# loro-dev/loro

Hardware: AMD Instinct MI355X
Metric: merged docs/sec (batch of N docs x M remote ops) (higher is better)
Workload: dtype u32; 1 GPU; configs[1]: 10000 docs/GPU x 100000-op automerge-paper-shaped text trace, 2 concurrent peers, 3 FastUpdates blobs/doc (4683 op runs, 30 changes, 103435 blob bytes/doc); docs_per_gpu=10000, ops_per_doc=100000, contexts_in_flight=2, streams_per_context=2

## Files before the change

loro_amd/csrc/lm_k_dag.h:

```cpp
#pragma once
#include "lm_k_decode.h"

namespace lm {

#ifndef LM_FUSE_ROWS
#define LM_FUSE_ROWS 1
#endif
#ifndef LM_NO_NODE_CUT
#define LM_NO_NODE_CUT 0
#endif

struct DevDag {
  uint32_t* blk_sorted;
  uint32_t* chg_node;
  uint32_t* node_done;
  uint32_t* node_lam;
};

LM_KERNEL void k_doc_ranges(Dev d) {
  uint32_t doc = (uint32_t)(lmw::bid() * lmw::bdim() + lmw::tid());
  if (doc >= d.n_docs) return;
  DocMeta m;
  uint32_t* mw = (uint32_t*)&m;
  for (uint32_t i = 0; i < sizeof(DocMeta) / 4; i++) mw[i] = 0;
// ... 34 lines not shown
  if (m.status == ST_MF_BAIL) { if (lane == 0) { d.doc[doc].status = ST_DATA_CORRUPTION; d.doc[doc].flags = DF_REDO; } return; }
  if (status_fatal(m.status)) { if (lane == 0) d.doc[doc].status = m.status; return; }
  uint32_t P = 0;
  bool too_many = false;
  for (uint32_t i = 0; i < m.n_praw; i++) {
    uint64_t v = d.peer_raw[m.praw0 + i];
    bool hit = false;
    for (uint32_t k = (uint32_t)lane; k < P; k += 64) hit |= s_peers[k] == v;
    if (!lmw::any(hit)) {
      if (P >= MAX_PEERS - 1) { too_many = true; break; }
      if (lane == 0) s_peers[P] = v;
      P++;
      lmw::block_sync();
    }
  }
  if (too_many) { if (lane == 0) LM_SETERR(d.doc[doc].status, ST_UNSUPPORTED); return; }
  lmw::block_sync();
  for (uint32_t e = (uint32_t)lane; e < P; e += 64) {
    uint64_t v = s_peers[e];
    uint32_t rank = 0;
    for (uint32_t j = 0; j < P; j++) rank += s_peers[j] < v ? 1u : 0u;
    d.peer_uniq[m.praw0 + rank] = v;
  }
  lmw::block_sync();
  for (uint32_t i = (uint32_t)lane; i < m.n_praw; i += 64) {
    uint64_t v = d.peer_raw[m.praw0 + i];
    uint32_t lo = 0, hi = P;
    while (lo < hi) { uint32_t mid = (lo + hi) >> 1; if (d.peer_uniq[m.praw0 + mid] < v) lo = mid + 1; else hi = mid; }
    d.peer_map[m.praw0 + i] = lo;
  }
  lmw::block_sync();
  uint32_t C = 0;
  bool cont_overflow = false;
  for (uint32_t i = 0; i < m.n_cid; i++) {
    const uint32_t* w = d.cid_raw + (uint64_t)(m.cid0 + i) * 4;
    uint32_t kr = w[0], blk = w[3];
    const uint32_t* bo = d.boff + (uint64_t)blk * BCN;
    bool is_root = (kr & 0x100) != 0;
    uint64_t noff = 0;
    uint32_t nlen = 0, cpeer = 0, cctr = 0;
    if (is_root) { noff = d.key_off[bo[BC_KEY] + w[2]]; nlen = d.key_len[bo[BC_KEY] + w[2]]; }
    else { cpeer = d.peer_map[bo[BC_PEER] + w[1]]; cctr = w[2]; }
    uint32_t idx = NONE;
    for (uint32_t c0 = 0; c0 < C && idx == NONE; c0 += 64) {
      bool match = false;
      if (c0 + (uint32_t)lane < C) {
        ContRow c = d.cont[m.cid0 + c0 + lane];
        if (c.kind_root == kr) {
          if (is_root) {
            if (c.name_len == nlen) {
              match = true;
              const uint8_t* a = d.data + c.name_off;
              const uint8_t* b = d.data + noff;
              for (uint32_t k = 0; k < nlen; k++) if (a[k] != b[k]) { match = false; break; }
            }
          } else match = c.peer == cpeer && c.counter == cctr;
        }
      }
      uint64_t mm = lmw::ballot(match);
      if (mm) idx = c0 + (uint32_t)lmw::ffs64(mm);
    }
    if (idx != NONE) {}
    else {
      if (C >= MAX_CONTAINERS) { cont_overflow = true; break; }
      idx = C;
      if (lane == 0) {
        ContRow c;
        c.name_off = noff; c.name_len = nlen; c.kind_root = kr; c.peer = cpeer; c.counter = cctr; c.touched = 0; c.pad = 0;
        d.cont[m.cid0 + C] = c;
      }
      C++;
      lmw::block_sync();
    }
    if (lane == 0) d.cid_map[m.cid0 + i] = idx;
  }
  if (lane == 0) {
    d.doc[doc].status = cont_overflow ? ST_UNSUPPORTED : m.status;
    d.doc[doc].n_peers = P;
    d.doc[doc].n_cont = C;
  }
  (void)s_n;
}

LM_KERNEL void k_remap(Dev d, uint32_t n_ops, uint32_t n_chg) {
  uint32_t t = (uint32_t)(lmw::bid() * lmw::bdim() + lmw::tid());
  uint32_t m_chg = NONE, m_bit = 0;
  if (t < n_ops) {
    uint32_t blk = d.op_blk[t];
    const BlockDesc& bd = d.blk[blk];
    if (bd.status == ST_OK && d.doc[bd.doc].status == ST_OK) {
      const uint32_t* bo = d.boff + (uint64_t)blk * BCN;
      OpRow r = d.op[t];
      uint32_t local = r.cidx_kind & 0xffff, kind = (r.cidx_kind >> 16) & 0xff;
      uint32_t ci = d.cid_map[bo[BC_CID] + local];
      if (r.cidx_kind & OPF_NESTED) {
        const uint8_t* vend = d.data + bd.base + bd.sec_rel[SEC_VALUES] + bd.sec_len[SEC_VALUES];
        Rd v{d.data + d.op_val[t], vend, false};
        uint32_t n_keys = d.bcnt[(uint64_t)blk * BCN + BC_KEY];
        if (kind == OK_STYLE_START) { (void)rd_u8(v); (void)rd_uleb(v); (void)rd_uleb(v); }
        uint32_t vf = 0;
        skip_loro_value_keys(v, vf, n_keys);
        if ((vf & VF_CORRUPT) && !v.bad) LM_SETERR(d.doc[bd.doc].status, ST_DATA_CORRUPTION);
      }
      r.cidx_kind = ci | (kind << 16);
      if (kind == OK_DEL || kind == OK_LIST_MOVE || kind == OK_LIST_SET) r.a0 = d.peer_map[bo[BC_PEER] + r.a0];
      else if (kind == OK_MAP_SET || kind == OK_MAP_DEL) r.a0 = bo[BC_KEY] + (uint32_t)r.prop;
      d.op[t] = r;
      m_chg = r.chg; m_bit = ci & 63;
    }
  }
  {
    uint32_t p_chg = lmw::shfl_up(m_chg, 1), p_bit = lmw::shfl_up(m_bit, 1);
    bool lead = m_chg != NONE && (lmw::lane() == 0 || p_chg != m_chg || p_bit != m_bit);
    if (lead) lmw::atomic_or(&d.chg_mask[2 * (uint64_t)m_chg + (m_bit >> 5)], 1u << (m_bit & 31));
  }
  if (t < n_chg) {
    ChangeRow c = d.chg[t];
    const BlockDesc& bd = d.blk[c.blk];
    if (bd.status == ST_OK && d.doc[bd.doc].status == ST_OK) {
      const uint32_t* bo = d.boff + (uint64_t)c.blk * BCN;
      c.peer = d.peer_map[bo[BC_PEER] + 0];
      d.chg[t] = c;
      for (uint32_t k = c.dep0; k < c.dep0 + c.n_dep; k++) d.dep_peer[k] = d.peer_map[bo[BC_PEER] + d.dep_peer[k]];
    }
  }
}

LM_DEV uint32_t find_change(const Dev& d, const DocMeta& m, uint32_t peer, uint32_t c) {
  uint32_t lo = d.peer_chg0[m.praw0 + peer], hi = d.peer_chg1[m.praw0 + peer];
  uint32_t end = hi;
  while (lo < hi) {
    uint32_t mid = (lo + hi) >> 1;
    const ChangeRow& ch = d.chg[d.chg_sorted[m.chg0 + mid]];
    if (ch.ctr + ch.len <= c) lo = mid + 1; else hi = mid;
  }
  if (lo >= end) return NONE;
  const ChangeRow& ch = d.chg[d.chg_sorted[m.chg0 + lo]];
  return ch.ctr <= c ? lo : NONE;
}

#ifdef LM_PROF_DAG
#define DAG_PH(i) do { uint64_t n_ = lmw::clock(); dpacc[i] += n_ - dptp; dptp = n_; } while (0)
#else
#define DAG_PH(i) do {} while (0)
#endif
LM_DEV bool vvo_has(const Dev& d, uint32_t doc) { return d.vvo && d.vvo_off[doc + 1] - d.vvo_off[doc] > 8; }
LM_DEV uint64_t vvo_synth_peer(const Dev& d, uint32_t doc) { uint64_t v = 0; const uint8_t* p = d.vvo + d.vvo_off[doc]; for (int k = 0; k < 8; k++) v |= (uint64_t)p[k] << (8 * k); return v; }
LM_DEV uint32_t vvo_base_end(const Dev& d, uint32_t doc, uint64_t peer) {
  if (!vvo_has(d, doc)) return 0;
  Rd r = rd_make(d.vvo + d.vvo_off[doc] + 8, d.vvo_off[doc + 1] - d.vvo_off[doc] - 8);
  const uint64_t n = rd_uleb(r);
  for (uint64_t i = 0; i < n && !r.bad; i++) {
    const uint64_t q = rd_uleb(r);
    const uint64_t z = rd_uleb(r);
    if (q == peer) return (uint32_t)(z >> 1);
    if (q > peer) break;
  }
  return 0;
}
LM_KERNEL void k_dag_a(Dev d, DevDag g) {
  uint32_t doc = (uint32_t)lmw::bid();
  int lane = lmw::lane();
#ifdef LM_PROF_DAG
  uint64_t dpacc[8] = {0, 0, 0, 0, 0, 0, 0, 0}, dptp = lmw::clock();
#endif
  LM_SHARED(uint32_t, s_valid, MAX_PEERS);
  LM_SHARED(uint32_t, s_ext, MAX_PEERS);
  DocMeta m = d.doc[doc];
  if (status_fatal(m.status)) return;
  uint32_t P = m.n_peers;
  for (uint32_t i = (uint32_t)lane; i < m.n_blk; i += 64) {
    uint32_t bi = m.blk0 + i;
    const BlockDesc& b = d.blk[bi];
    uint64_t key = ((uint64_t)d.chg[d.boff[(uint64_t)bi * BCN + BC_CHG]].peer << 32) | b.counter_start;
    uint32_t rank = 0;
    for (uint32_t j = 0; j < m.n_blk; j++) {
      uint32_t bj = m.blk0 + j;
      uint64_t kj = ((uint64_t)d.chg[d.boff[(uint64_t)bj * BCN + BC_CHG]].peer << 32) | d.blk[bj].counter_start;
      rank += (kj < key || (kj == key && j < i)) ? 1u : 0u;
    }
    g.blk_sorted[m.blk0 + rank] = bi;
  }
  for (uint32_t p = (uint32_t)lane; p < P; p += 64) { s_ext[p] = vvo_base_end(d, doc, d.peer_uniq[m.praw0 + p]); d.peer_base[m.praw0 + p] = s_ext[p]; s_valid[p] = 0; d.peer_chg0[m.praw0 + p] = 0; d.peer_chg1[m.praw0 + p] = 0; }
  lmw::block_sync();
  DAG_PH(0);
  uint32_t n_sorted = 0;
  bool any_skip = false;
  uint32_t pending = 0;
  uint32_t cur_peer = NONE, covered = 0;
  bool gap = false;
  for (uint32_t i = 0; i < m.n_blk; i++) {
    uint32_t bi = g.blk_sorted[m.blk0 + i];
    const BlockDesc& b = d.blk[bi];
    uint32_t c0 = d.boff[(uint64_t)bi * BCN + BC_CHG];
    uint32_t peer = d.chg[c0].peer;
    if (peer != cur_peer) {
      if (cur_peer != NONE && lane == 0) { s_ext[cur_peer] = covered; d.peer_chg1[m.praw0 + cur_peer] = n_sorted; }
      cur_peer = peer; covered = s_ext[peer]; gap = false;
      if (lane == 0) d.peer_chg0[m.praw0 + peer] = n_sorted;
    }
    if (b.counter_start > covered) gap = true;
    uint32_t bend = b.counter_start + b.counter_len;
    for (uint32_t k0 = 0; k0 < b.n_changes; k0 += 64) {
      uint32_t k = k0 + (uint32_t)lane;
      bool in = k < b.n_changes;
      uint32_t row = c0 + (in ? k : 0);
      ChangeRow ch = d.chg[row];
// ... 60 lines not shown
  for (uint32_t p = (uint32_t)lane; p < P; p += 64) { d.peer_chg0[m.praw0 + p] = NONE; d.peer_chg1[m.praw0 + p] = 0; }
  lmw::block_sync();
  for (uint32_t i = (uint32_t)lane; i < n_valid; i += 64) {
    uint32_t peer = d.chg[d.chg_sorted[m.chg0 + i]].peer;
    uint32_t prev = i ? d.chg[d.chg_sorted[m.chg0 + i - 1]].peer : NONE;
    uint32_t next = i + 1 < n_valid ? d.chg[d.chg_sorted[m.chg0 + i + 1]].peer : NONE;
    if (prev != peer) d.peer_chg0[m.praw0 + peer] = i;
    if (next != peer) d.peer_chg1[m.praw0 + peer] = i + 1;
  }
  lmw::block_sync();
  for (uint32_t p = (uint32_t)lane; p < P; p += 64) {
    if (d.peer_chg0[m.praw0 + p] == NONE) { d.peer_chg0[m.praw0 + p] = 0; d.peer_chg1[m.praw0 + p] = 0; }
    d.peer_end[m.praw0 + p] = s_valid[p];
    d.peer_ext[m.praw0 + p] = s_ext[p];
  }
  {
    uint32_t run = 0;
    for (uint32_t p0 = 0; p0 < P; p0 += 64) {
      uint32_t p = p0 + (uint32_t)lane;
      uint32_t e = p < P ? s_ext[p] : 0;
      uint32_t inc = lmw::scan_incl_add(e);
      if (p < P) d.elem_base[m.praw0 + p] = run + inc - e;
      run += lmw::bcast(inc, 63);
    }
    if (vvo_has(d, doc)) { if (run > m.atoms && lane == 0) d.doc[doc].atoms = run; }
    else if (run > m.atoms && lane == 0) LM_SETERR(d.doc[doc].status, ST_INTERNAL);
  }
  lmw::mem_fence();
  lmw::block_sync();
  DAG_PH(4);
  for (uint32_t i = (uint32_t)lane; i < n_valid; i += 64) {
    uint32_t row = d.chg_sorted[m.chg0 + i];
    const ChangeRow& ch = d.chg[row];
    for (uint32_t k = ch.dep0; k < ch.dep0 + ch.n_dep; k++) {
      uint32_t q = d.dep_peer[k], c = d.dep_ctr[k];
      uint32_t ci = NONE;
      if (q == ch.peer && i > 0 && c + 1 == ch.ctr) {
        const ChangeRow& pv = d.chg[d.chg_sorted[m.chg0 + i - 1]];
        if (pv.peer == q && pv.ctr <= c && c < pv.ctr + pv.len) ci = i - 1;
      }
      if (ci == NONE && q < P) ci = find_change(d, m, q, c);
      d.dep_ci[k] = ci;
      if (q != ch.peer && ci != NONE && d.chg_skip[row] == 0)
        lmw::atomic_or(&d.chg_flag[d.chg_sorted[m.chg0 + ci]], 2u);
    }
  }
  lmw::mem_fence();
  lmw::block_sync();
  DAG_PH(5);
  const bool cut_doc = !LM_NO_NODE_CUT && m.n_op >= d.cut_min_rows;
  uint32_t n_nodes = 0;
  for (uint32_t i0 = 0; i0 < n_valid; i0 += 64) {
    uint32_t i = i0 + (uint32_t)lane;
    bool in = i < n_valid;
    bool head = false;
    if (in) {
      uint32_t row = d.chg_sorted[m.chg0 + i];
      const ChangeRow& ch = d.chg[row];
      bool cont = false;
      if (d.chg_skip[row] != 0) cont = true;
      else if (ch.n_dep == 1 && d.dep_peer[ch.dep0] == ch.peer && ch.ctr > 0 && d.dep_ctr[ch.dep0] == ch.ctr - 1) cont = true;
      if (cont && (i == 0 || d.chg[d.chg_sorted[m.chg0 + i - 1]].peer != ch.peer)) cont = false;
      if (cont && cut_doc && d.chg_skip[row] == 0 && (d.chg_flag[d.chg_sorted[m.chg0 + i - 1]] & 2u)) cont = false;
      head = !cont;
    }
    uint64_t hm = lmw::ballot(head);
    uint32_t nid = n_nodes + (uint32_t)lmw::popc64(hm & ((2ull << lane) - 1)) - 1;
    if (in) {
      g.chg_node[m.chg0 + i] = nid;
      if (head) d.node_first[m.chg0 + nid] = i;
    }
    n_nodes += (uint32_t)lmw::popc64(hm);
  }
  lmw::block_sync();
  for (uint32_t n = (uint32_t)lane; n < n_nodes; n += 64) {
    d.node_last[m.chg0 + n] = (n + 1 < n_nodes ? d.node_first[m.chg0 + n + 1] : n_valid) - 1;
    g.node_done[m.chg0 + n] = 0;
  }
  DAG_PH(6);
  uint32_t n_map = 0, n_el = 0, n_style = 0;
  for (uint32_t i = (uint32_t)lane; i < m.n_blk; i += 64) {
    const BlockDesc& kb = d.blk[m.blk0 + i];
    if (kb.status != ST_OK) continue;
    n_map += kb.flags & 0x7fffffffu; n_el += kb.pad; n_style += kb.flags >> 31;
  }
  bool has_ml = false;
  for (uint32_t c = (uint32_t)lane; c < m.n_cont; c += 64) has_ml |= (d.cont[m.cid0 + c].kind_root & 0xff) == CK_MOVABLE;
  has_ml = lmw::any(has_ml);
  bool any_skip_doc = lmw::any(any_skip);
  n_map = lmw::reduce_add(n_map);
  n_el = lmw::reduce_add(n_el);
  n_style = lmw::reduce_add(n_style);
  if (lane == 0) {
    d.doc[doc].n_valid_chg = n_valid;
    d.doc[doc].n_nodes = n_nodes;
    d.doc[doc].pending_lo = pending;
    d.doc[doc].pending_hi = 0;
    d.doc[doc].n_mapop = n_map;
    d.doc[doc].n_elems = n_el;
    if (cut_doc) d.doc[doc].flags |= DF_CUT;
    if (has_ml) d.doc[doc].flags |= DF_MOVABLE;
    else if (!any_skip_doc && n_style == 0) d.doc[doc].flags |= DF_PLAIN | ((LM_FUSE_ROWS && (uint64_t)n_valid * 8 > m.n_op) ? DF_FUSED : 0u);
  }
#ifdef LM_PROF_DAG
  DAG_PH(7);
  if (lane == 0) for (int i = 0; i < 8; i++) atomicAdd(&d.prof[i], (unsigned long long)dpacc[i]);
#endif
}

LM_KERNEL void k_dag_b(Dev d, DevDag g, uint32_t res_mode) {
  uint32_t doc = (uint32_t)lmw::bid();
  int lane = lmw::lane();
  DocMeta m = d.doc[doc];
  if (status_fatal(m.status)) return;
  uint32_t P = m.n_peers, N = m.n_nodes;
  uint64_t vvh0 = ((uint64_t)m.vvh0_hi << 32) | m.vvh0_lo;
  uint32_t n_done = 0;
  if (res_mode == 2) {
    for (uint32_t p = (uint32_t)lane; p < P; p += 64) d.peer_end[m.praw0 + p] = d.peer_end_all[m.praw0 + p];
    lmw::mem_fence();
    lmw::block_sync();
    N = 0;
  }
  LM_SHARED(uint32_t, s_next, MAX_PEERS);
  LM_SHARED(uint32_t, s_pend, MAX_PEERS);
  for (uint32_t p = (uint32_t)lane; p < P; p += 64) { s_next[p] = 0; s_pend[p] = 0; }
  lmw::block_sync();
  if (res_mode != 2)
    for (uint32_t n = (uint32_t)lane; n < N; n += 64) {
      uint32_t pr = d.chg[d.chg_sorted[m.chg0 + d.node_first[m.chg0 + n]]].peer;
      uint32_t prev = n ? d.chg[d.chg_sorted[m.chg0 + d.node_first[m.chg0 + n - 1]]].peer : NONE;
      uint32_t next = n + 1 < N ? d.chg[d.chg_sorted[m.chg0 + d.node_first[m.chg0 + n + 1]]].peer : NONE;
      if (pr < P && prev != pr) s_next[pr] = n;
      if (pr < P && next != pr) s_pend[pr] = n + 1;
    }
  lmw::block_sync();
  for (uint32_t pass = 0; pass <= N && n_done < N; pass++) {
    uint32_t batch0 = n_done;
    if (m.flags & DF_CUT) {
    {
      uint32_t pick = NONE;
      for (uint32_t p0 = ((P - 1) >> 6) << 6;; p0 -= 64) {
        uint32_t pr = p0 + (uint32_t)lane;
        uint32_t n = pr < P ? s_next[pr] : NONE;
        bool ready = false;
        if (pr < P && n < s_pend[pr] && !g.node_done[m.chg0 + n]) {
          ready = true;
          const ChangeRow& ch = d.chg[d.chg_sorted[m.chg0 + d.node_first[m.chg0 + n]]];
          for (uint32_t k = ch.dep0; k < ch.dep0 + ch.n_dep; k++) {
            uint32_t ci = d.dep_ci[k];
            if (ci == NONE || !g.node_done[m.chg0 + g.chg_node[m.chg0 + ci]]) ready = false;
          }
        }
        uint64_t rm = lmw::ballot(ready);
        if (rm) { pick = p0 + (uint32_t)(63 - __builtin_clzll((unsigned long long)rm)); break; }
        if (p0 == 0) break;
      }
      if (pick != NONE) {
        lmw::block_sync();
        uint32_t n = s_next[pick];
        lmw::block_sync();
        if (lane == 0) { d.node_order[m.chg0 + n_done] = n; s_next[pick] = n + 1; }
        n_done++;
      }
    }
    } else {
    for (uint32_t p0 = 0; p0 < P; p0 += 64) {
// ... 79 lines not shown
    cnt = rd_uleb(r);
    if (r.bad || cnt > f1 - f0) ferr = ST_DECODE_ERROR;
    for (uint64_t i = 0; i < cnt && !ferr; i++) {
      uint64_t peer = rd_uleb(r);
      int64_t ctr = rd_zigzag(r);
      if (r.bad) { ferr = ST_DECODE_ERROR; break; }
      uint32_t lo = 0, hi = P;
      while (lo < hi) { uint32_t mid = (lo + hi) >> 1; if (d.peer_uniq[m.praw0 + mid] < peer) lo = mid + 1; else hi = mid; }
      if (lo >= P || d.peer_uniq[m.praw0 + lo] != peer || ctr < 0 || (uint64_t)ctr >= d.peer_end[m.praw0 + lo] ||
          find_change(d, m, lo, (uint32_t)ctr) == NONE)
        ferr = ST_FRONTIERS_NOT_FOUND;
    }
    if (!ferr && rd_left(r) != 0) ferr = ST_DECODE_ERROR;
  }
  lmw::block_sync();
  if (ferr && res_mode == 2) { if (lane == 0) { d.doc[doc].front_err = ferr; d.doc[doc].flags |= DF_FRONT_ERR; } return; }
  if (ferr) { if (lane == 0) LM_SETERR(d.doc[doc].status, ferr); return; }
  if (res_mode == 0) for (uint32_t p = (uint32_t)lane; p < P; p += 64) d.peer_end_all[m.praw0 + p] = d.peer_end[m.praw0 + p];
  lmw::block_sync();
  for (uint32_t p0 = 0; p0 < P; p0 += 64) {
    uint32_t p = p0 + (uint32_t)lane, acc = 0;
    Rd r = rd_make(d.front + f0, f1 - f0);
    (void)rd_uleb(r);
    for (uint64_t i = 0; i < cnt; i++) {
      uint64_t peer = rd_uleb(r);
      uint32_t ctr = (uint32_t)rd_zigzag(r);
      uint32_t lo = 0, hi = P;
      while (lo < hi) { uint32_t mid = (lo + hi) >> 1; if (d.peer_uniq[m.praw0 + mid] < peer) lo = mid + 1; else hi = mid; }
      uint32_t ci = find_change(d, m, lo, ctr);
      if (p < P) {
        uint32_t x = d.vvh[vvh0 + (uint64_t)g.chg_node[m.chg0 + ci] * P + p];
        if (p == lo && ctr + 1 > x) x = ctr + 1;
        acc = x > acc ? x : acc;
      }
    }
    if (p < P) d.peer_end[m.praw0 + p] = acc;
  }
}

template <bool BYTES>
LM_DEV bool fill_text_coop(const Dev& d, const uint8_t* s, uint32_t nbytes, uint64_t e0, uint32_t len) {
  uint32_t lane = (uint32_t)lmw::lane();
  bool bad = false;
  uint32_t n = 0;
  for (uint32_t c = 0; c < nbytes;) {
    uint32_t i = c + lane;
    bool inb = i < nbytes;
    uint32_t b = inb ? s[i] : 0u;
    if (!lmw::ballot(b >= 0x80)) {
      if (inb & (n + lane < len)) { if (BYTES) d.tb[e0 + n + lane] = (uint8_t)b; else d.cp[e0 + n + lane] = b; }
      uint32_t took = nbytes - c < 64 ? nbytes - c : 64u;
      n += took; c += 64;
      continue;
    }
    bool last_chunk = c + 61 >= nbytes;
    bool mine = inb & (last_chunk | (lane < 61));
    bool lead = mine & ((b & 0xC0) != 0x80);
    uint32_t b1 = lmw::shfl(b, (int)((lane + 1) & 63)), b2 = lmw::shfl(b, (int)((lane + 2) & 63)), b3 = lmw::shfl(b, (int)((lane + 3) & 63));
    uint64_t lm_ = lmw::ballot(lead);
    uint32_t rank = (uint32_t)lmw::popc64(lm_ & ((1ull << lane) - 1));
    if (lead) {
      uint32_t cpv, extra;
      if (b < 0x80) { cpv = b; extra = 0; }
      else if ((b & 0xE0) == 0xC0) { cpv = ((b & 0x1F) << 6) | (b1 & 0x3F); extra = 1; }
      else if ((b & 0xF0) == 0xE0) { cpv = ((b & 0x0F) << 12) | ((b1 & 0x3F) << 6) | (b2 & 0x3F); extra = 2; }
      else if ((b & 0xF8) == 0xF0) { cpv = ((b & 0x07) << 18) | ((b1 & 0x3F) << 12) | ((b2 & 0x3F) << 6) | (b3 & 0x3F); extra = 3; }
      else { cpv = 0; extra = 0; bad = true; }
      if (i + extra >= nbytes) bad = true;
      if (extra >= 1 && (b1 & 0xC0) != 0x80) bad = true;
      if (extra >= 2 && (b2 & 0xC0) != 0x80) bad = true;
      if (extra >= 3 && (b3 & 0xC0) != 0x80) bad = true;
      if (lane + extra > 63) bad = true;
      if (n + rank < len) {
        if (BYTES) { d.tb[e0 + n + rank] = (uint8_t)(extra ? TB_WIDE : cpv); if (extra) d.cp[e0 + n + rank] = cpv; }
        else d.cp[e0 + n + rank] = cpv;
      }
    }
    n += (uint32_t)lmw::popc64(lm_);
    c += 61;
  }
  return lmw::any(bad) || n != len;
}

LM_KERNEL void k_elem_fill(Dev d) {
  uint32_t bi = (uint32_t)lmw::bid();
  int lane = lmw::lane();
  const BlockDesc& bd = d.blk[bi];
  if (bd.status != ST_OK) return;
  uint32_t doc = bd.doc;
  const DocMeta& m = d.doc[doc];
  if (status_fatal(m.status)) return;
  if (d.res_old_blobs && (m.flags & DF_FILL_KEPT) && bd.blob - d.doc_blob[doc] < d.res_old_blobs[doc]) return;
  const bool span = d.span != 0;
  const uint32_t* off = d.boff + (uint64_t)bi * BCN;
  uint32_t op0 = off[BC_OP], n_op = d.bcnt[(uint64_t)bi * BCN + BC_OP];
  uint32_t chg0 = off[BC_CHG];
  uint32_t peer = d.chg[chg0].peer;
  uint64_t ebase = (((uint64_t)m.elem0_hi << 32) | m.elem0_lo) + d.elem_base[m.praw0 + peer];
  uint32_t ext = d.peer_ext[m.praw0 + peer];
  uint64_t doc_data0 = d.blob_off[d.doc_blob[doc]];
  const uint8_t* vsec = d.data + bd.base + bd.sec_rel[SEC_VALUES];
  const uint8_t* lim = vsec + bd.sec_len[SEC_VALUES];
  LM_SHARED(uint32_t, s_inc, 64);
  LM_SHARED(uint32_t, s_nb, 64);
  LM_SHARED(uint32_t, s_src, 64);
  LM_SHARED(uint32_t, s_dst, 64);
  bool bad = false;
  for (uint32_t g0 = 0; g0 < n_op; g0 += 64) {
    uint32_t row = op0 + g0 + (uint32_t)lane;
    bool valid = g0 + (uint32_t)lane < n_op;
    OpRow r;
    r.cidx_kind = 0; r.prop = 0; r.len = 0; r.ctr = 0; r.a0 = r.a1 = 0; r.a2 = 0; r.chg = 0;
    if (valid) r = d.op[row];
    uint32_t kind = (r.cidx_kind >> 16) & 0xff;
    bool want = valid && (kind == OK_TEXT_INS || kind == OK_LIST_INS || kind == OK_STYLE_START || kind == OK_STYLE_END);
    const bool cand_text = want && kind == OK_TEXT_INS;
    if (want && !d.chg_flag[r.chg]) want = false;
    if (want && r.ctr + r.len > ext) want = false;
    if (cand_text && !want) {
      const uint8_t* q = d.data + d.op_val[row];
      Rd vq = rd_make(q, q < lim ? (uint64_t)(lim - q) : 0ull);
      uint64_t nb = rd_uleb(vq);
      if (vq.bad || nb > rd_left(vq)) bad = true;
      else {
        uint32_t n = 0;
        for (uint64_t i = 0; i < nb && !bad;) {
          uint32_t b0 = vq.p[i], extra = b0 < 0x80 ? 0u : (b0 & 0xE0) == 0xC0 ? 1u : (b0 & 0xF0) == 0xE0 ? 2u : (b0 & 0xF8) == 0xF0 ? 3u : 4u;
          if (extra == 4 || i + extra >= nb + (extra ? 0 : 1)) { bad = true; break; }
          for (uint32_t k = 1; k <= extra; k++) if ((vq.p[i + k] & 0xC0) != 0x80) bad = true;
          n++; i += extra + 1;
        }
        if (n != r.len) bad = true;
      }
    }
    uint64_t e0 = ebase + r.ctr;
    if (want && (kind == OK_STYLE_START || kind == OK_STYLE_END)) { if (span) d.tb[e0] = (uint8_t)TB_ANCHOR; d.cp[e0] = CP_ANCHOR | (row - m.op0); want = false; }
    const uint8_t* p = want ? d.data + d.op_val[row] : lim;
    Rd v = rd_make(p, (uint64_t)(lim - p));
    uint64_t nbytes = 0;
    bool is_long = false, flat = false;
    if (want && kind == OK_TEXT_INS) {
      nbytes = rd_uleb(v);
      if (v.bad || nbytes > rd_left(v)) { bad = true; want = false; }
      else if (span && nbytes == r.len) flat = true;
      else if (nbytes > 64) { is_long = true; }
      else {
        const uint8_t* s = v.p;
        uint32_t n = 0;
        for (uint32_t i = 0; i < (uint32_t)nbytes;) {
          if (span && i + 4 <= (uint32_t)nbytes && n + 3 < r.len) {
            uint32_t w = ld32u(s + i);
            if (!(w & 0x80808080u)) { st32u(d.tb + e0 + n, w); n += 4; i += 4; continue; }
          }
          if (!span && i + 4 <= (uint32_t)nbytes) {
            uint32_t q0 = s[i], q1 = s[i + 1], q2 = s[i + 2], q3 = s[i + 3];
            if (((q0 | q1 | q2 | q3) & 0x80) == 0) {
              if (n + 3 < r.len) { d.cp[e0 + n] = q0; d.cp[e0 + n + 1] = q1; d.cp[e0 + n + 2] = q2; d.cp[e0 + n + 3] = q3; }
              else { if (n < r.len) d.cp[e0 + n] = q0; if (n + 1 < r.len) d.cp[e0 + n + 1] = q1; if (n + 2 < r.len) d.cp[e0 + n + 2] = q2; }
              n += 4; i += 4;
              continue;
            }
          }
          uint32_t b = s[i], cpv, extra;
          if (b < 0x80) { cpv = b; extra = 0; }
          else if ((b & 0xE0) == 0xC0) { cpv = b & 0x1F; extra = 1; }
          else if ((b & 0xF0) == 0xE0) { cpv = b & 0x0F; extra = 2; }
          else if ((b & 0xF8) == 0xF0) { cpv = b & 0x07; extra = 3; }
          else { bad = true; break; }
          if (i + extra >= (uint32_t)nbytes) { bad = true; break; }
          for (uint32_t k = 1; k <= extra; k++) {
            uint32_t t = s[i + k];
            if ((t & 0xC0) != 0x80) bad = true;
            cpv = (cpv << 6) | (t & 0x3F);
          }
          if (n < r.len) {
            if (span) { d.tb[e0 + n] = (uint8_t)(extra ? TB_WIDE : cpv); if (extra) d.cp[e0 + n] = cpv; }
            else d.cp[e0 + n] = cpv;
          }
          n++;
          i += extra + 1;
        }
        if (n != r.len) bad = true;
      }
    } else if (want) {
      (void)rd_u8(v);
      uint64_t cnt = rd_uleb(v);
      if (cnt != r.len) bad = true;
      for (uint32_t k = 0; k < r.len && !bad; k++) {
        d.cp[e0 + k] = (uint32_t)((uint64_t)(v.p - d.data) - doc_data0);
        bool u = false;
        skip_loro_value(v, u);
        if (v.bad) bad = true;
      }
    }
    if (span) {
      uint32_t nd = flat ? ((uint32_t)nbytes + 3) / 4 : 0u;
      uint32_t inc = lmw::scan_incl_add(nd);
      uint32_t total = lmw::bcast(inc, 63);
      if (total) {
        lmw::block_sync();
        s_inc[lane] = inc; s_nb[lane] = (uint32_t)nbytes; s_src[lane] = (uint32_t)(v.p - vsec); s_dst[lane] = r.ctr;
        lmw::block_sync();
        uint32_t hi = 0;
        for (uint32_t f0 = 0; f0 < total; f0 += 64) {
          uint32_t f = f0 + (uint32_t)lane;
          if (f < total) {
            uint32_t lo = 0, hh = 63;
            while (lo < hh) { uint32_t mid = (lo + hh) >> 1; if (s_inc[mid] > f) hh = mid; else lo = mid + 1; }
            uint32_t nbr = s_nb[lo];
            uint32_t k4 = 4u * (f - (s_inc[lo] - (nbr + 3) / 4));
            const uint8_t* src = vsec + s_src[lo] + k4;
            uint8_t* dst = d.tb + ebase + s_dst[lo] + k4;
            if (k4 + 4 <= nbr) { uint32_t w = ld32u(src); hi |= w; st32u(dst, w); }
            else for (uint32_t i = 0; k4 + i < nbr; i++) { uint32_t b = src[i]; hi |= b; dst[i] = (uint8_t)b; }
          }
        }
        if (hi & 0x80808080u) bad = true;
      }
    }
    uint64_t lm_ = lmw::ballot(is_long);
    while (lm_) {
      int l = lmw::ffs64(lm_);
      lm_ &= lm_ - 1;
      uint64_t sp = (uint64_t)(v.p - d.data);
      uint32_t sp_lo = lmw::bcast((uint32_t)sp, l), sp_hi = lmw::bcast((uint32_t)(sp >> 32), l);
      uint32_t nb = lmw::bcast((uint32_t)nbytes, l);
      uint32_t e_lo = lmw::bcast((uint32_t)e0, l), e_hi = lmw::bcast((uint32_t)(e0 >> 32), l);
      uint32_t ln = lmw::bcast(r.len, l);
      const uint8_t* str = d.data + (((uint64_t)sp_hi << 32) | sp_lo);
      uint64_t e0l = ((uint64_t)e_hi << 32) | e_lo;
      if (span ? fill_text_coop<true>(d, str, nb, e0l, ln) : fill_text_coop<false>(d, str, nb, e0l, ln)) bad = true;
    }
  }
  if (lmw::any(bad) && lane == 0) LM_SETERR(d.doc[doc].status, ST_DATA_CORRUPTION);
}

}
```

loro_amd/csrc/lm_k_decode.h:

```cpp
#pragma once
#include "lm_dev_util.h"

namespace lm {

struct Dev {
  const uint8_t* data;
  const uint64_t* blob_off;
  const uint32_t* blob_len;
  const uint32_t* doc_blob;
  uint32_t n_blobs, n_docs;
  uint32_t span;
  const uint32_t* res_old_blobs;
  uint32_t loc_cleared;
  uint32_t* posdel;
  const uint64_t* posdel_off;
  uint32_t* pd_row_idx;
  const uint8_t* vvo;
  const uint64_t* vvo_off;
  const uint8_t* doc_fused;
  uint32_t n_op_rows;
  uint32_t* blk_kind;
  uint32_t posdel_redo;
  uint32_t no_linear;
  uint32_t res_vis;
// ... 338 lines not shown
      lmw::atomic_add(&d.dec_stat[0], 1u); lmw::atomic_max32(&d.dec_stat[1], span);
      lmw::atomic_max32(&d.dec_stat[2], (uint32_t)((bd.base + bd.sec_rel[SEC_OPS]) & 15) + bd.sec_rel[SEC_VALUES] - bd.sec_rel[SEC_OPS]);
    }
  }
  c[BC_CHG] = N;
  c[BC_DEP] = (uint32_t)ndep;
  c[BC_OP] = fused ? 0u : (uint32_t)nops;
  c[BC_KEY] = (uint32_t)nkeys;
  c[BC_CID] = (uint32_t)ncid;
  c[BC_PEER] = (uint32_t)np;
  c[BC_MAPOP] = fused ? (uint32_t)nops : 0u;
  c[BC_ATOMS] = bd.counter_len;
}

static constexpr uint32_t VF_UNSUPPORTED = 1u, VF_CORRUPT = 2u;
template <bool KEYS = false, class R> LM_DEV void skip_loro_value_fs(R& r, uint32_t& vf, int cdepth, uint32_t* f_cnt, uint32_t n_keys = 0xffffffffu);
template <class R> LM_DEV void skip_loro_value_top(R& r, uint32_t& vf, int cdepth, uint32_t* f_cnt, uint32_t tag_peek) {
  if (tag_peek > 6 || r.bad) { skip_loro_value_fs(r, vf, cdepth, f_cnt); return; }
  (void)rd_u8(r);
  if (tag_peek == 3) (void)rd_sleb(r);
  else if (tag_peek == 4) rd_skip(r, 8);
  else if (tag_peek >= 5) { uint64_t l = rd_uleb(r); rd_skip(r, l); }
}
template <bool KEYS, class R> LM_DEV void skip_loro_value_fs(R& r, uint32_t& vf, int cdepth, uint32_t* f_cnt, uint32_t n_keys) {
  uint32_t f_map = 0;
  int sp = 0;
  uint32_t cnt = 1;
  bool in_map = false;
  for (uint32_t guard = 0; guard < (1u << 28); guard++) {
    while (cnt == 0) {
      if (sp == 0) return;
      sp--;
      cnt = f_cnt[sp];
      in_map = (f_map >> sp) & 1;
    }
    if (r.bad) return;
    cnt--;
    if (in_map) {
      uint64_t kidx = rd_uleb(r);
      if (KEYS) vf |= (kidx >= n_keys && !r.bad) ? VF_CORRUPT : 0u;
    }
    uint32_t tag = rd_u8(r);
    switch (tag) {
      case 0: case 1: case 2: break;
      case 3: (void)rd_sleb(r); break;
      case 4: rd_skip(r, 8); break;
      case 5: case 6: { uint64_t l = rd_uleb(r); rd_skip(r, l); break; }
      case 7: case 8: {
        uint64_t n = rd_uleb(r);
        if (KEYS) vf |= (n > (1u << 28) && !r.bad) ? VF_CORRUPT : 0u;
        if (n > (1u << 28) || sp >= 16) { r.bad = true; return; }
        f_cnt[sp] = cnt;
        f_map = (f_map & ~(1u << sp)) | ((in_map ? 1u : 0u) << sp);
        sp++;
        cnt = (uint32_t)n;
        in_map = tag == 8;
        break;
      }
      case 9: { (void)rd_u8(r); if (sp > cdepth) vf |= VF_UNSUPPORTED; break; }
      default: if (KEYS) vf |= r.bad ? 0u : VF_CORRUPT; r.bad = true; return;
    }
  }
  r.bad = true;
}
LM_DEV void skip_loro_value(Rd& r, uint32_t& vf, int cdepth = -1) {
  uint32_t f_cnt[16];
  skip_loro_value_fs(r, vf, cdepth, f_cnt);
}
LM_DEV void skip_loro_value_keys(Rd& r, uint32_t& vf, uint32_t n_keys) {
  uint32_t f_cnt[16];
  skip_loro_value_fs<true>(r, vf, -1, f_cnt, n_keys);
}
LM_DEV void skip_loro_value(Rd& r, bool& unsupported, int cdepth = -1) {
  uint32_t vf = 0;
  skip_loro_value(r, vf, cdepth);
  if (vf & VF_UNSUPPORTED) unsupported = true;
}

#if defined(LM_EMU) && defined(LM_EMU_TRACE)
#define DEC_ST(code) do { if (!st) { if (getenv("LM_EMU_DEC")) fprintf(stderr, "lm emu: block verdict " #code " at %s:%d\n", __FILE__, __LINE__); st = (code); } } while (0)
#else
#define DEC_ST(code) do { st = st ? st : (code); } while (0)
#endif
LM_DEV void kc_add(uint32_t& n_map, uint32_t& n_el, uint32_t& n_style, uint32_t k, uint32_t len) {
  n_map += (k == OK_MAP_SET || k == OK_MAP_DEL || k == OK_LIST_MOVE || k == OK_LIST_SET || k == OK_OTHER) ? 1u : 0u;
  n_el += (k == OK_TEXT_INS || k == OK_LIST_INS || k == OK_STYLE_START || k == OK_STYLE_END) ? len : (k == OK_LIST_MOVE ? 1u : 0u);
  n_style += (k == OK_STYLE_START || k == OK_STYLE_END) ? 1u : 0u;
}
LM_DEV uint32_t kc_pack(uint32_t n_map, uint32_t n_style) { return (n_map & 0x7fffffffu) | (n_style ? 0x80000000u : 0u); }

static constexpr uint32_t DEC_RECLASS = 0xDEC0DE01u;
template <bool EXACT> LM_DEV void lane_skip_value(Rd& r, uint32_t& vf, int cdepth, uint32_t n_keys) {
  uint32_t f_cnt[16];
  if (EXACT) skip_loro_value_fs<true>(r, vf, cdepth, f_cnt, n_keys);
  else skip_loro_value_fs(r, vf, cdepth, f_cnt);
}
template <bool EXACT, bool HEAD = false> LM_DEV void block_decode_lane(Dev d) {
  uint32_t bi = (uint32_t)(lmw::bid() * lmw::bdim() + lmw::tid());
  if (bi >= d.n_blocks) return;
  BlockDesc bd = d.blk[bi];
  if (EXACT ? ((bd.status != ST_DECODE_ERROR && bd.status != ST_DATA_CORRUPTION) || bd.pad != DEC_RECLASS) : (bd.status != ST_OK)) return;
  if (HEAD != (d.doc_fused && d.doc_fused[bd.doc])) return;
  const uint32_t* off = d.boff + (uint64_t)bi * BCN;
  const uint32_t* cnt = d.bcnt + (uint64_t)bi * BCN;
  uint32_t N = bd.n_changes;
  uint32_t chg0 = off[BC_CHG], dep0 = off[BC_DEP], op0 = off[BC_OP], key0 = off[BC_KEY], cid0 = off[BC_CID], peer0 = off[BC_PEER];
  uint32_t n_peers = cnt[BC_PEER], n_ops = cnt[BC_OP], n_keys = cnt[BC_KEY], n_cids = cnt[BC_CID];
  int32_t st = ST_OK;
  bool unsupported = false;
  uint32_t kc_map = 0, kc_el = 0, kc_style = 0;
  Rd h = blk_sec(d, bd, SEC_HEADER);
  (void)rd_uleb(h);
  for (uint32_t i = 0; i < n_peers; i++) {
    uint64_t v = 0;
    for (int k = 0; k < 8; k++) v |= (uint64_t)rd_u8(h) << (8 * k);
    d.peer_raw[peer0 + i] = v;
  }
  {
    uint64_t known = 0;
    uint32_t ctr = bd.counter_start;
    for (uint32_t i = 0; i < N; i++) {
      uint64_t l;
      if (i + 1 < N) { l = rd_uleb(h); known += l; if (known > bd.counter_len) { st = ST_DECODE_ERROR; l = 0; } }
      else l = bd.counter_len - (known > bd.counter_len ? bd.counter_len : known);
      ChangeRow c;
      c.peer = 0; c.ctr = ctr; c.len = (uint32_t)l; c.dep0 = 0; c.n_dep = 0; c.op0 = 0; c.n_op = 0; c.blk = bi;
      d.chg[chg0 + i] = c;
      ctr += (uint32_t)l;
    }
    BoolCur bc = bool_make(h);
    for (uint32_t i = 0; i < N; i++) d.chg[chg0 + i].op0 = bool_next(bc) ? 1u : 0u;
    if (bc.rem != 0) bc.r.bad = true;
    RleCur dc = rle_make(bc.r);
    uint32_t dcur = dep0;
    uint64_t others_total = 0;
    for (uint32_t i = 0; i < N; i++) {
      uint64_t others = rle_next_uvar(dc);
      ChangeRow c = d.chg[chg0 + i];
      uint32_t ds = c.op0;
      if (dcur + ds + others > dep0 + cnt[BC_DEP]) { st = ST_DECODE_ERROR; others = 0; ds = 0; }
      others_total += others;
      c.dep0 = dcur;
      c.n_dep = ds + (uint32_t)others;
      if (ds) {
        if (c.ctr == 0) st = ST_DECODE_ERROR;
        d.dep_peer[dcur] = 0;
        d.dep_ctr[dcur] = c.ctr ? c.ctr - 1 : 0;
      }
      dcur += c.n_dep;
      d.chg[chg0 + i] = c;
    }
    if (dc.rem != 0) dc.r.bad = true;
    if (dcur - dep0 != cnt[BC_DEP]) st = ST_DECODE_ERROR;
    RleCur pc = rle_make(dc.r);
    uint64_t D = 0;
    for (uint32_t i = 0; i < N && others_total; i++) {
      ChangeRow c = d.chg[chg0 + i];
      for (uint32_t k = c.dep0 + c.op0; k < c.dep0 + c.n_dep; k++) {
        uint64_t pi = rle_next_uvar(pc);
        if (pi >= n_peers) { st = ST_DECODE_ERROR; pi = 0; }
        d.dep_peer[k] = (uint32_t)pi;
        D++;
      }
    }
    if (pc.rem != 0) pc.r.bad = true;
    Rd hr = pc.r;
    DodCur dd = dod_make(hr);
    for (uint32_t i = 0; i < N && D; i++) {
      ChangeRow c = d.chg[chg0 + i];
      for (uint32_t k = c.dep0 + c.op0; k < c.dep0 + c.n_dep; k++) {
        int64_t v = dod_next(dd);
        if (v < 0 || v >= (int64_t)MAX_COUNTER) { st = st ? st : ST_DECODE_ERROR; v = 0; }
// ... 18 lines not shown
    dod_skip(td, N);
    dod_finish(td, m, N);
    RleCur mc = rle_make(m);
    const uint64_t tot = rle_sum_uvar(mc, N);
    if (mc.rem != 0) mc.r.bad = true;
    if (mc.r.bad || tot > rd_left(mc.r)) DEC_ST(ST_DATA_CORRUPTION);
  }
  if (!HEAD) {
    Rd k = blk_sec(d, bd, SEC_KEYS);
    for (uint32_t i = 0; i < n_keys; i++) {
      uint64_t l = rd_uleb(k);
      d.key_off[key0 + i] = (uint64_t)(k.p - d.data);
      d.key_len[key0 + i] = (uint32_t)l;
      rd_skip(k, l);
    }
    if (k.bad) st = st ? st : ST_DECODE_ERROR;
  }
  uint32_t head_root = 0;
  {
    Rd k = blk_sec(d, bd, SEC_CIDS);
    if (n_cids) (void)rd_uleb(k);
    for (uint32_t i = 0; i < n_cids; i++) {
      uint64_t fields = rd_uleb(k);
      uint32_t is_root = rd_u8(k), kind = rd_u8(k);
      uint64_t pidx = rd_uleb(k);
      int64_t koc = rd_zigzag(k);
      if (fields != 4) st = st ? st : ST_DECODE_ERROR;
      uint32_t* w = d.cid_raw + (uint64_t)(cid0 + i) * 4;
      if (HEAD && is_root) {
        Rd kk = blk_sec(d, bd, SEC_KEYS);
        bool found = koc >= 0;
        uint64_t l = 0;
        for (int64_t q = 0; found && q <= koc; q++) { if (kk.p >= kk.end) { found = false; break; } l = rd_uleb(kk); if (q < koc) rd_skip(kk, l); if (kk.bad) found = false; }
        if (found && l > rd_left(kk)) found = false;
        if (!found || head_root >= n_keys) { DEC_ST(ST_DATA_CORRUPTION); d.key_off[key0 + (head_root < n_keys ? head_root : 0)] = 0; d.key_len[key0 + (head_root < n_keys ? head_root : 0)] = 0; koc = 0; }
        else { d.key_off[key0 + head_root] = (uint64_t)(kk.p - d.data); d.key_len[key0 + head_root] = (uint32_t)l; koc = head_root; }
        head_root++;
      }
      else if (is_root) { if (koc < 0 || (uint64_t)koc >= n_keys) { DEC_ST(ST_DATA_CORRUPTION); koc = 0; } }
      else { if (pidx >= n_peers) { DEC_ST(ST_DATA_CORRUPTION); pidx = 0; } if (koc < 0 || koc >= (int64_t)MAX_COUNTER) { st = st ? st : ST_UNSUPPORTED; koc = 0; } }
      w[0] = kind | (is_root ? 0x100u : 0u);
      w[1] = (uint32_t)pidx;
      w[2] = (uint32_t)koc;
      w[3] = bi;
    }
    if (k.bad) st = st ? st : ST_DECODE_ERROR;
  }
  if (HEAD) {
    d.blk[bi].status = (st != ST_OK || unsupported) ? (int32_t)ST_MF_BAIL : (int32_t)ST_OK;
    d.blk[bi].flags = kc_pack(d.blk_kind[bi] & 0x7fffffffu, 0); d.blk[bi].pad = 0;
    return;
  }
  {
    Rd o = blk_sec(d, bd, SEC_OPS);
    (void)rd_uleb(o); (void)rd_uleb(o);
    RleCur c_cont = rle_make(rd_bytes(o));
    RleCur c_prop = rle_make(rd_bytes(o));
    RleCur c_vt = rle_make(rd_bytes(o));
    RleCur c_len = rle_make(rd_bytes(o));
    Rd dsec = blk_sec(d, bd, SEC_DEL);
    bool has_del = dsec.p < dsec.end;
    RleCur d_peer = rle_make(dsec), d_ctr = rle_make(dsec), d_len = rle_make(dsec);
    if (has_del) {
      uint64_t outer = rd_uleb(dsec), ncols = rd_uleb(dsec);
      if (outer != 1 || ncols != 3) st = st ? st : ST_DECODE_ERROR;
      d_peer = rle_make(rd_bytes(dsec));
      d_ctr = rle_make(rd_bytes(dsec));
      d_len = rle_make(rd_bytes(dsec));
    }
    {
      bool colbad = false;
      { RleCur t = c_cont; uint32_t n = rle_drain(t, 2, n_ops); colbad |= t.r.bad || n != n_ops; }
      { RleCur t = c_prop; uint32_t n = rle_drain(t, 2, n_ops); colbad |= t.r.bad || n != n_ops; }
      { RleCur t = c_vt; uint32_t n = rle_drain(t, 0, n_ops); colbad |= t.r.bad || n != n_ops; }
      { RleCur t = c_len; uint32_t n = rle_drain(t, 1, n_ops); colbad |= t.r.bad || n != n_ops; }
      if (has_del) {
        RleCur t1 = d_peer, t2 = d_ctr, t3 = d_len;
        uint32_t n1 = rle_drain(t1, 2), n2 = rle_drain(t2, 2), n3 = rle_drain(t3, 2);
        colbad |= t1.r.bad || t2.r.bad || t3.r.bad || n1 != n2 || n1 != n3;
      }
      if (colbad) st = st ? st : ST_DECODE_ERROR;
    }
    Rd v = blk_sec(d, bd, SEC_VALUES);
    uint64_t counter = bd.counter_start;
    uint32_t change_index = 0;
    uint64_t next_boundary = N > 1 ? d.chg[chg0 + 1].ctr : (uint64_t)bd.counter_start + bd.counter_len;
    d.chg[chg0].op0 = op0;
    for (uint32_t row = 0; row < n_ops; row++) {
      int64_t ci = rle_next_delta(c_cont);
      int64_t prop = rle_next_delta(c_prop);
      uint32_t vt = rle_next_u8(c_vt) & 0x7f;
      uint64_t len = rle_next_uvar(c_len);
      if (ci < 0 || (uint64_t)ci >= n_cids) { DEC_ST(ST_DATA_CORRUPTION); ci = 0; }
      if (prop < INT32_MIN || prop > INT32_MAX) { st = st ? st : ST_DECODE_ERROR; prop = 0; }
      uint32_t ckind = n_cids ? (d.cid_raw[(uint64_t)(cid0 + (uint32_t)ci) * 4] & 0xff) : 0xff;
      OpRow r;
      r.cidx_kind = (uint32_t)ci;
      r.prop = (int32_t)prop;
      r.len = (uint32_t)len;
      r.ctr = (uint32_t)counter;
      r.a0 = 0; r.a1 = 0; r.a2 = 0;
      r.chg = chg0 + change_index;
      uint64_t val_at = (uint64_t)(v.p - d.data);
      uint32_t kind = OK_OTHER;
      uint32_t mark_len = 0;
      uint64_t mv_from = 0, mv_peer = 0, mv_lam = 0;
      uint32_t vfl = 0;
      bool nested = false;
      bool is_list_value = false;
      switch (vt) {
        case 0: case 1: case 2: case 8: case 9: break;
        case 3: (void)rd_sleb(v); break;
        case 4: rd_skip(v, 8); break;
        case 5: case 6: { uint64_t l = rd_uleb(v); rd_skip(v, l); break; }
        case 7: (void)rd_uleb(v); break;
        case 10: (void)rd_sleb(v); break;
        case 11: {
          is_list_value = v.p < v.end && *v.p == 7;
          nested = v.p < v.end && (*v.p == 7 || *v.p == 8);
          if (is_list_value) {
            Rd t = v;
            (void)rd_u8(t);
            r.a0 = (uint32_t)rd_uleb(t);
          }
          lane_skip_value<EXACT>(v, vfl, ckind == CK_MAP ? 0 : (is_list_value && (ckind == CK_LIST || ckind == CK_MOVABLE) ? 1 : (ckind > CK_TEXT && ckind != CK_MOVABLE ? 16 : -1)), n_keys);
          break;
        }
        case 12: {
          (void)rd_u8(v);
          mark_len = (uint32_t)rd_uleb(v);
          uint64_t key_idx = rd_uleb(v);
          if (key_idx >= n_keys) DEC_ST(ST_DATA_CORRUPTION);
          uint32_t u = 0;
          lane_skip_value<EXACT>(v, u, -1, n_keys);
          vfl |= u & VF_CORRUPT;
          nested = true;
          break;
        }
        case 13: { (void)rd_uleb(v); uint32_t isn = rd_u8(v); (void)rd_uleb(v); if (!isn) (void)rd_uleb(v); break; }
        case 14: mv_from = rd_uleb(v); mv_peer = rd_uleb(v); mv_lam = rd_uleb(v); break;
        case 15: {
          mv_peer = rd_uleb(v); mv_lam = rd_uleb(v);
          val_at = (uint64_t)(v.p - d.data);
          if (ckind == CK_MOVABLE) lane_skip_value<EXACT>(v, vfl, 0, n_keys);
          else { uint32_t u = 0; lane_skip_value<EXACT>(v, u, -1, n_keys); vfl |= u & VF_CORRUPT; }
          nested = true;
          break;
        }
        case 16: {
          (void)rd_uleb(v); (void)rd_uleb(v); (void)rd_uleb(v);
          uint32_t isn = rd_u8(v);
          if (!isn) { (void)rd_uleb(v); (void)rd_uleb(v); }
          break;
        }
        default: { uint64_t l = rd_uleb(v); rd_skip(v, l); break; }
      }
      if (vfl & VF_UNSUPPORTED) unsupported = true;
      if (vfl & VF_CORRUPT) DEC_ST(ST_DATA_CORRUPTION);
      if (EXACT && v.bad) DEC_ST(ST_DECODE_ERROR);
      bool take_del = false;
      if (ckind == CK_TEXT) {
        if (vt == 5) kind = OK_TEXT_INS;
        else if (vt == 9) { kind = OK_DEL; take_del = true; }
        else if (vt == 12) { kind = OK_STYLE_START; r.a0 = mark_len; }
        else if (vt == 0) kind = OK_STYLE_END;
        else DEC_ST(ST_DATA_CORRUPTION);
      } else if (ckind == CK_MAP) {
        if (prop < 0 || (uint64_t)prop >= n_keys) DEC_ST(ST_DATA_CORRUPTION);
        if (vt == 8) kind = OK_MAP_DEL;
        else if (vt == 11) kind = OK_MAP_SET;
        else DEC_ST(ST_DATA_CORRUPTION);
      } else if (ckind == CK_LIST) {
        if (vt == 11) { if (is_list_value) kind = OK_LIST_INS; else DEC_ST(ST_DATA_CORRUPTION); }
        else if (vt == 9) { kind = OK_DEL; take_del = true; }
        else DEC_ST(ST_DATA_CORRUPTION);
      } else if (ckind == CK_MOVABLE) {
        if (vt == 11) { if (is_list_value) kind = OK_LIST_INS; else DEC_ST(ST_DATA_CORRUPTION); }
        else if (vt == 9) { kind = OK_DEL; take_del = true; }
        else if (vt == 14 || vt == 15) {
          kind = vt == 14 ? OK_LIST_MOVE : OK_LIST_SET;
          if (mv_peer >= n_peers || mv_lam > 0xFFFFFFFFull || mv_from > 0x7FFFFFFFull || prop < 0 || len != 1) { DEC_ST(ST_DATA_CORRUPTION); mv_peer = 0; }
          r.a0 = (uint32_t)mv_peer; r.a1 = (uint32_t)mv_lam; r.a2 = (int32_t)(uint32_t)mv_from;
        } else DEC_ST(ST_DATA_CORRUPTION);
      }
      if (take_del) {
        if (!has_del) DEC_ST(ST_DATA_CORRUPTION);
        else {
          int64_t dp = rle_next_delta(d_peer), dctr = rle_next_delta(d_ctr), dl = rle_next_delta(d_len);
          if (dp < 0 || (uint64_t)dp >= n_peers) { DEC_ST(ST_DATA_CORRUPTION); dp = 0; }
          if (dl == 0 || dl > (int64_t)MAX_COUNTER || dl < -(int64_t)MAX_COUNTER) { DEC_ST(ST_DATA_CORRUPTION); dl = 1; }
          if (dctr < 0 || dctr >= (int64_t)MAX_COUNTER) { DEC_ST(ST_DATA_CORRUPTION); dctr = 0; }
          r.a0 = (uint32_t)dp; r.a1 = (uint32_t)dctr; r.a2 = (int32_t)dl;
          if (d_peer.r.bad || d_ctr.r.bad || d_len.r.bad) DEC_ST(ST_DATA_CORRUPTION);
        }
      }
      r.cidx_kind |= (kind << 16) | ((nested && (vt != 12 || kind == OK_STYLE_START)) ? OPF_NESTED : 0u);
      kc_add(kc_map, kc_el, kc_style, kind, (uint32_t)len);
      d.op[op0 + row] = r;
      d.op_val[op0 + row] = val_at;
      d.op_blk[op0 + row] = bi;
      counter += len;
      if (counter > MAX_COUNTER) { st = st ? st : ST_UNSUPPORTED; counter = MAX_COUNTER; }
      if (change_index >= N) { DEC_ST(ST_DATA_CORRUPTION); change_index = N - 1; }
      d.chg[chg0 + change_index].n_op++;
      if (counter > next_boundary && change_index + 1 < N) DEC_ST(ST_DATA_CORRUPTION);
      if (counter >= next_boundary && change_index + 1 < N) {
        change_index++;
        d.chg[chg0 + change_index].op0 = op0 + row + 1;
        next_boundary = change_index + 1 < N ? d.chg[chg0 + change_index + 1].ctr : (uint64_t)bd.counter_start + bd.counter_len;
      }
    }
    for (uint32_t i = 1; i < N; i++) if (d.chg[chg0 + i].n_op == 0) d.chg[chg0 + i].op0 = op0 + n_ops;
    if (c_cont.r.bad || c_prop.r.bad || c_vt.r.bad || c_len.r.bad || v.bad) st = st ? st : ST_DECODE_ERROR;
    if (counter != (uint64_t)bd.counter_start + bd.counter_len) DEC_ST(ST_DATA_CORRUPTION);
  }
  if (EXACT) { if (st == ST_DATA_CORRUPTION || st == ST_DECODE_ERROR) d.blk[bi].status = st; return; }
  if (st == ST_OK && unsupported) st = ST_UNSUPPORTED;
  d.blk[bi].status = st;
  d.blk[bi].flags = kc_pack(kc_map, kc_style); d.blk[bi].pad = (st == ST_DECODE_ERROR || st == ST_DATA_CORRUPTION) ? DEC_RECLASS : kc_el;
}
LM_KERNEL void k_block_decode(Dev d) { block_decode_lane<false>(d); }
LM_KERNEL void k_block_head(Dev d) { block_decode_lane<false, true>(d); }
LM_KERNEL void k_block_reclassify(Dev d) { block_decode_lane<true>(d); }

}

#include "lm_k_decode_wave.h"
```

loro_amd/csrc/lm_k_decode_wave.h:

```cpp
#pragma once

namespace lm {

#ifndef LM_DEC_G
#define LM_DEC_G 8
#endif
#ifndef LM_NO_PARTIAL_STAGE
#define LM_NO_PARTIAL_STAGE 0
#endif
static constexpr uint32_t DEC_G = LM_DEC_G;
static constexpr uint32_t DEC_R = 8;
static constexpr uint32_t DEC_WW = 6;
static constexpr uint32_t DEC_VW2 = 128;
static constexpr uint32_t DEC_LDS_FIXED = DEC_G * 16 * 4 + DEC_G * DEC_R * 8 * 4 + DEC_G * DEC_R * DEC_WW * 4 + DEC_G * DEC_VW + DEC_G * DEC_VW2;
static constexpr uint32_t DEC_KINDS = 16;
LM_DEV void dec_err(uint32_t& key, uint32_t row, uint32_t prio, int32_t code) {
  uint32_t k = (row << 8) | (prio << 4) | (uint32_t)code;
  if (k < key) key = k;
}

#ifdef LM_PROF_DEC
#define DEC_PH(i) do { uint64_t n_ = lmw::clock(); pacc[i] += n_ - ptp; ptp = n_; } while (0)
#else
#define DEC_PH(i) do {} while (0)
// ... 234 lines not shown
    }
    {
      Rd m = sec(SEC_META);
      DodCur td = dod_make(m);
      dod_skip(td, N);
      dod_finish(td, m, N);
      RleCur mc = rle_make(m);
      const uint64_t tot = rle_sum_uvar(mc, N);
      if (mc.rem != 0) mc.r.bad = true;
      if (mc.r.bad || tot > rd_left(mc.r)) st = st ? st : ST_DATA_CORRUPTION;
    }
    {
      Rd k = sec(SEC_KEYS);
      for (uint32_t i = 0; i < n_keys; i++) {
        uint64_t l = rd_uleb(k);
        d.key_off[key0 + i] = abs_of(k.p);
        d.key_len[key0 + i] = (uint32_t)l;
        rd_skip(k, l);
      }
      if (k.bad) st = st ? st : ST_DECODE_ERROR;
    }
    {
      Rd k = sec(SEC_CIDS);
      if (n_cids) (void)rd_uleb(k);
      for (uint32_t i = 0; i < n_cids; i++) {
        uint64_t fields = rd_uleb(k);
        uint32_t is_root = rd_u8(k), kind = rd_u8(k);
        uint64_t pidx = rd_uleb(k);
        int64_t koc = rd_zigzag(k);
        if (fields != 4) st = st ? st : ST_DECODE_ERROR;
        uint32_t* w = d.cid_raw + (uint64_t)(cid0 + i) * 4;
        if (is_root) { if (koc < 0 || (uint64_t)koc >= n_keys) { st = st ? st : ST_DATA_CORRUPTION; koc = 0; } }
        else { if (pidx >= n_peers) { st = st ? st : ST_DATA_CORRUPTION; pidx = 0; } if (koc < 0 || koc >= (int64_t)MAX_COUNTER) { st = st ? st : ST_UNSUPPORTED; koc = 0; } }
        w[0] = kind | (is_root ? 0x100u : 0u);
        w[1] = (uint32_t)pidx;
        w[2] = (uint32_t)koc;
        w[3] = bi;
        if (i < DEC_KINDS) s_kinds[b * DEC_KINDS + i] = (uint8_t)kind;
      }
      if (k.bad) st = st ? st : ST_DECODE_ERROR;
    }
  }
  lmw::block_sync();
  DEC_PH(1);
  RleCur col = rle_make(rd_make(blk_p, 0));
  ColCur fcol = col_make((lm_lds_bytes)slot, 0, 0, false);
  bool has_del = false;
  uint32_t errk = 0xffffffffu;
  uint32_t kc_map = 0, kc_el = 0, kc_style = 0;
  bool colbad = false;
  uint32_t n_del_read = 0;
  bool shape_bad = false;
  if (ok) {
    Rd o = sec(SEC_OPS);
    uint64_t outer = rd_uleb(o), ncols = rd_uleb(o);
    Rd mine = rd_make(blk_p, 0);
    for (uint32_t c = 0; c < 4; c++) { Rd cc = rd_bytes(o); if (r == c) mine = cc; }
    if (outer != 1 || ncols != 4 || o.bad) shape_bad = true;
    Rd ds = sec(SEC_DEL);
    has_del = ds.p < ds.end;
    if (has_del) {
      uint64_t douter = rd_uleb(ds), dcols = rd_uleb(ds);
      if (douter != 1 || dcols != 3) shape_bad = true;
      for (uint32_t c = 4; c < 7; c++) { Rd cc = rd_bytes(ds); if (r == c) mine = cc; }
    }
    col = rle_make(mine);
    if (staged) fcol = col_make((lm_lds_bytes)slot, (uint32_t)(mine.p - (const uint8_t*)slot), (uint32_t)(mine.end - (const uint8_t*)slot), mine.bad);
  }
  uint32_t mode = r == 2 ? 0u : (r == 3 ? 1u : 2u);
  int64_t v_lo = 0, v_repl = 0;
  uint64_t v_span = 256;
  uint32_t v_prio = 0, v_mask = 0xffffffffu;
  int32_t v_code = ST_DATA_CORRUPTION;
  bool v_nz = false;
  if (r == 0) { v_span = n_cids; v_prio = 0; }
  else if (r == 1) { v_lo = INT32_MIN; v_span = 1ull << 32; v_prio = 1; v_code = ST_DECODE_ERROR; }
  else if (r == 2) { v_mask = 0x7f; }
  else if (r == 3) { v_span = (uint64_t)MAX_COUNTER + 1; v_repl = MAX_COUNTER; v_prio = 5; v_code = ST_UNSUPPORTED; }
  else if (r == 4) { v_span = n_peers; v_prio = 6; }
  else if (r == 5) { v_span = MAX_COUNTER; v_prio = 8; }
  else if (r == 6) { v_lo = -(int64_t)MAX_COUNTER; v_span = 2ull * MAX_COUNTER + 1; v_nz = true; v_repl = 1; v_prio = 7; }
  Rd v = rd_make(blk_p, 0);
  const uint64_t v_end_abs = ok ? bd.base + bdp->sec_rel[SEC_VALUES] + bdp->sec_len[SEC_VALUES] : 0ull;
  uint64_t counter = bd.counter_start;
  uint32_t change_index = 0, rows_in_change = 0;
  uint64_t next_boundary = 0;
  Rd hl7 = rd_make(d.data, 0);
  uint64_t kn7 = 0;
  auto next_len7 = [&]() -> uint64_t { uint64_t l = rd_uleb(hl7); kn7 += l; return kn7 > bd.counter_len ? 0ull : l; };
  bool unsupported = false;
  if (ok && r == 7) {
    v = rd_make(d.data + bd.base + bdp->sec_rel[SEC_VALUES], bdp->sec_len[SEC_VALUES]);
    hl7 = sec(SEC_HEADER);
    (void)rd_uleb(hl7);
    rd_skip(hl7, (uint64_t)n_peers * 8);
    next_boundary = N > 1 ? (uint64_t)bd.counter_start + next_len7() : (uint64_t)bd.counter_start + bd.counter_len;
    d.chg[chg0].op0 = op0;
  }
  uint32_t max_rows = lmw::reduce_max(ok ? n_ops : 0u);
  uint32_t* sx = s_x + (size_t)b * (DEC_R * 8);
  uint32_t* sw = s_w + (size_t)b * (DEC_R * DEC_WW);
  DEC_PH(2);
  for (uint32_t k = 0; k < DEC_R; k++) {
    if (ok && k < n_ops && r < 4) {
      int64_t w = staged ? col_next_any(fcol, mode) : rle_next_any(col, mode);
      if ((uint64_t)(w - v_lo) >= v_span) { dec_err(errk, k, v_prio, v_code); w = v_repl; }
      sx[k * 8 + r] = (uint32_t)w & v_mask;
    }
  }
  lmw::wave_sync();
  for (uint32_t c0 = 0; c0 < max_rows; c0 += DEC_R) {
    DEC_PH(3);
    uint32_t row = c0 + r;
    bool act = ok && row < n_ops;
    uint32_t ci = 0, prop = 0, vt = 0, len = 0;
    if (act) { ci = sx[r * 8]; prop = sx[r * 8 + 1]; vt = sx[r * 8 + 2]; len = sx[r * 8 + 3]; }
    uint32_t ckind = 0xff;
    if (act && n_cids) ckind = ci < DEC_KINDS ? s_kinds[b * DEC_KINDS + ci] : (d.cid_raw[(uint64_t)(cid0 + ci) * 4] & 0xff);
    bool take_del = act && vt == 9 && (ckind == CK_TEXT || ckind == CK_LIST || ckind == CK_MOVABLE);
    if (act) sx[r * 8 + 7] = ckind;
    uint64_t tdm = lmw::ballot(take_del && has_del);
    uint32_t todo = (r >= 4 && r < 7) ? (uint32_t)(tdm >> (b * 8)) & 0xffu : 0u;
    DEC_PH(4);
    {
      uint32_t wn = (ok && r == 7 && c0 < n_ops) ? (n_ops - c0 < DEC_R ? n_ops - c0 : DEC_R) : 0u;
      uint32_t* fs = s_fs + b * 16;
      bool spec = false;
      {
        const bool str_r = act && vt == 5;
        const uint32_t hdr_r = len < 128u ? 1u : (len < 16384u ? 2u : (len < 2097152u ? 3u : 4u));
        const uint32_t pay_r = str_r ? hdr_r + len : 0u;
        bool ok_r = !act || str_r || vt <= 2 || vt == 8 || vt == 9;
        if (lmw::any(str_r)) {
          uint32_t inc = lmw::scan_incl_add(pay_r);
          uint32_t base = lmw::shfl(inc, (int)(b ? b * 8 - 1 : 0));
          if (!b) base = 0;
          int wl_ = (int)(b * 8 + 7);
          uint64_t vp = (uint64_t)(v.p - d.data);
          uint64_t wpos = ((uint64_t)lmw::shfl((uint32_t)(vp >> 32), wl_) << 32) | lmw::shfl((uint32_t)vp, wl_);
          if (str_r) {
            uint64_t pos = wpos + (inc - pay_r - base);
            ok_r = pos + pay_r <= v_end_abs;
            if (ok_r) {
              uint32_t w4 = ld32u(d.data + pos);
              uint32_t b0 = w4 & 0xff, b1 = (w4 >> 8) & 0xff, b2 = (w4 >> 16) & 0xff, b3 = w4 >> 24;
              uint32_t val, used;
              if (!(b0 & 0x80)) { val = b0; used = 1; }
              else if (!(b1 & 0x80)) { val = (b0 & 0x7f) | (b1 << 7); used = 2; }
              else if (!(b2 & 0x80)) { val = (b0 & 0x7f) | ((b1 & 0x7f) << 7) | (b2 << 14); used = 3; }
              else { val = (b0 & 0x7f) | ((b1 & 0x7f) << 7) | ((b2 & 0x7f) << 14) | ((b3 & 0x7f) << 21); used = (b3 & 0x80) ? 0u : 4u; }
              ok_r = val == len && used == hdr_r;
            }
          }
          uint64_t okm = lmw::ballot(ok_r);
          spec = ((okm >> (b * 8)) & 0xffull) == 0xffull;
          uint32_t cinc = lmw::scan_incl_add(act ? len : 0u);
          uint32_t cbase = lmw::shfl(cinc, (int)(b ? b * 8 - 1 : 0));
          if (!b) cbase = 0;
          uint32_t tot_len = lmw::shfl(cinc, wl_) - cbase, tot_pay = lmw::shfl(inc, wl_) - base;
          uint32_t ctr7 = lmw::shfl((uint32_t)counter, wl_), ci7 = lmw::shfl(change_index, wl_);
          uint32_t nb7 = lmw::shfl((uint32_t)(next_boundary > 0xffffffffull ? 0xffffffffull : next_boundary), wl_);
          const bool whole = spec && ci7 < N && (uint64_t)ctr7 + tot_len <= MAX_COUNTER && ((uint64_t)ctr7 + tot_len < nb7 || ci7 + 1 >= N);
          if (whole) {
            if (act) {
              uint64_t va = wpos + (inc - pay_r - base);
              uint32_t* o = sw + r * DEC_WW;
              o[0] = (uint32_t)va; o[1] = (uint32_t)(va >> 32); o[2] = 0; o[3] = 0; o[4] = ctr7 + (cinc - len - cbase); o[5] = chg0 + ci7;
            }
            if (wn) { v.p += tot_pay; counter += tot_len; rows_in_change += wn; wn = 0; }
          }
        }
      }
#ifndef LM_NO_I64_FAST
      if (I64)
      {
        const bool int_r = act && vt == 11 && ckind == CK_MAP;
        const uint64_t cand_m = lmw::ballot(int_r || !act);
        const bool blk_cand = ((cand_m >> (b * 8)) & 0xffull) == 0xffull;
        const uint32_t wn_blk = lmw::shfl(wn, (int)(b * 8 + 7));
        if (lmw::any(blk_cand && wn_blk != 0)) {
          int wl_ = (int)(b * 8 + 7);
          uint64_t vp = (uint64_t)(v.p - d.data);
          uint64_t wpos = ((uint64_t)lmw::shfl((uint32_t)(vp >> 32), wl_) << 32) | lmw::shfl((uint32_t)vp, wl_);
          const bool go = blk_cand && wn_blk != 0;
          uint8_t* win = s_vw2 + (size_t)b * DEC_VW2;
          if (go && wpos + 16ull * r < v_end_abs) {
            struct V16b { uint32_t x, y, z, w; } pc;
            __builtin_memcpy(&pc, d.data + wpos + 16ull * r, 16);
            *(V16b*)(win + 16u * r) = pc;
          }
          lmw::wave_sync();
          bool ok_r = true;
          uint32_t st_k = 0, en_k = 0;
          if (go && act) {
            uint64_t left = v_end_abs - wpos;
            uint64_t t0 = 0, t1 = 0;
            const uint32_t* w32 = (const uint32_t*)win;
            for (uint32_t q = 0; q < 16; q++) {
              uint32_t x = ~w32[q] & 0x80808080u;
              uint64_t nib = ((x >> 7) & 1u) | ((x >> 14) & 2u) | ((x >> 21) & 4u) | ((x >> 28) & 8u);
              t0 |= nib << (4 * q);
            }
            for (uint32_t q = 16; q < 32; q++) {
              uint32_t x = ~w32[q] & 0x80808080u;
              uint64_t nib = ((x >> 7) & 1u) | ((x >> 14) & 2u) | ((x >> 21) & 4u) | ((x >> 28) & 8u);
              t1 |= nib << (4 * (q - 16));
            }
            if (left < 64) { t0 &= (1ull << left) - 1; t1 = 0; }
            else if (left < 128) t1 &= (1ull << (left - 64)) - 1;
            auto nth = [&](uint32_t n, uint32_t& pos) -> bool {
              uint64_t a = t0, bq = t1;
              uint32_t c0 = (uint32_t)lmw::popc64(a);
              if (n < c0) { for (uint32_t i = 0; i < n; i++) a &= a - 1; pos = (uint32_t)lmw::ffs64(a); return true; }
              n -= c0;
              if (n >= (uint32_t)lmw::popc64(bq)) return false;
              for (uint32_t i = 0; i < n; i++) bq &= bq - 1;
              pos = 64u + (uint32_t)lmw::ffs64(bq);
              return true;
            };
            ok_r = nth(2 * r, st_k) && nth(2 * r + 1, en_k);
            if (ok_r) ok_r = win[st_k] == 3 && en_k - st_k <= 10;
            if (ok_r) {
              uint32_t pen = 0;
              if (r == 0) ok_r = st_k == 0;
              else ok_r = nth(2 * r - 1, pen) && st_k == pen + 1;
            }
          }
          uint64_t okm = lmw::ballot(!go || !act || ok_r);
          const bool all_ok = go && ((okm >> (b * 8)) & 0xffull) == 0xffull;
          uint32_t n_act = (uint32_t)lmw::popc64((lmw::ballot(act) >> (b * 8)) & 0xffull);
          uint32_t last_en = lmw::shfl(en_k, (int)(b * 8 + (n_act ? n_act - 1 : 0)));
          uint32_t cinc = lmw::scan_incl_add(act ? len : 0u);
          uint32_t cbase = lmw::shfl(cinc, (int)(b ? b * 8 - 1 : 0));
          if (!b) cbase = 0;
          uint32_t tot_len = lmw::shfl(cinc, wl_) - cbase;
          uint32_t ctr7 = lmw::shfl((uint32_t)counter, wl_), ci7 = lmw::shfl(change_index, wl_);
          uint32_t nb7 = lmw::shfl((uint32_t)(next_boundary > 0xffffffffull ? 0xffffffffull : next_boundary), wl_);
          const bool whole = all_ok && n_act == wn_blk && ci7 < N && (uint64_t)ctr7 + tot_len <= MAX_COUNTER && ((uint64_t)ctr7 + tot_len < nb7 || ci7 + 1 >= N);
#ifdef LM_EMU_TRACE
          if (getenv("LM_EMU_I64") && go && r == 7) fprintf(stderr, "I64 %s\n", whole ? "fast" : (all_ok ? "boundary" : "declined"));
#endif
          if (whole) {
            if (act) {
              uint64_t va = wpos + st_k;
              uint32_t* o = sw + r * DEC_WW;
              o[0] = (uint32_t)va; o[1] = (uint32_t)(va >> 32); o[2] = 0; o[3] = 0; o[4] = ctr7 + (cinc - len - cbase); o[5] = chg0 + ci7;
            }
            if (wn) { v.p += last_en + 1; counter += tot_len; rows_in_change += wn; wn = 0; }
          }
        }
      }
#endif
      auto walk = [&](auto& v, const uint32_t k) {
        uint32_t wvt = sx[k * 8 + 2], wlen = sx[k * 8 + 3], wkind = sx[k * 8 + 7];
        uint64_t val_at = (uint64_t)(v.p - d.data);
        uint32_t aux = 0, flags = 0;
        uint32_t vfl = 0;
        switch (wvt) {
          case 0: case 1: case 2: case 8: case 9: break;
          case 3: (void)rd_sleb(v); break;
          case 4: rd_skip(v, 8); break;
          case 5: if (spec) { v.p += (wlen < 128u ? 1u : (wlen < 16384u ? 2u : (wlen < 2097152u ? 3u : 4u))) + wlen; break; }
            [[fallthrough]];
          case 6: { uint64_t l = rd_uleb(v); rd_skip(v, l); break; }
          case 7: (void)rd_uleb(v); break;
          case 10: (void)rd_sleb(v); break;
          case 11: {
            uint32_t tag0 = v.p < v.end ? rd_peek(v) : 0xffu;
            bool is_list_value = tag0 == 7;
            if (is_list_value) { auto t = v; (void)rd_u8(t); aux = (uint32_t)rd_uleb(t); flags = 1; }
            if (tag0 == 7 || tag0 == 8) flags |= 4;
            skip_loro_value_top(v, vfl, wkind == CK_MAP ? 0 : (is_list_value && (wkind == CK_LIST || wkind == CK_MOVABLE) ? 1 : (wkind > CK_TEXT && wkind != CK_MOVABLE ? 16 : -1)), fs, tag0);
            break;
          }
          case 12: {
            (void)rd_u8(v);
            aux = (uint32_t)rd_uleb(v);
            uint64_t key_idx = rd_uleb(v);
            if (key_idx >= n_keys) dec_err(errk, c0 + k, 2, ST_DATA_CORRUPTION);
            uint32_t u = 0;
            skip_loro_value_fs(v, u, -1, fs);
            vfl |= u & VF_CORRUPT;
            flags |= 4;
            break;
          }
          case 13: { (void)rd_uleb(v); uint32_t isn = rd_u8(v); (void)rd_uleb(v); if (!isn) (void)rd_uleb(v); break; }
          case 14: {
            uint64_t f = rd_uleb(v), pi = rd_uleb(v), lm_ = rd_uleb(v);
            if (pi >= n_peers || lm_ > 0xFFFFFFFFull || f > 0x7FFFFFFFull) flags |= 2;
            sx[k * 8 + 4] = (uint32_t)pi; sx[k * 8 + 5] = (uint32_t)lm_; sx[k * 8 + 6] = (uint32_t)f;
            break;
          }
          case 15: {
            uint64_t pi = rd_uleb(v), lm_ = rd_uleb(v);
            if (pi >= n_peers || lm_ > 0xFFFFFFFFull) flags |= 2;
            sx[k * 8 + 4] = (uint32_t)pi; sx[k * 8 + 5] = (uint32_t)lm_; sx[k * 8 + 6] = 0;
            val_at = (uint64_t)(v.p - d.data);
            if (wkind == CK_MOVABLE) skip_loro_value_fs(v, vfl, 0, fs);
            else { uint32_t u = 0; skip_loro_value_fs(v, u, -1, fs); vfl |= u & VF_CORRUPT; }
            flags |= 4;
            break;
          }
          case 16: {
            (void)rd_uleb(v); (void)rd_uleb(v); (void)rd_uleb(v);
            uint32_t isn = rd_u8(v);
            if (!isn) { (void)rd_uleb(v); (void)rd_uleb(v); }
            break;
          }
          default: { uint64_t l = rd_uleb(v); rd_skip(v, l); break; }
        }
        if (vfl & VF_UNSUPPORTED) unsupported = true;
        if (vfl & VF_CORRUPT) dec_err(errk, c0 + k, 2, ST_DATA_CORRUPTION);
        uint32_t* o = sw + k * DEC_WW;
        o[0] = (uint32_t)val_at; o[1] = (uint32_t)(val_at >> 32); o[2] = aux; o[3] = flags;
        o[4] = (uint32_t)counter; o[5] = chg0 + change_index;
        counter += wlen;
        if (counter > MAX_COUNTER) { dec_err(errk, c0 + k, 10, ST_UNSUPPORTED); counter = MAX_COUNTER; }
        if (change_index >= N) { dec_err(errk, c0 + k, 11, ST_DATA_CORRUPTION); change_index = N - 1; }
        rows_in_change++;
        if (counter > next_boundary && change_index + 1 < N) dec_err(errk, c0 + k, 12, ST_DATA_CORRUPTION);
        if (counter >= next_boundary && change_index + 1 < N) {
          d.chg[chg0 + change_index].n_op = rows_in_change;
          rows_in_change = 0;
          change_index++;
          d.chg[chg0 + change_index].op0 = op0 + c0 + k + 1;
          next_boundary = change_index + 1 < N ? next_boundary + next_len7() : (uint64_t)bd.counter_start + bd.counter_len;
        }
      };
      bool dense = false, jumps = false;
      for (uint32_t k = 0; k < wn; k++) { uint32_t t_ = sx[k * 8 + 2]; jumps |= t_ == 5 || t_ == 6 || t_ > 16; dense |= t_ == 3 || t_ == 4 || (t_ >= 10 && t_ <= 16); }
      dense &= !jumps;
      if (!lmw::any(dense)) {
        for (uint32_t k = 0; k < wn; k++) walk(v, k);
      } else {
        RdW w;
        w.p = v.p; w.end = v.end; w.bad = v.bad; w.wl = (lm_lds_bytes)(s_vw + (size_t)b * DEC_VW);
        uint32_t wk = 0;
        while (lmw::any(wk < wn)) {
          uint64_t vp = (uint64_t)(w.p - d.data);
          int wl_ = (int)(b * 8 + 7);
          uint64_t wpos = ((uint64_t)lmw::shfl((uint32_t)(vp >> 32), wl_) << 32) | lmw::shfl((uint32_t)vp, wl_);
          bool more = lmw::shfl((dense && wk < wn) ? 1u : 0u, wl_) != 0;
          if (more && wpos + 8ull * r < v_end_abs) {
            struct V8 { uint32_t x, y; } pc;
            __builtin_memcpy(&pc, d.data + wpos + 8ull * r, 8);
            *(V8*)(s_vw + (size_t)b * DEC_VW + 8u * r) = pc;
          }
          lmw::wave_sync();
          if (wk < wn) {
            w.wp = dense ? w.p : w.p - DEC_VW;
            for (bool first = true; wk < wn && (first || !dense || (uint64_t)(w.p - w.wp) + 12 <= DEC_VW); wk++, first = false) walk(w, wk);
          }
          lmw::wave_sync();
        }
        v.p = w.p; v.bad = w.bad;
      }
    }
    lmw::wave_sync();
    DEC_PH(5);
    for (uint32_t k = 0; k < DEC_R; k++) {
      const bool a1 = ok && r < 4 && c0 + DEC_R + k < n_ops, a2 = todo != 0;
      if (!lmw::any(a1 | a2)) break;
      if (a1 | a2) {
        uint32_t kk = a2 ? (uint32_t)__builtin_ctz(todo) : k;
        uint32_t rowx = a2 ? c0 + kk : c0 + DEC_R + k;
        todo &= todo - 1;
        const bool used_up = a2 && (staged ? col_exhausted(fcol) : rle_exhausted(col));
        int64_t w = used_up ? v_repl : (staged ? col_next_any(fcol, mode) : rle_next_any(col, mode));
        if (a2 && !used_up) { if (staged ? fcol.bad : col.r.bad) colbad = true; else n_del_read++; }
        if (!used_up && ((uint64_t)(w - v_lo) >= v_span || (v_nz && w == 0))) { dec_err(errk, rowx, v_prio, v_code); w = v_repl; }
        if (a2 && (used_up || (staged ? fcol.bad : col.r.bad))) dec_err(errk, rowx, 9, ST_DATA_CORRUPTION);
        sx[kk * 8 + r] = (uint32_t)w & v_mask;
      }
    }
    lmw::wave_sync();
    if (act) {
      const uint32_t* o = sw + r * DEC_WW;
      uint32_t aux = o[2];
      bool is_list_value = (o[3] & 1) != 0;
      OpRow orow;
      orow.cidx_kind = ci;
      orow.prop = (int32_t)prop;
      orow.len = len;
      orow.ctr = o[4];
      orow.a0 = (vt == 11 && is_list_value) ? aux : 0u; orow.a1 = 0; orow.a2 = 0;
      orow.chg = o[5];
      uint32_t kind = OK_OTHER;
      if (ckind == CK_TEXT) {
        if (vt == 5) kind = OK_TEXT_INS;
        else if (vt == 9) kind = OK_DEL;
        else if (vt == 12) { kind = OK_STYLE_START; orow.a0 = aux; }
        else if (vt == 0) kind = OK_STYLE_END;
        else dec_err(errk, row, 3, ST_DATA_CORRUPTION);
      } else if (ckind == CK_MAP) {
        if ((int32_t)prop < 0 || prop >= n_keys) dec_err(errk, row, 3, ST_DATA_CORRUPTION);
        if (vt == 8) kind = OK_MAP_DEL;
        else if (vt == 11) kind = OK_MAP_SET;
        else dec_err(errk, row, 3, ST_DATA_CORRUPTION);
      } else if (ckind == CK_LIST) {
        if (vt == 11) { if (is_list_value) kind = OK_LIST_INS; else dec_err(errk, row, 3, ST_DATA_CORRUPTION); }
        else if (vt == 9) kind = OK_DEL;
        else dec_err(errk, row, 3, ST_DATA_CORRUPTION);
      } else if (ckind == CK_MOVABLE) {
        if (vt == 11) { if (is_list_value) kind = OK_LIST_INS; else dec_err(errk, row, 3, ST_DATA_CORRUPTION); }
        else if (vt == 9) kind = OK_DEL;
        else if (vt == 14 || vt == 15) {
          kind = vt == 14 ? OK_LIST_MOVE : OK_LIST_SET;
          orow.a0 = sx[r * 8 + 4]; orow.a1 = sx[r * 8 + 5]; orow.a2 = (int32_t)sx[r * 8 + 6];
          if ((o[3] & 2) || (int32_t)prop < 0 || len != 1) { dec_err(errk, row, 3, ST_DATA_CORRUPTION); orow.a0 = 0; }
        } else dec_err(errk, row, 3, ST_DATA_CORRUPTION);
      }
      if (take_del) {
        if (!has_del) dec_err(errk, row, 4, ST_DATA_CORRUPTION);
        else { orow.a0 = sx[r * 8 + 4]; orow.a1 = sx[r * 8 + 5]; orow.a2 = (int32_t)sx[r * 8 + 6]; }
      }
      orow.cidx_kind |= (kind << 16) | (((o[3] & 4) && (vt != 12 || kind == OK_STYLE_START)) ? OPF_NESTED : 0u);
      kc_add(kc_map, kc_el, kc_style, kind, len);
      d.op[op0 + row] = orow;
      d.op_val[op0 + row] = (uint64_t)o[0] | ((uint64_t)o[1] << 32);
      d.op_blk[op0 + row] = bi;
    }
    lmw::wave_sync();
    DEC_PH(6);
  }
  uint32_t tail = 0;
  if (ok && r == 7) {
    d.chg[chg0 + change_index].n_op = rows_in_change;
    for (uint32_t i = change_index + 1; i < N; i++) { d.chg[chg0 + i].op0 = op0 + n_ops; d.chg[chg0 + i].n_op = 0; }
    if (v.bad) tail |= 1;
    if (counter != (uint64_t)bd.counter_start + bd.counter_len) tail |= 2;
    if (unsupported) tail |= 4;
  }
  if (ok && r < 4 && ((staged ? fcol.bad : col.r.bad) || !(staged ? col_exhausted(fcol) : rle_exhausted(col)))) tail |= 16;
  {
    uint32_t tot = n_del_read;
    if (ok && has_del && r >= 4 && r < 7) {
      tot += staged ? col_drain(fcol, mode) : rle_drain(col, mode);
      if (colbad || (staged ? fcol.bad : col.r.bad)) tail |= 16;
    }
    uint32_t t4 = lmw::shfl(tot, (int)(b * 8 + 4)), t5 = lmw::shfl(tot, (int)(b * 8 + 5)), t6 = lmw::shfl(tot, (int)(b * 8 + 6));
    if (ok && has_del && (t4 != t5 || t4 != t6)) tail |= 16;
  }
  if (ok && shape_bad) tail |= 8;
  for (int m = 1; m < 8; m <<= 1) {
    uint32_t oe = lmw::shfl_xor(errk, m), ot = lmw::shfl_xor(tail, m);
    errk = oe < errk ? oe : errk;
    tail |= ot;
    kc_map += lmw::shfl_xor(kc_map, m); kc_el += lmw::shfl_xor(kc_el, m); kc_style += lmw::shfl_xor(kc_style, m);
  }
  if (ok && r == 0) {
#ifdef LM_EMU_TRACE
    if (getenv("LM_EMU_DECERR") && (st != ST_OK || errk != 0xffffffffu || tail)) fprintf(stderr, "DECERR blk %u st %d errk %x tail %x\n", bi, st, errk, tail);
#endif
    if (st == ST_OK && (tail & 8)) st = ST_DECODE_ERROR;
    if (st == ST_OK && (tail & 16)) st = ST_DECODE_ERROR;
    if (st == ST_OK && errk != 0xffffffffu) st = (int32_t)(errk & 0xf);
    if (st == ST_OK && (tail & 1)) st = ST_DECODE_ERROR;
    if (st == ST_OK && (tail & 2)) st = ST_DATA_CORRUPTION;
    if (st == ST_OK && (tail & 4)) st = ST_UNSUPPORTED;
    d.blk[bi].status = st;
    d.blk[bi].flags = kc_pack(kc_map, kc_style); d.blk[bi].pad = (st == ST_DECODE_ERROR || st == ST_DATA_CORRUPTION) ? DEC_RECLASS : kc_el;
  }
#ifdef LM_PROF_DEC
  DEC_PH(7);
  if (lane == 0) for (int i = 0; i < 8; i++) atomicAdd(&d.prof[i], (unsigned long long)pacc[i]);
#endif
}

LM_KERNEL LM_WAVES_PER_SIMD(3) LM_ONE_WAVE_GROUPS void k_block_decode_wave(Dev d, uint32_t slot_cap, uint32_t head_lo, uint32_t head_hi) {
  block_decode_wave_body<false>(d, slot_cap, head_lo, head_hi);
}
LM_KERNEL LM_WAVES_PER_SIMD(3) LM_ONE_WAVE_GROUPS void k_block_decode_wave_map(Dev d, uint32_t slot_cap, uint32_t head_lo, uint32_t head_hi) {
  block_decode_wave_body<true>(d, slot_cap, head_lo, head_hi);
}

}
```

loro_amd/csrc/lm_k_map_fused.h:

```cpp
#pragma once

namespace lm {

static constexpr uint32_t MF_WG = 1024;
static constexpr uint32_t MF_WAVES = MF_WG / 64;
static constexpr uint32_t MF_KMAX = 1020;
static constexpr uint32_t MF_RMAX = 1024;
static constexpr uint32_t MF_WAVE_LDS = (MF_KMAX + 4) * 2 + MF_RMAX * 2 * 2 + 3 * 64 * 4 + 128;
static constexpr uint32_t MF_LDS = LWW_LDS_CAP * 24 + (MAX_PEERS + MAX_CONTAINERS / 32 + 8) * 4 + MF_WAVES * MF_WAVE_LDS;

struct DevMf {
  const uint32_t* docs;
  const uint8_t* doc_fused;
  const uint32_t* key0;
  uint32_t stop_after;
};

struct MfCol { uint64_t p, end; int64_t rem; int64_t runv; int32_t acc; uint32_t mode; bool run, uniform; int32_t uval; };

#ifdef LM_PROF_MF
#define MF_PH(i) do { uint64_t n_ = lmw::clock(); mfp[i] += n_ - mft; mft = n_; } while (0)
#define MF_PH_ARGS , uint64_t* mfp, uint64_t& mft
#define MF_PH_PASS , mfp, mft
#else
// ... 369 lines not shown
    if (n >= max_n) { bad = true; break; }
    const uint64_t w0 = start;
    const uint64_t at = w0 + (uint32_t)lane;
    uint32_t len = 0;
    if (at < send) {
      Rd r = rd_make(data + at, send - at);
      if (KEYS) { uint64_t l = rd_uleb(r); rd_skip(r, l); }
      else {
        uint32_t tag = rd_u8(r);
        switch (tag) {
          case 0: case 1: case 2: break;
          case 3: (void)rd_sleb(r); break;
          case 4: rd_skip(r, 8); break;
          case 5: case 6: { uint64_t l = rd_uleb(r); rd_skip(r, l); break; }
          case 9: (void)rd_u8(r); break;
          default: r.bad = true; break;
        }
      }
      if (!r.bad) len = (uint32_t)(r.p - (data + at));
    }
    uint32_t off = 0;
    while (off < 64 && (KEYS ? w0 + off < send : n < want_n)) {
      if (!KEYS) {
        bool d = (dels[n >> 5] >> (n & 31)) & 1u;
        if (d) { if (lane == 0) out[n] = (uint16_t)(w0 + off - sec); n++; continue; }
        if (w0 + off >= send) { bad = true; break; }
      }
      if (n >= max_n) { bad = true; break; }
      const uint32_t l = lmw::bcast(len, (int)off);
      if (l == 0) { bad = true; break; }
      if (lane == 0) out[n] = (uint16_t)(w0 + off - sec);
      n++;
      off += l;
    }
    if (bad) break;
    start = w0 + off;
  }
  if (bad || start > send || (KEYS && start != send)) return NONE;
  if (!KEYS && start != send) return NONE;
  if (KEYS && lane == 0) out[n] = (uint16_t)(send - sec);
  mf_wave_lds_sync();
  return n;
}

LM_KERNEL LM_WAVES_PER_SIMD(4) void k_map_fused(Dev d, DevMf f, uint32_t* retry_count) {
  const uint32_t doc = f.docs[(uint32_t)lmw::bid()];
  const uint32_t tid = (uint32_t)lmw::tid();
  const int lane = lmw::lane();
  const uint32_t wv = (uint32_t)lmw::wave_in_block();
  const DocMeta m = d.doc[doc];
  if (status_fatal(m.status)) return;
  const uint32_t cap = d.ht_cap[doc];
  LM_DYN_SHARED(unsigned long long, s_mem64);
  unsigned long long* s_key = s_mem64;
  unsigned long long* s_pfx = s_key + LWW_LDS_CAP;
  unsigned long long* s_best = s_pfx + LWW_LDS_CAP;
  uint32_t* s_end = (uint32_t*)(s_best + LWW_LDS_CAP);
  uint32_t* s_touch = s_end + MAX_PEERS;
  uint32_t* s_misc = s_touch + MAX_CONTAINERS / 32;
  uint8_t* s_wave = (uint8_t*)(s_misc + 8) + (size_t)wv * MF_WAVE_LDS;
  uint16_t* kpos = (uint16_t*)s_wave;
  uint16_t* a_prop = kpos + (MF_KMAX + 4);
  uint16_t* a_voff = a_prop + MF_RMAX;
  uint32_t* tmp = (uint32_t*)(a_voff + MF_RMAX);
  uint32_t* dels = tmp + 3 * 64;
  if (cap == 0 || cap > LWW_LDS_CAP) {
    if (cap != 0 && tid == 0) { lmw::atomic_or(&d.doc[doc].flags, DF_REDO); LM_SETERR(d.doc[doc].status, ST_DATA_CORRUPTION); }
    return;
  }
  for (uint32_t i = tid; i < cap; i += MF_WG) { s_key[i] = HT_EMPTY; s_pfx[i] = LWW_PFX_UNSET; s_best[i] = 0; }
  for (uint32_t i = tid; i < m.n_peers && i < MAX_PEERS; i += MF_WG) s_end[i] = d.peer_end[m.praw0 + i];
  for (uint32_t i = tid; i < MAX_CONTAINERS / 32 + 8; i += MF_WG) s_touch[i] = 0;
  lmw::block_sync();
  const uint64_t seed = 0xcbf29ce484222325ull;
  const uint8_t* data = d.data;
#ifdef LM_PROF_MF
  uint64_t mfp[16] = {0, 0, 0, 0, 0, 0, 0, 0, 0, 0, 0, 0, 0, 0, 0, 0}, mft = lmw::clock();
#endif
  for (uint32_t bk = wv; bk < m.n_blk; bk += MF_WAVES) {
    const uint32_t bi = m.blk0 + (m.n_blk - 1 - bk);
    const BlockDesc* bdp = d.blk + bi;
    const uint64_t base = bdp->base;
    const uint32_t N = bdp->n_changes, cs = bdp->counter_start, cl = bdp->counter_len;
    const uint32_t n_ops = bdp->flags & 0x7fffffffu;
    const uint32_t* bo = d.boff + (uint64_t)bi * BCN;
    const uint32_t chg0 = bo[BC_CHG], cidr0 = bo[BC_CID];
    const uint32_t n_cids = d.bcnt[(uint64_t)bi * BCN + BC_CID];
    bool bail = lmw::bcast(s_misc[1] != 0 ? 1u : 0u, 0) != 0;
    if (n_ops > MF_RMAX || n_ops != cl || N == 0 || N > n_ops || bdp->sec_len[SEC_DEL] != 0) bail = true;
    MF_PH(0);
    const uint64_t k0 = base + bdp->sec_rel[SEC_KEYS];
    const uint32_t klen_sec = bdp->sec_len[SEC_KEYS];
    uint32_t nk = 0;
    if (!bail) {
      if (klen_sec > 0xfff0u) bail = true;
      bool fastk = !bail;
      for (uint32_t w0 = 0; w0 < klen_sec && fastk; w0 += 256) {
        const uint32_t o = w0 + 4u * (uint32_t)lane;
        const uint32_t x = mf_ld4(data, k0 + o, k0 + klen_sec, 0xffu);
        const uint32_t c5 = ~(x | (x >> 1) | (x >> 2)) & 0x20202020u;
        const uint32_t cand = ((c5 >> 5) & 1u) | ((c5 >> 12) & 2u) | ((c5 >> 19) & 4u) | ((c5 >> 26) & 8u);
        const uint32_t ncl = (uint32_t)__builtin_popcount(c5);
        const uint32_t incl = lmw::scan_incl_add(ncl);
        uint32_t rk = nk + incl - ncl;
        const uint32_t tot = lmw::bcast(incl, 63);
        if (nk + tot > MF_KMAX) { fastk = false; bail = true; break; }
#pragma unroll
        for (int q = 0; q < 4; q++) if ((cand >> q) & 1u) { kpos[rk] = (uint16_t)(o + q); rk++; }
        nk += tot;
      }
      if (fastk) {
        if ((uint32_t)lane == 0) kpos[nk] = (uint16_t)klen_sec;
        mf_wave_lds_sync();
        bool okc = nk == 0 ? klen_sec == 0 : kpos[0] == 0;
        for (uint32_t k = (uint32_t)lane; k < nk; k += 64) {
          const uint32_t a = kpos[k], nx = kpos[k + 1];
          okc &= a + 1u + (uint32_t)data[k0 + a] == nx;
        }
        if (lmw::ballot(!okc)) fastk = false;
        mf_wave_lds_sync();
      }
      if (!fastk && !bail) {
        nk = mf_chain<true>(data, k0, k0 + klen_sec, MF_KMAX, 0, nullptr, kpos, lane);
        if (nk == NONE) { nk = 0; bail = true; }
      }
    }
    MF_PH(1);
    if (f.stop_after == 1) continue;
    MfCol c_ci, c_vt, c_len;
    c_ci.p = c_ci.end = c_vt.p = c_vt.end = c_len.p = c_len.end = 0; c_ci.rem = c_vt.rem = c_len.rem = 0; c_ci.uniform = c_vt.uniform = c_len.uniform = false;
    c_ci.runv = c_vt.runv = c_len.runv = 0; c_ci.acc = c_vt.acc = c_len.acc = 0; c_ci.mode = 2; c_vt.mode = 0; c_len.mode = 1; c_ci.run = c_vt.run = c_len.run = false; c_ci.uval = c_vt.uval = c_len.uval = 0;
    const uint64_t vsec = base + bdp->sec_rel[SEC_VALUES], vend = vsec + bdp->sec_len[SEC_VALUES];
    if (!bail) {
      const uint64_t os = base + bdp->sec_rel[SEC_OPS], oe = os + bdp->sec_len[SEC_OPS];
      MfWin w = mf_win(data, os, oe, lane);
      MfRd o{os, oe, false};
      uint64_t outer = mw_uleb(data, w, o), ncols = mw_uleb(data, w, o);
      if (outer != 1 || ncols != 4) bail = true;
      uint64_t pp = 0, pe = 0;
      MfWin wprop = w;
      auto open_col = [&](MfCol& c, uint32_t mode) {
        if (bail) return;
        if (o.p + 12 > w.w0 + 256) w = mf_win(data, o.p, oe, lane);
        uint64_t n = mw_uleb(data, w, o);
        if (o.bad || n > o.end - o.p) { bail = true; return; }
        c.p = o.p; c.end = o.p + n;
        c.rem = 0; c.runv = 0; c.acc = 0; c.run = false; c.uniform = false; c.uval = 0; c.mode = mode;
        if (c.p + 24 > w.w0 + 256 && n) w = mf_win(data, c.p, oe, lane);
        if (!mf_col_open(data, w, c, n_ops)) bail = true;
        o.p += n;
      };
      open_col(c_ci, 2u);
      if (!bail) {
        if (o.p + 12 > w.w0 + 256) w = mf_win(data, o.p, oe, lane);
        uint64_t n = mw_uleb(data, w, o);
        if (o.bad || n > o.end - o.p) bail = true;
        else { pp = o.p; pe = o.p + n; wprop = w; o.p += n; }
      }
      open_col(c_vt, 0u);
      open_col(c_len, 1u);
      if (o.bad || o.p != o.end || bdp->sec_len[SEC_VALUES] > 0xfff0u) bail = true;
      (void)wprop;
      MF_PH(2);
      if (!bail && !mf_prop_all(data, pp, pe, n_ops, nk, a_prop, (uint8_t*)a_voff, MF_RMAX * 2 - 8, (uint8_t*)tmp, 3 * 64 * 4, lane MF_PH_PASS)) bail = true;
    }
    if (f.stop_after == 2) continue;
    if (!bail) {
// ... 175 lines not shown
```

loro_amd/csrc/lm_pipeline.h:

```cpp
#pragma once
#include <algorithm>
#include <map>
#include <mutex>
#include <thread>
#include <atomic>
#include <cstdint>
#include <cstring>
#include <cstdlib>
#include <functional>
#include <string>
#include <vector>
#include <stdexcept>
#include "lm_k_scan.h"
#include "lm_k_emit.h"
#include "lm_k_lww_doc.h"
#include "lm_k_map_fused.h"
#include "lm_k_fuse.h"
#include "lm_k_lca.h"
#include "lm_k_richtext.h"
#include "lm_k_cursor.h"
#include "lm_k_delta.h"
#include "lm_k_delta_map.h"
#include "lm_k_delta_movable.h"
#include "lm_k_delta_richtext.h"
// ... 66 lines not shown
  std::vector<uint8_t> h_fused;
  uint32_t n_fused = 0;
  DBuf b_chg, b_dep_peer, b_dep_ctr, b_dep_ci, b_op, b_op_val, b_op_blk, b_key_off, b_key_len, b_cid_raw, b_cid_map, b_peer_raw, b_peer_map;
  DBuf b_doc, b_peer_uniq, b_peer_end, b_peer_ext, b_peer_base, b_peer_end_all, b_elem_base, b_peer_chg0, b_peer_chg1, b_cont;
  DBuf b_chg_mask, b_chg_sorted, b_chg_lamport, b_chg_skip, b_chg_flag, b_node_first, b_node_last, b_node_order, b_vvh;
  DBuf b_blk_sorted, b_chg_node, b_node_done, b_node_lam;
  DBuf b_cp, b_loc, b_kept, b_tb, b_fuse, b_dcnt, b_posdel;
  DBuf b_it, b_dir_out, b_lf_chunk;
  DBuf b_cont_root0, b_cont_nroot;
  DBuf b_ht_key, b_ht_pfx, b_ht_best, b_ht0, b_ht_cap, b_ht_list, b_ht_cnt;
  DBuf b_out, b_out_off, b_vv_out, b_vv_off, b_hash, b_order, b_prof, b_slab, b_vslab, b_slab_off, b_vslab_off, b_slab2, b_slab2_off;
  uint64_t payload_bytes = 0;
  std::vector<uint64_t> h_prof, h_hash, h_ht0;
  std::vector<uint32_t> h_ht_cap, h_ht_full;
  std::vector<DocMeta> h_doc;
  std::vector<DocResult> results;
  std::vector<uint8_t> h_out, h_vv;
  std::vector<uint64_t> h_out_off, h_vv_off;
  uint64_t out_bytes = 0, vv_bytes = 0;
  bool ran = false, fetched = false;
  Dev last_d;
  DBuf b_rt_out, b_rt_off, b_rt_len;
  std::vector<uint8_t> h_rt;
  std::vector<uint64_t> h_rt_off;
  std::vector<uint32_t> h_rt_len;
  std::vector<int32_t> h_rt_status;
  bool rt_ran = false;
  int rt_launches = 0;
  DBuf b_cur_doc, b_cur_dg, b_cur_grp, b_cur_q, b_cur_names, b_cur_res;
  bool no_map_fused = false;
  bool keep_tombstones = false;
  double cur_ms = 0;
  DBuf b_dl_q, b_dl_bnd, b_dl_bits, b_dl_res, b_dl_out, b_dl_off, b_dl_pack, b_dl_poff;
  uint64_t dl_d2h_bytes = 0;
  std::vector<KernelTime> dl_times;
  int dl_launches = 0;
  std::vector<KernelTime> times;
  bool profiling = false;
  std::string last_error;
  uint64_t device_bytes = 0;
  uint32_t last_retries = 0, last_reemits = 0, last_posdel = 0;
  lmbe::StreamCtx* sc = nullptr;
  long long* sum_rows = nullptr;
  long long sum_id0 = 0, sum_stride = 1;

  struct BlobRef { uint64_t off; uint32_t len; };
  bool resident = false;
  uint32_t shared_mode = 0;
  std::vector<std::vector<BlobRef>> r_blobs;
  std::vector<uint32_t> r_step;
  std::vector<std::vector<uint8_t>> r_front;
  uint64_t arena_top = 0;
  bool tables_valid = false;
  std::vector<uint32_t> tk_leaf0, tk_leaf_cap, tk_pcap, tk_ccap, tk_elem_cap, h_old_blobs;
  std::vector<uint64_t> tk_off, tk_elem0;
  uint64_t elem_top = 0;
  DBuf b_elem_cap, b_old_blobs, b_prev_doc, b_prev_uniq, b_prev_end, b_lca_out, b_lca_scratch, b_lca_off;
  bool have_prev = false;
  std::vector<uint32_t> h_lca;
  std::vector<std::vector<std::pair<uint64_t, uint32_t>>> keep_ver;
  std::vector<uint8_t> keep_on;
  bool prev_copied = false;
  DBuf b_keep_idx, b_keep_uniq, b_keep_end;
  std::vector<uint8_t> tk_reset;
  void upload_res() {
    std::vector<ResDoc> hres(n_docs);
    for (uint32_t i = 0; i < n_docs; i++) hres[i] = ResDoc{tk_off[i], tk_pcap[i], tk_ccap[i], tk_reset[i], tk_elem_cap[i]};
    b_res.ensure((size_t)n_docs * sizeof(ResDoc));
    lmbe::h2d(b_res.p, hres.data(), (size_t)n_docs * sizeof(ResDoc));
  }
  uint64_t tk_top = 0;
  uint32_t leaf_top = 0;
  int dir_parity = 0;
  DBuf b_tk, b_res, b_dir_out2, b_dir_b, b_dir_b2, b_doc_saved;
  uint32_t last_fresh = 0;
  struct Saved {
    Dev d; DevDag g;
    uint32_t NB = 0, NC = 0, NO = 0, NCID = 0, NP = 0, dir_cap = 0, dir_opt = 0, pmax = 0;
    uint64_t ht = 0;
    bool any_ml = false, any_common = false;
    std::vector<DocMeta> h_doc;
  } sv;

  struct Knobs { bool span = true, decode_wave = true, no_opt_dir = false, loc_memset = true, loc_poison = false; int plain = 2; uint32_t dec_slot = 1264, dec_slot_big = 4096, dec_big_mode = 1, dir_opt_max = 0; size_t lds_pad = 0; long long slab_cap = -1; uint32_t ht_opt = 2048, cut_min_rows = 2048, vs_row_cost = 300; bool lww_lds = true, fuse_rows = true, version_sweep = true, span_auto = true, linear = true, posdel = true, reclass = true, redo = true, map_fused = true, snapshot_state = true, snapshot_state_force = false, stage_direct = true; uint32_t mf_min_rows = 2048, mf_chg_ratio = 4, pd_state_pieces = 2; } kn;
  void read_knobs() {
    Knobs k;
    if (const char* e = getenv("LM_SPAN")) k.span = atoi(e) != 0;
    if (const char* e = getenv("LM_PLAIN")) k.plain = atoi(e);
    if (const char* e = getenv("LM_DECODE")) k.decode_wave = atoi(e) != 0;
    if (const char* e = getenv("LM_RECLASS")) k.reclass = atoi(e) != 0;
    if (const char* e = getenv("LM_DEC_SLOT")) k.dec_slot = ((uint32_t)atoi(e) + 15u) & ~15u;
    if (const char* e = getenv("LM_DEC_SLOT_BIG")) k.dec_slot_big = ((uint32_t)atoi(e) + 15u) & ~15u;
    if (const char* e = getenv("LM_DEC_BIG_MODE")) k.dec_big_mode = (uint32_t)atoi(e);
    if (const char* e = getenv("LM_LDS_PAD")) k.lds_pad = (size_t)atoi(e);
    k.no_opt_dir = getenv("LM_NO_OPT_DIR") != nullptr;
    if (const char* e = getenv("LM_LOC_MEMSET")) k.loc_memset = atoi(e) != 0;
    if (const char* e = getenv("LM_LOC_POISON")) k.loc_poison = atoi(e) != 0;
    if (const char* e = getenv("LM_DIR_OPT_MAX")) k.dir_opt_max = (uint32_t)atoi(e);
    if (const char* e = getenv("LM_SLAB_CAP")) k.slab_cap = atoll(e);
    if (const char* e = getenv("LM_HT_OPT")) k.ht_opt = (uint32_t)atoi(e);
    if (const char* e = getenv("LM_CUT_MIN_ROWS")) k.cut_min_rows = (uint32_t)atoll(e);
    if (const char* e = getenv("LM_SPAN_AUTO")) k.span_auto = atoi(e) != 0;
    if (const char* e = getenv("LM_VS_ROW_COST")) k.vs_row_cost = (uint32_t)atoi(e);
    if (const char* e = getenv("LM_VERSION_SWEEP")) k.version_sweep = atoi(e) != 0;
    if (const char* e = getenv("LM_FUSE_ROWS")) k.fuse_rows = atoi(e) != 0;
    if (const char* e = getenv("LM_POSDEL")) k.posdel = atoi(e) != 0;
    if (const char* e = getenv("LM_LINEAR")) k.linear = atoi(e) != 0;
    if (const char* e = getenv("LM_LWW_LDS")) k.lww_lds = atoi(e) != 0;
    if (const char* e = getenv("LM_REDO")) k.redo = atoi(e) != 0;
    if (const char* e = getenv("LM_MAP_FUSED")) k.map_fused = atoi(e) != 0;
    if (const char* e = getenv("LM_MF_MIN_ROWS")) k.mf_min_rows = (uint32_t)atoi(e);
    if (const char* e = getenv("LM_STAGE_DIRECT")) k.stage_direct = atoi(e) != 0;
    if (const char* e = getenv("LM_PD_STATE_PIECES")) k.pd_state_pieces = (uint32_t)atoi(e);
    if (const char* e = getenv("LM_SNAPSHOT_STATE")) { k.snapshot_state = atoi(e) != 0; k.snapshot_state_force = atoi(e) == 2; }
    if (const char* e = getenv("LM_MF_CHG_RATIO")) k.mf_chg_ratio = (uint32_t)atoi(e);
    if (force_span) { k.span = true; k.span_auto = false; k.posdel = true; k.redo = false; k.map_fused = false; }
    kn = k;
  }
  bool force_span = false;
  bool allow_state = true;
  std::vector<uint8_t> h_vvo;
  std::vector<uint64_t> h_vvo_off;
  std::vector<std::vector<std::vector<uint8_t>>> st_hist;
  uint32_t n_state_docs = 0;
  bool stage_history_only = false;
  DBuf b_vvo, b_vvo_off, b_pd_off, b_pd_row;
  std::vector<uint8_t> redo_hist;
  bool st_valid = false;
  std::vector<uint32_t> st_doc_blob, st_blob_len;
  std::vector<uint64_t> st_blob_off, st_froot_off;
  std::vector<uint8_t> st_froot;
  std::vector<uint32_t> redo_docs;
  struct RedoItem { uint32_t doc; const uint8_t* front; size_t front_len; };
  bool redo_by_history(uint32_t doc) const { return doc < redo_hist.size() && redo_hist[doc] != 0; }
  void stage_from(const std::vector<Engine*>& parents, const std::vector<RedoItem>& items) {
    for (Engine* pe : parents) if (!pe->st_valid) throw std::runtime_error("redo: the staged blobs are gone");
    std::vector<std::vector<const uint8_t*>> bp(items.size());
    std::vector<std::vector<size_t>> bl(items.size());
    std::vector<DocIn> in(items.size());
    for (size_t k = 0; k < items.size(); k++) {
      const uint32_t i = items[k].doc;
      Engine& parent = *parents[k];
      if (parent.redo_by_history(i)) for (auto& hb : parent.st_hist[i]) { bp[k].push_back(hb.data()); bl[k].push_back(hb.size()); }
      else
      for (uint32_t b = parent.st_doc_blob[i]; b < parent.st_doc_blob[i + 1]; b++) { bp[k].push_back(parent.st_base + parent.st_blob_off[b]); bl[k].push_back(parent.st_blob_len[b]); }
      in[k] = DocIn{bp[k].data(), bl[k].data(), bp[k].size(), items[k].front, items[k].front_len};
    }
    stage_history_only = true;
    try { stage(in.data(), in.size()); } catch (...) { stage_history_only = false; throw; }
    stage_history_only = false;
    h_froot.clear();
    h_froot_off.assign(items.size() + 1, 0);
    for (size_t k = 0; k < items.size(); k++) {
      h_froot_off[k] = h_froot.size();
      const uint32_t i = items[k].doc;
      Engine& parent = *parents[k];
      if ((size_t)i + 1 < parent.st_froot_off.size()) h_froot.insert(h_froot.end(), parent.st_froot.begin() + parent.st_froot_off[i], parent.st_froot.begin() + parent.st_froot_off[i + 1]);
    }
    h_froot_off[items.size()] = h_froot.size();
    h_vvo.clear(); h_vvo_off.assign(items.size() + 1, 0); n_state_docs = 0;
    for (size_t k = 0; k < items.size(); k++) {
      h_vvo_off[k] = h_vvo.size();
      Engine& parent = *parents[k];
      const uint32_t i = items[k].doc;
      if (parent.n_state_docs && (size_t)i + 1 < parent.h_vvo_off.size() && parent.h_vvo_off[i + 1] > parent.h_vvo_off[i] && !parent.redo_by_history(i)) {
        h_vvo.insert(h_vvo.end(), parent.h_vvo.begin() + parent.h_vvo_off[i], parent.h_vvo.begin() + parent.h_vvo_off[i + 1]);
        n_state_docs++;
      }
    }
    h_vvo_off[items.size()] = h_vvo.size();
    lmbe::bind(sc);
    if (n_state_docs) {
      b_vvo.ensure(h_vvo.size() + 16); lmbe::h2d(b_vvo.p, h_vvo.data(), h_vvo.size());
      b_vvo_off.ensure((items.size() + 1) * 8); lmbe::h2d(b_vvo_off.p, h_vvo_off.data(), (items.size() + 1) * 8);
    }
    b_froot.ensure(h_froot.size() + 16); if (!h_froot.empty()) lmbe::h2d(b_froot.p, h_froot.data(), h_froot.size());
    b_froot_off.ensure((items.size() + 1) * 8); lmbe::h2d(b_froot_off.p, h_froot_off.data(), (items.size() + 1) * 8);
    lmbe::sync();
  }

  explicit Engine(int device) { sc = lmbe::stream_create(device); }
  Engine(const Engine&) = delete;
  Engine& operator=(const Engine&) = delete;
  uint8_t* h_stage = nullptr;
  const uint8_t* st_base = nullptr;
  bool staged_direct = false;
  size_t h_stage_cap = 0;
  ~Engine() { release_all(); if (h_stage) lmbe::hfree(h_stage); lmbe::stream_destroy(sc); }
  void release_all() {
// ... 408 lines not shown
        src.push_back(Src{p, l, top});
        add_refs[i].push_back(BlobRef{top, (uint32_t)l});
        top += (l + 15) & ~(uint64_t)15;
      }
      if (!add_refs[i].empty()) {
        uint64_t first = r_blobs[i].empty() ? add_refs[i].front().off : r_blobs[i].front().off;
        if (add_refs[i].back().off + add_refs[i].back().len - first >= 0xfffffff0ull)
          throw std::runtime_error("lm_import: a resident document's blobs span more than 4 GiB of the arena (stage the batch again)");
      }
    }
    uint64_t add = top - arena_top;
    if (add) {
      st_valid = false;
      if (add + 64 > h_stage_cap) {
        uint8_t* nh = (uint8_t*)lmbe::halloc(add + add / 4 + 4096);
        if (!nh) throw std::runtime_error("host staging allocation failed");
        if (h_stage) lmbe::hfree(h_stage);
        h_stage = nh; h_stage_cap = add + add / 4 + 4096;
      }
      for (const Src& x : src) {
        uint64_t o = x.off - arena_top, pad = ((x.l + 15) & ~(uint64_t)15) - x.l;
        memcpy(h_stage + o, x.p, x.l);
        if (pad) memset(h_stage + o + x.l, 0, pad);
      }
      memset(h_stage + add, 0, 64);
      b_data.ensure_keep(top + 64, arena_top);
      lmbe::h2d_async((uint8_t*)b_data.p + arena_top, h_stage, add + 64);
    }
    for (size_t i = 0; i < nd; i++) {
      r_blobs[i].insert(r_blobs[i].end(), add_refs[i].begin(), add_refs[i].end());
      r_step[i] += (uint32_t)add_refs[i].size();
      std::vector<uint8_t> f;
      if (docs[i].front) f.assign(docs[i].front, docs[i].front + docs[i].front_len);
      r_front[i].swap(f);
    }
    if (add) { arena_top = top; tables_valid = false; }
    rebuild_blob_tables();
    lmbe::sync();
    ran = fetched = false;
  }

  void scan(const uint32_t* in, uint32_t* out, uint32_t n, uint32_t ncomp) {
    uint32_t tiles = (n + 1 + SCAN_TILE - 1) / SCAN_TILE;
    b_tile.ensure((size_t)tiles * ncomp * 4 + 64);
    b_tot.ensure(64 * 4);
    LM_LAUNCH(k_scan_tile, tiles, SCAN_TILE, in, out, b_tile.as<uint32_t>(), n, ncomp);
    LM_LAUNCH(k_scan_sums, 1, 64, b_tile.as<uint32_t>(), tiles, ncomp, b_tot.as<uint32_t>());
    LM_LAUNCH(k_scan_add, tiles, SCAN_TILE, out, b_tile.as<uint32_t>(), b_tot.as<uint32_t>(), n, ncomp);
  }

  int selftest() {
    lmbe::bind(sc);
    DBuf b;
    b.ensure(64 * 4);
    LM_LAUNCH(k_selftest, 64, 64, b.as<uint32_t>(), 200u);
    uint32_t h[64];
    lmbe::d2h(h, b.p, sizeof h);
    b.release();
    int bad = 0;
    for (int i = 0; i < 64; i++) bad += (int)h[i];
    return bad;
  }

  static uint32_t cdiv(uint64_t a, uint32_t b) { return (uint32_t)((a + b - 1) / b); }

  void run() {
    lmbe::bind(sc);
    times.clear();
    lmbe::reset_times();
    Dev d;
    memset(&d, 0, sizeof d);
    d.data = b_data.as<uint8_t>();
    d.front = b_front.as<uint8_t>(); d.front_off = b_front_off.as<uint64_t>();
    d.froot = b_froot.as<uint8_t>(); d.froot_off = b_froot_off.as<uint64_t>();
    d.blob_off = b_blob_off.as<uint64_t>();
    d.blob_len = b_blob_len.as<uint32_t>();
    d.doc_blob = b_doc_blob.as<uint32_t>();
    d.n_blobs = n_blobs;
    d.n_docs = n_docs;
    if (n_state_docs && !resident) { d.vvo = b_vvo.as<uint8_t>(); d.vvo_off = b_vvo_off.as<uint64_t>(); }
    results.assign(n_docs, DocResult{0, 0, 0, 0, 0, 0});
    if (n_docs == 0) { ran = true; return; }
    const bool reuse = resident && tables_valid;
    prev_copied = resident && have_prev;
    if (resident && have_prev) {
      b_prev_doc.ensure((size_t)n_docs * sizeof(DocMeta)); lmbe::d2d(b_prev_doc.p, b_doc_saved.p, (size_t)n_docs * sizeof(DocMeta));
      b_prev_uniq.ensure((size_t)(sv.NP + 1) * 8); lmbe::d2d(b_prev_uniq.p, b_peer_uniq.p, (size_t)(sv.NP + 1) * 8);
      b_prev_end.ensure((size_t)(sv.NP + 1) * 4); lmbe::d2d(b_prev_end.p, b_peer_end_all.p, (size_t)(sv.NP + 1) * 4);
    }
    uint32_t NB = 0, NC = 0, NO = 0, NCID = 0, NP = 0, sv_NK = 0;
    DevDag g;
    memset(&g, 0, sizeof g);
    bool span = kn.span;
    if (resident && !span) throw std::runtime_error("resident documents need the span-granular integrate kernel (LM_SPAN=0 is set)");
    uint64_t ht = 0;
    uint32_t dir_cap = 64, dir_opt = 64, pmax = 2;
    uint32_t DIR_CAP_MAX = span ? 18000u : 36000u;
    int plain_mode = !span ? 0 : kn.plain;
    bool plain_on = plain_mode == 1 || plain_mode == 2;
    bool any_plain = false, any_fused = false, want_dcnt = false;
    if (reuse) {
      d = sv.d; g = sv.g;
      d.front = b_front.as<uint8_t>(); d.front_off = b_front_off.as<uint64_t>();
      d.blob_off = b_blob_off.as<uint64_t>(); d.blob_len = b_blob_len.as<uint32_t>(); d.doc_blob = b_doc_blob.as<uint32_t>(); d.blob_doc = b_blob_doc.as<uint32_t>();
      NB = sv.NB; NC = sv.NC; NO = sv.NO; NCID = sv.NCID; NP = sv.NP; ht = sv.ht; dir_cap = sv.dir_cap; dir_opt = sv.dir_opt; pmax = sv.pmax;
      h_doc = sv.h_doc;
      lmbe::d2d(b_doc.p, b_doc_saved.p, (size_t)n_docs * sizeof(DocMeta));
      if (ht) { lmbe::dmemset(b_ht_key.p, 0xff, ht * 8); lmbe::dmemset(b_ht_best.p, 0, ht * 8); }
      lmbe::dmemset(b_ht_cnt.p, 0, (size_t)n_docs * 4 + 4);
      if (shared_mode == 2 && NCID) LM_LAUNCH(k_cont_untouch, cdiv(NCID, 256), 256, d, NCID);
    } else {
    b_blob_status.ensure((size_t)n_blobs * 4 + 4);
    b_blob_nblk.ensure((size_t)(n_blobs + 1) * 4);
    b_blob_blk0.ensure((size_t)(n_blobs + 1) * 4);
    d.blob_status = b_blob_status.as<int32_t>();
    d.blob_nblk = b_blob_nblk.as<uint32_t>();
    d.blob_blk0 = b_blob_blk0.as<uint32_t>();
    d.blob_doc = b_blob_doc.as<uint32_t>();
    lmbe::tic(profiling);
    {
      std::vector<uint32_t> big;
      for (uint32_t i = 0; i < n_blobs; i++) if (h_blob_len[i] >= BIG_BLOB) big.push_back(i);
      std::stable_sort(big.begin(), big.end(), [&](uint32_t a, uint32_t b) { return h_blob_len[a] > h_blob_len[b]; });
      b_blob_hash.ensure((size_t)n_blobs * 4 + 4);
      d.blob_hash = b_blob_hash.as<uint32_t>();
      if (!big.empty()) {
        b_big.ensure(big.size() * 4);
        lmbe::h2d(b_big.p, big.data(), big.size() * 4);
        LM_LAUNCH(k_hash_big_blobs, cdiv(big.size(), HASH_G), 64, d, (const uint32_t*)b_big.as<uint32_t>(), (uint32_t)big.size());
      }
    }
    if (n_blobs) LM_LAUNCH(k_frame_count, cdiv(n_blobs, 64), 64, d);
    lmbe::toc("k_frame_count", times, profiling);
    scan(d.blob_nblk, d.blob_blk0, n_blobs, 1);
    lmbe::d2h(&NB, d.blob_blk0 + n_blobs, 4);
    d.n_blocks = NB;
    b_blk.ensure((size_t)(NB + 1) * sizeof(BlockDesc));
    b_bcnt.ensure((size_t)(NB + 1) * BCN * 4);
    b_boff.ensure((size_t)(NB + 1) * BCN * 4);
    d.blk = b_blk.as<BlockDesc>();
    d.bcnt = b_bcnt.as<uint32_t>();
    d.boff = b_boff.as<uint32_t>();
    lmbe::tic(profiling);
    if (n_blobs) LM_LAUNCH(k_frame_fill, cdiv(n_blobs, 64), 64, d);
    if (NB) LM_LAUNCH(k_block_desc, cdiv(NB, 64), 64, d);
    b_tot.ensure(64 * 4);
    d.dec_stat = b_tot.as<uint32_t>() + 48; d.dec_slot = kn.dec_slot; d.cut_min_rows = kn.cut_min_rows; d.vs_row_cost = kn.vs_row_cost;
    lmbe::dmemset(d.dec_stat, 0, 12);
    n_fused = 0;
    h_fused.assign(n_docs, 0);
    const bool mf_on = kn.map_fused && !no_map_fused && kn.redo && kn.lww_lds && kn.ht_opt && kn.ht_opt <= LWW_LDS_CAP && !resident && st_valid && NB;
    if (mf_on) {
      b_blk_kind.ensure((size_t)(NB + 1) * 4); b_doc_fused.ensure((size_t)n_docs + 16);
      d.blk_kind = b_blk_kind.as<uint32_t>();
      LM_LAUNCH(k_block_kind, cdiv(NB, 64), 64, d);
      LM_LAUNCH(k_doc_kind, cdiv(n_docs, 64), 64, d, b_doc_fused.as<uint8_t>(), kn.mf_min_rows, kn.mf_chg_ratio);
      d.doc_fused = b_doc_fused.as<uint8_t>();
    }
    if (NB) LM_LAUNCH(k_block_count, cdiv(NB, 64), 64, d);
    lmbe::toc("k_frame_fill+k_block_count", times, profiling);
    scan(d.bcnt, d.boff, NB, BCN);
    uint32_t tot[BCN];
    lmbe::d2h(tot, d.boff + (uint64_t)NB * BCN, sizeof tot);
    if (mf_on) { lmbe::d2h(h_fused.data(), b_doc_fused.p, n_docs); for (uint32_t i = 0; i < n_docs; i++) n_fused += h_fused[i]; }
    if (!n_fused) d.doc_fused = nullptr;
    const uint32_t NF = n_fused ? tot[BC_MAPOP] : 0u;
    const uint32_t KF = n_fused * LWW_LDS_CAP;
    uint32_t dec_stat[3] = {0, 0, 0};
    lmbe::d2h(dec_stat, d.dec_stat, 12);
    uint32_t ND = tot[BC_DEP], NK = tot[BC_KEY];
    NC = tot[BC_CHG]; NO = tot[BC_OP]; NCID = tot[BC_CID]; NP = tot[BC_PEER];
    b_chg.ensure((size_t)(NC + 1) * sizeof(ChangeRow));
    b_dep_peer.ensure((size_t)(ND + 1) * 4); b_dep_ctr.ensure((size_t)(ND + 1) * 4); b_dep_ci.ensure((size_t)(ND + 1) * 4);
    if ((uint64_t)NO + NF > 0xfffffff0ull || (uint64_t)NK + KF > 0xfffffff0ull) throw std::runtime_error("batch too large for 32-bit row indices");
    b_op.ensure((size_t)(NO + NF + 1) * sizeof(OpRow)); b_op_val.ensure((size_t)(NO + NF + 1) * 8); b_op_blk.ensure((size_t)(NO + NF + 1) * 4);
    b_key_off.ensure((size_t)(NK + KF + 1) * 8); b_key_len.ensure((size_t)(NK + KF + 1) * 4);
    d.n_op_rows = NO; sv_NK = NK;
    b_cid_raw.ensure((size_t)(NCID + 1) * 16); b_cid_map.ensure((size_t)(NCID + 1) * 4);
    b_peer_raw.ensure((size_t)(NP + 1) * 8); b_peer_map.ensure((size_t)(NP + 1) * 4);
    b_doc.ensure((size_t)n_docs * sizeof(DocMeta));
    b_peer_uniq.ensure((size_t)(NP + 1) * 8);
    for (DBuf* b : {&b_peer_end, &b_peer_ext, &b_peer_base, &b_peer_end_all, &b_elem_base, &b_peer_chg0, &b_peer_chg1}) b->ensure((size_t)(NP + 1) * 4);
    b_cont.ensure((size_t)(NCID + 1) * sizeof(ContRow));
    for (DBuf* b : {&b_chg_sorted, &b_chg_lamport, &b_chg_skip, &b_chg_flag, &b_node_first, &b_node_last, &b_node_order, &b_chg_node,
                    &b_node_done, &b_node_lam})
      b->ensure((size_t)(NC + 1) * 4);
    b_blk_sorted.ensure((size_t)(NB + 1) * 4);
    b_chg_mask.ensure((size_t)(NC + 1) * 8);
    b_cont_root0.ensure((size_t)(NCID + 1) * 4); b_cont_nroot.ensure((size_t)(NCID + 1) * 4);
    d.chg = b_chg.as<ChangeRow>(); d.dep_peer = b_dep_peer.as<uint32_t>(); d.dep_ctr = b_dep_ctr.as<uint32_t>(); d.dep_ci = b_dep_ci.as<uint32_t>();
    d.op = b_op.as<OpRow>(); d.op_val = b_op_val.as<uint64_t>(); d.op_blk = b_op_blk.as<uint32_t>();
    d.key_off = b_key_off.as<uint64_t>(); d.key_len = b_key_len.as<uint32_t>();
    d.cid_raw = b_cid_raw.as<uint32_t>(); d.cid_map = b_cid_map.as<uint32_t>();
    d.peer_raw = b_peer_raw.as<uint64_t>(); d.peer_map = b_peer_map.as<uint32_t>();
    d.doc = b_doc.as<DocMeta>(); d.peer_uniq = b_peer_uniq.as<uint64_t>();
    d.peer_end = b_peer_end.as<uint32_t>(); d.peer_ext = b_peer_ext.as<uint32_t>(); d.peer_base = b_peer_base.as<uint32_t>(); d.peer_end_all = b_peer_end_all.as<uint32_t>(); d.elem_base = b_elem_base.as<uint32_t>();
    d.peer_chg0 = b_peer_chg0.as<uint32_t>(); d.peer_chg1 = b_peer_chg1.as<uint32_t>();
    d.cont = b_cont.as<ContRow>();
    d.chg_sorted = b_chg_sorted.as<uint32_t>(); d.chg_lamport = b_chg_lamport.as<uint32_t>();
    d.chg_skip = b_chg_skip.as<uint32_t>(); d.chg_flag = b_chg_flag.as<uint32_t>(); d.chg_mask = b_chg_mask.as<uint32_t>();
    d.node_first = b_node_first.as<uint32_t>(); d.node_last = b_node_last.as<uint32_t>(); d.node_order = b_node_order.as<uint32_t>();
    d.cont_root0 = b_cont_root0.as<uint32_t>(); d.cont_nroot = b_cont_nroot.as<uint32_t>();
    g.blk_sorted = b_blk_sorted.as<uint32_t>(); g.chg_node = b_chg_node.as<uint32_t>();
    g.node_done = b_node_done.as<uint32_t>(); g.node_lam = b_node_lam.as<uint32_t>();
    lmbe::dmemset(b_chg_flag.p, 0, (size_t)(NC + 1) * 4);
    lmbe::dmemset(b_chg_mask.p, 0, (size_t)(NC + 1) * 8);
    lmbe::dmemset(b_chg_skip.p, 0, (size_t)(NC + 1) * 4);
    lmbe::dmemset(b_chg_lamport.p, 0, (size_t)(NC + 1) * 4);
    lmbe::tic(profiling);
    if (NB) {
#if defined(LM_PROF_DEC) || defined(LM_PROF_DAG)
      b_prof.ensure((size_t)n_docs * 16 * 8); d.prof = b_prof.as<unsigned long long>(); lmbe::dmemset(b_prof.p, 0, (size_t)n_docs * 16 * 8);
#endif
      if (n_fused) LM_LAUNCH(k_block_head, cdiv(NB, 64), 64, d);
      if (n_fused == n_docs) {}
      else if (!kn.decode_wave) LM_LAUNCH(k_block_decode, cdiv(NB, 64), 64, d);
      else {
        uint32_t slot_cap = kn.dec_slot;
        uint32_t slot_big = 0;
        if (dec_stat[0] && kn.dec_slot_big && (kn.dec_big_mode == 2 || (uint64_t)dec_stat[0] * 10 >= (uint64_t)NB * 9)) {
          if (kn.dec_big_mode == 2) { slot_big = (dec_stat[1] + 15u) & ~15u; if (slot_big > kn.dec_slot_big) slot_big = kn.dec_slot_big; }
          else { slot_big = (dec_stat[2] + 15u) & ~15u; if (slot_big < 64) slot_big = 64; if (slot_big >= slot_cap) slot_big = 0; }
        }
        if (!(slot_big && dec_stat[0] == NB))
          LM_LAUNCH_DYN(k_block_decode_wave, cdiv(NB, DEC_G), 64, (size_t)DEC_G * slot_cap + DEC_LDS_FIXED + DEC_G * DEC_KINDS, d, slot_cap, 0u, slot_big ? slot_cap : 0xffffffffu);
        if (slot_big) LM_LAUNCH_DYN(k_block_decode_wave_map, cdiv(NB, DEC_G), 64, (size_t)DEC_G * slot_big + DEC_LDS_FIXED + DEC_G * DEC_KINDS, d, slot_big, slot_cap, 0xffffffffu);
      }
      if (kn.reclass) LM_LAUNCH(k_block_reclassify, cdiv(NB, 64), 64, d);
    }
    lmbe::toc("k_block_decode", times, profiling);
    lmbe::tic(profiling);
    LM_LAUNCH(k_doc_ranges, cdiv(n_docs, 64), 64, d);
    LM_LAUNCH(k_doc_tables, n_docs, 64, d);
    uint32_t nmax = NO > NC ? NO : NC;
    if (nmax) LM_LAUNCH(k_remap, cdiv(nmax, 256), 256, d, NO, NC);
    lmbe::toc("k_doc_tables+k_remap", times, profiling);
    lmbe::tic(profiling);
    LM_LAUNCH(k_dag_a, n_docs, 64, d, g);
    lmbe::toc("k_dag_a", times, profiling);
    h_doc.resize(n_docs);
    lmbe::d2h(h_doc.data(), d.doc, (size_t)n_docs * sizeof(DocMeta));
    if (span && !resident && kn.span_auto) {
      uint64_t rows_all = 0, rows_common = 0, atoms_common = 0;
      uint32_t rows_max = 0, elems_max = 0;
      for (uint32_t i = 0; i < n_docs; i++) {
        const DocMeta& m = h_doc[i];
        if (m.status != ST_OK) continue;
        const bool checked_out = h_front_off.size() > i + 1 && h_front_off[i + 1] > h_front_off[i];
        rows_all += m.n_op;
        if (!(m.flags & DF_PLAIN) || checked_out || !plain_on) { rows_common += m.n_op; atoms_common += m.atoms; }
        rows_max = m.n_op > rows_max ? m.n_op : rows_max;
        elems_max = m.n_elems > elems_max ? m.n_elems : elems_max;
      }
      if (rows_all && rows_max < 4096 && elems_max < 65536 && rows_common * 2 >= rows_all && atoms_common < 3 * rows_common) {
        span = false; DIR_CAP_MAX = 36000u; plain_mode = 0; plain_on = false;
      }
    }
    d.span = span ? 1u : 0u;
    d.res_vis = resident ? 1u : 0u;
    uint64_t elem = 0, leaves = 0, vvh = 0;
    h_ht0.assign(n_docs, 0); h_ht_cap.assign(n_docs, 0); h_ht_full.assign(n_docs, 0);
    for (uint32_t i = 0; i < n_docs; i++) {
      DocMeta& m = h_doc[i];
      bool ok = m.status == ST_OK;
      if (!plain_on || !ok || (!resident && h_front_off.size() > i + 1 && h_front_off[i + 1] > h_front_off[i])) m.flags &= ~(DF_PLAIN | DF_FUSED);
      if (resident || plain_mode != 2 || !kn.fuse_rows) m.flags &= ~DF_FUSED;
      any_plain |= (m.flags & DF_PLAIN) != 0;
      any_fused |= (m.flags & DF_FUSED) != 0;
      want_dcnt |= ok && !(m.flags & (DF_PLAIN | DF_MOVABLE));
      m.elem0_lo = (uint32_t)elem; m.elem0_hi = (uint32_t)(elem >> 32);
      if (resident) {
        uint64_t need = (uint64_t)m.atoms + m.atoms / 2 + 96ull * (m.n_peers + 1) + 8;
        if (ok && need > tk_elem_cap[i]) {
          uint64_t cap = ((need + need / 2 + 80ull * 8) + 31) & ~31ull;
          if (cap > 0xfffffff0ull) throw std::runtime_error("resident element slice beyond 32-bit indices");
          tk_elem0[i] = elem_top; tk_elem_cap[i] = (uint32_t)cap; elem_top += cap;
        }
        m.elem0_lo = (uint32_t)tk_elem0[i]; m.elem0_hi = (uint32_t)(tk_elem0[i] >> 32);
      }
      uint32_t lc = ok ? m.n_elems / 32 + 2 * m.n_cont + 2 : 0;
      if (ok && span) {
        uint64_t items = 3ull * m.n_op + 2ull * m.n_nodes * m.n_peers + 64;
        uint64_t lcs = items / 32 + 2 * m.n_cont + 2;
        if (lcs < lc) lc = (uint32_t)lcs;
      }
      if (leaves + lc > 0xfffffff0ull) throw std::runtime_error("batch too large for 32-bit pool indices");
      m.leaf0 = (uint32_t)leaves; m.leaf_cap = lc;
      if (resident) {
        if (ok && lc > tk_leaf_cap[i]) {
          uint32_t cap = lc + lc / 2 + 8;
          if ((uint64_t)leaf_top + cap > 0xfffffff0ull) throw std::runtime_error("resident leaf pool beyond 32-bit indices");
          tk_leaf0[i] = leaf_top; tk_leaf_cap[i] = cap; leaf_top += cap; tk_reset[i] = 1;
        }
        m.leaf0 = tk_leaf0[i]; m.leaf_cap = ok ? tk_leaf_cap[i] : 0;
        if (ok && (tk_pcap[i] == 0 || m.n_peers > tk_pcap[i] || m.n_cont > tk_ccap[i])) tk_grow(i, m.n_peers, m.n_cont);
      }
      m.vvh0_lo = (uint32_t)vvh; m.vvh0_hi = (uint32_t)(vvh >> 32);
      if (ok) { elem += ((uint64_t)m.atoms + 31) & ~31ull; leaves += lc; vvh += (uint64_t)m.n_nodes * m.n_peers; }
      if (ok && m.leaf_cap > dir_cap) dir_cap = m.leaf_cap;
      uint32_t lo = ok ? m.n_elems / 40 + 2 * m.n_cont + 16 : 0;
      if (ok && span) { uint32_t los = (uint32_t)((3ull * m.n_op / 2) / 40) + 2 * m.n_cont + 16; if (los < lo) lo = los; }
      if (lo > lc) lo = lc;
      if (lo > dir_opt) dir_opt = lo;
      if (ok && m.n_peers > pmax) pmax = m.n_peers;
      uint32_t cap = 0;
      if (ok && m.n_mapop) { cap = 64; while (cap < 2 * m.n_mapop) cap <<= 1; }
      h_ht_full[i] = cap;
      if (kn.ht_opt && !resident && !(m.flags & DF_MOVABLE) && cap > kn.ht_opt) cap = kn.ht_opt;
      h_ht0[i] = ht; h_ht_cap[i] = cap;
      ht += cap;
    }
    if (resident) tk_flush();
    if (dir_cap > DIR_CAP_MAX) dir_cap = DIR_CAP_MAX;
    {
      std::vector<uint32_t> order(n_docs);
      for (uint32_t i = 0; i < n_docs; i++) order[i] = i;
      std::stable_sort(order.begin(), order.end(), [&](uint32_t a, uint32_t b) { return h_doc[a].n_op > h_doc[b].n_op; });
      b_order.ensure((size_t)n_docs * 4 + 4);
// ... 57 lines not shown
      const uint64_t n4 = ((uint64_t)elem / 32 + 3) / 4;
      const uint32_t blocks = (uint32_t)std::min<uint64_t>((n4 + 255) / 256, 4096);
      LM_LAUNCH(k_fill_words, blocks, 256, b_kept.as<uint32_t>(), n4, 0u, blocks * 256u);
    }
    if (kn.loc_poison && span && (resident ? elem_top : elem)) {
      const uint64_t n = resident ? elem_top : elem, n4 = (n + 3) / 4;
      const uint32_t blocks = (uint32_t)std::min<uint64_t>(((resident ? n : n4) + 255) / 256, 4096);
      if (resident) LM_LAUNCH(k_fill_unkept, blocks, 256, b_loc.as<uint32_t>(), b_kept.as<uint32_t>(), n, 0u, blocks * 256u);
      else LM_LAUNCH(k_fill_words, blocks, 256, b_loc.as<uint32_t>(), n4, 0u, blocks * 256u);
    }
    if (ht) { lmbe::dmemset(b_ht_key.p, 0xff, ht * 8); lmbe::dmemset(b_ht_best.p, 0, ht * 8); }
      if (resident) {
        sv.d = d; sv.g = g; sv.NB = NB; sv.NC = NC; sv.NO = NO; sv.NCID = NCID; sv.NP = NP; sv.ht = ht;
        sv.dir_cap = dir_cap; sv.dir_opt = dir_opt; sv.pmax = pmax; sv.h_doc = h_doc;
      }
    }
    lmbe::dmemset(b_cont_root0.p, 0, (size_t)(NCID + 1) * 4);
    lmbe::dmemset(b_cont_nroot.p, 0, (size_t)(NCID + 1) * 4);
    DevRes rs;
    memset(&rs, 0, sizeof rs);
    if (resident) {
      upload_res();
      rs.doc = b_res.as<ResDoc>(); rs.tk = b_tk.as<uint32_t>();
      if (!reuse) {
        h_old_blobs.resize(n_docs);
        for (uint32_t i = 0; i < n_docs; i++) h_old_blobs[i] = (uint32_t)r_blobs[i].size() - r_step[i];
        b_old_blobs.ensure((size_t)n_docs * 4 + 4);
        lmbe::h2d(b_old_blobs.p, h_old_blobs.data(), (size_t)n_docs * 4);
        d.res_old_blobs = b_old_blobs.as<uint32_t>();
        sv.d.res_old_blobs = d.res_old_blobs;
      }
      if (!reuse) { b_elem_cap.ensure((size_t)(NP + 1) * 4); d.elem_cap = b_elem_cap.as<uint32_t>(); sv.d.elem_cap = d.elem_cap; }
      LM_LAUNCH(k_res_layout, n_docs, 64, d, rs);
    }
    lmbe::tic(profiling);
    d.fuse = nullptr;
    if (!resident && any_fused && NO) {
      b_fuse.ensure(((size_t)NO + 1) * 8);
      d.fuse = b_fuse.as<uint32_t>();
      LM_LAUNCH(k_fuse_rows, cdiv(NO, 256), 256, d, NO);
    }
    if (!resident) LM_LAUNCH(k_dag_b, n_docs, 64, d, g, 0u);
    else {
      if (!reuse) {
        LM_LAUNCH(k_dag_b, n_docs, 64, d, g, 1u);
        b_doc_saved.ensure((size_t)n_docs * sizeof(DocMeta));
        lmbe::d2d(b_doc_saved.p, b_doc.p, (size_t)n_docs * sizeof(DocMeta));
      }
      LM_LAUNCH(k_dag_b, n_docs, 64, d, g, 2u);
    }
    lmbe::toc("k_dag_b", times, profiling);
    if (resident) {
      std::vector<uint64_t> loff(n_docs + 1, 0);
      for (uint32_t i = 0; i < n_docs; i++) { uint64_t N = h_doc[i].status == ST_OK ? h_doc[i].n_nodes : 0; loff[i + 1] = loff[i] + 3 * (8 * N + 64) + 3 * (4 * N + 64) + N + 16; }
      b_lca_off.ensure((size_t)(n_docs + 1) * 8); lmbe::h2d(b_lca_off.p, loff.data(), (size_t)(n_docs + 1) * 8);
      b_lca_scratch.ensure((loff[n_docs] + 16) * 4);
      b_lca_out.ensure((size_t)n_docs * LCA_OUT * 4 + 16);
      DevLca lc;
      lc.out = b_lca_out.as<uint32_t>(); lc.scratch = b_lca_scratch.as<uint32_t>(); lc.scratch_off = b_lca_off.as<uint64_t>();
      lc.prev_doc = have_prev ? b_prev_doc.as<DocMeta>() : nullptr; lc.prev_uniq = b_prev_uniq.as<uint64_t>(); lc.prev_end = b_prev_end.as<uint32_t>();
      lc.keep_idx = nullptr; lc.keep_uniq = nullptr; lc.keep_end = nullptr;
      bool any_keep = false;
      for (uint32_t i = 0; i < n_docs && !any_keep; i++) any_keep = i < keep_on.size() && keep_on[i];
      if (any_keep) {
        std::vector<uint32_t> kidx((size_t)n_docs * 2, NONE), kend;
        std::vector<uint64_t> kuniq;
        for (uint32_t i = 0; i < n_docs; i++) {
          if (!keep_on[i]) continue;
          kidx[2 * i] = (uint32_t)kuniq.size(); kidx[2 * i + 1] = (uint32_t)keep_ver[i].size();
          for (const auto& pe : keep_ver[i]) { kuniq.push_back(pe.first); kend.push_back(pe.second); }
        }
        b_keep_idx.ensure(kidx.size() * 4); lmbe::h2d(b_keep_idx.p, kidx.data(), kidx.size() * 4);
        b_keep_uniq.ensure(kuniq.size() * 8 + 8); if (!kuniq.empty()) lmbe::h2d(b_keep_uniq.p, kuniq.data(), kuniq.size() * 8);
        b_keep_end.ensure(kend.size() * 4 + 4); if (!kend.empty()) lmbe::h2d(b_keep_end.p, kend.data(), kend.size() * 4);
        lc.keep_idx = b_keep_idx.as<uint32_t>(); lc.keep_uniq = b_keep_uniq.as<uint64_t>(); lc.keep_end = b_keep_end.as<uint32_t>();
      }
      lmbe::tic(profiling);
      LM_LAUNCH(k_import_lca, n_docs, 64, d, g, lc);
      lmbe::toc("k_import_lca", times, profiling);
    }
    lmbe::tic(profiling);
    bool any_elems = resident;
    for (uint32_t i = 0; i < n_docs && !any_elems; i++) any_elems = h_doc[i].status == ST_OK && h_doc[i].n_elems != 0;
    if (NB && !reuse && any_elems) LM_LAUNCH(k_elem_fill, NB, 64, d);
    lmbe::toc("k_elem_fill", times, profiling);
    lmbe::tic(profiling);
    b_tot.ensure(64 * 4);
    uint32_t* retry_cnt = b_tot.as<uint32_t>() + 32;
    lmbe::dmemset(retry_cnt, 0, 16);
    if (n_fused && ht && !reuse) {
      std::vector<uint32_t> mfd, mfk(n_docs, 0);
      uint32_t rank = 0;
      for (uint32_t i = 0; i < n_docs; i++) if (h_fused[i]) { mfk[i] = sv_NK + rank * LWW_LDS_CAP; rank++; if (h_doc[i].status == ST_OK && h_doc[i].n_mapop) mfd.push_back(i); }
      std::stable_sort(mfd.begin(), mfd.end(), [&](uint32_t a, uint32_t b) { return h_doc[a].n_op > h_doc[b].n_op; });
      b_mf_docs.ensure(mfd.size() * 4 + 4); b_mf_key0.ensure((size_t)n_docs * 4 + 4);
      if (!mfd.empty()) lmbe::h2d(b_mf_docs.p, mfd.data(), mfd.size() * 4);
      lmbe::h2d(b_mf_key0.p, mfk.data(), (size_t)n_docs * 4);
      DevMf mf; mf.docs = b_mf_docs.as<uint32_t>(); mf.doc_fused = d.doc_fused; mf.key0 = b_mf_key0.as<uint32_t>(); mf.stop_after = 0;
      if (const char* e = getenv("LM_MF_STOP")) mf.stop_after = (uint32_t)atoi(e);
      if (!mfd.empty()) LM_LAUNCH_DYN(k_map_fused, (uint32_t)mfd.size(), MF_WG, (size_t)MF_LDS, d, mf, retry_cnt);
    }
    if (NO && ht) {
      bool any_lds = false, any_hbm = false;
      for (uint32_t i = 0; i < n_docs; i++) if (h_doc[i].status == ST_OK && h_doc[i].n_mapop && !h_fused[i]) {
        if (kn.lww_lds && !resident && h_ht_cap[i] <= LWW_LDS_CAP && !(h_doc[i].flags & DF_MOVABLE)) any_lds = true; else any_hbm = true;
      }
      if (any_lds) LM_LAUNCH_DYN(k_map_lww_doc, n_docs, LWW_WG, (size_t)LWW_LDS_CAP * 24 + (MAX_PEERS + MAX_CONTAINERS / 32 + 8) * 4, d, retry_cnt);
      if (any_hbm) LM_LAUNCH(k_map_lww, cdiv(NO, 256), 256, d, NO, retry_cnt, 0u, any_lds ? 1u : 0u);
    }
    lmbe::toc("k_map_lww", times, profiling);
    lmbe::tic(profiling);
    dir_cap = (dir_cap + 3) & ~3u;
    dir_opt = (dir_opt + 3) & ~3u;
    if (dir_opt > DIR_CAP_MAX) dir_opt = DIR_CAP_MAX;
    size_t lds_pad = kn.lds_pad;
    if (kn.no_opt_dir) dir_opt = dir_cap;
    if (kn.dir_opt_max) { uint32_t mx = kn.dir_opt_max; if (mx >= 4 && mx < dir_opt) dir_opt = mx & ~3u; }
    const size_t dir_words = span ? 2 : 1;
    bool any_ml = false, any_common = false;
    if (resident) any_plain = false;
    for (uint32_t i = 0; i < n_docs; i++) if (h_doc[i].status == ST_OK) {
      uint32_t fl = h_doc[i].flags;
      if (resident && (fl & DF_PLAIN) && h_front_off[i + 1] > h_front_off[i]) fl &= ~DF_PLAIN;
      any_ml |= (fl & DF_MOVABLE) != 0; any_common |= (fl & (DF_MOVABLE | DF_PLAIN)) == 0;
      if (resident) any_plain |= (fl & (DF_MOVABLE | DF_PLAIN)) == DF_PLAIN;
    }
    if (resident) {
      DBuf& wa = dir_parity ? b_dir_out2 : b_dir_out; DBuf& ra = dir_parity ? b_dir_out : b_dir_out2;
      DBuf& wb = dir_parity ? b_dir_b2 : b_dir_b;     DBuf& rb = dir_parity ? b_dir_b : b_dir_b2;
      d.dir_out = wa.as<uint32_t>(); rs.dir_a_prev = ra.as<uint32_t>(); rs.dir_b = wb.as<uint32_t>(); rs.dir_b_prev = rb.as<uint32_t>();
      const size_t lds = (size_t)(2 * dir_opt + (dir_opt >> SD_BSH) + 2 + PD_LDS + 6 * pmax) * 4 + lds_pad;
      if (any_plain)
        LM_LAUNCH_DYN(k_integrate_span_res_plain, n_docs, 64, lds, d, g, dir_opt, pmax, (const OpRow*)d.op, (const ChangeRow*)d.chg, (const uint32_t*)d.chg_sorted,
                      (const uint32_t*)d.chg_skip, (const uint32_t*)d.vvh, 0u, retry_cnt, rs);
      if (any_common || !(any_ml || any_plain))
        LM_LAUNCH_DYN(k_integrate_span_res, n_docs, 64, lds, d, g, dir_opt, pmax, (const OpRow*)d.op, (const ChangeRow*)d.chg, (const uint32_t*)d.chg_sorted,
                      (const uint32_t*)d.chg_skip, (const uint32_t*)d.vvh, 0u, retry_cnt, rs);
      if (any_ml)
        LM_LAUNCH_DYN(k_integrate_span_res_ml, n_docs, 64, lds, d, g, dir_opt, pmax, (const OpRow*)d.op, (const ChangeRow*)d.chg, (const uint32_t*)d.chg_sorted,
                      (const uint32_t*)d.chg_skip, (const uint32_t*)d.vvh, 0u, retry_cnt, rs);
    } else if (span) {
      if (any_plain && plain_mode == 2) {
        LM_LAUNCH_DYN(k_integrate_span_plain_sweep, n_docs, 64, (size_t)(dir_words * dir_opt + (span ? (dir_opt >> SD_BSH) + 2 + PD_LDS : 0) + 4 * pmax + 1) * 4 + lds_pad, d, g, dir_opt, pmax, (const OpRow*)d.op,
                      (const ChangeRow*)d.chg, (const uint32_t*)d.chg_sorted, (const uint32_t*)d.chg_skip, (const uint32_t*)d.vvh, 0u, retry_cnt);
        if (d.fuse)
          LM_LAUNCH_DYN(k_integrate_span_plain_fuse, n_docs, 64, (size_t)(dir_words * dir_opt + (span ? (dir_opt >> SD_BSH) + 2 + PD_LDS : 0) + 4 * pmax + 1) * 4 + lds_pad, d, g, dir_opt, pmax, (const OpRow*)d.op,
                        (const ChangeRow*)d.chg, (const uint32_t*)d.chg_sorted, (const uint32_t*)d.chg_skip, (const uint32_t*)d.vvh, 0u, retry_cnt);
      }
      else if (any_plain)
        LM_LAUNCH_DYN(k_integrate_span_plain, n_docs, 64, (size_t)(dir_words * dir_opt + (span ? (dir_opt >> SD_BSH) + 2 + PD_LDS : 0) + 4 * pmax + 1) * 4 + lds_pad, d, g, dir_opt, pmax, (const OpRow*)d.op,
                      (const ChangeRow*)d.chg, (const uint32_t*)d.chg_sorted, (const uint32_t*)d.chg_skip, (const uint32_t*)d.vvh, 0u, retry_cnt);
      if (any_common || !(any_ml || any_plain))
        LM_LAUNCH_DYN(k_integrate_span, n_docs, 64, (size_t)(dir_words * dir_opt + (span ? (dir_opt >> SD_BSH) + 2 + PD_LDS : 0) + 4 * pmax + 1) * 4 + lds_pad, d, g, dir_opt, pmax, (const OpRow*)d.op,
                      (const ChangeRow*)d.chg, (const uint32_t*)d.chg_sorted, (const uint32_t*)d.chg_skip, (const uint32_t*)d.vvh, 0u, retry_cnt);
      if (any_ml)
        LM_LAUNCH_DYN(k_integrate_span_ml, n_docs, 64, (size_t)(dir_words * dir_opt + (span ? (dir_opt >> SD_BSH) + 2 + PD_LDS : 0) + 4 * pmax + 1) * 4 + lds_pad, d, g, dir_opt, pmax, (const OpRow*)d.op,
                      (const ChangeRow*)d.chg, (const uint32_t*)d.chg_sorted, (const uint32_t*)d.chg_skip, (const uint32_t*)d.vvh, 0u, retry_cnt);
    } else {
      LM_LAUNCH_DYN(k_integrate, n_docs, 64, (size_t)(dir_opt + 3 * pmax) * 4 + lds_pad, d, g, dir_opt, pmax, (const OpRow*)d.op,
                    (const ChangeRow*)d.chg, (const uint32_t*)d.chg_sorted, (const uint32_t*)d.chg_skip, (const uint32_t*)d.vvh, 0u, retry_cnt);
    }
    uint32_t n_retry = 0, n_lww = 0, n_posdel = 0;
    {
      uint32_t four[4] = {0, 0, 0, 0};
      lmbe::d2h(four, retry_cnt, 16);
      n_retry = four[0]; n_lww = four[2]; n_posdel = four[3];
      if (resident) last_fresh = four[1];
// ... 746 lines not shown
```

loro_amd/csrc/lm_types.h:

```cpp
#pragma once
#include <cstdint>

namespace lm {

static constexpr uint32_t NONE = 0xFFFFFFFFu;

enum : int32_t {
  ST_OK = 0,
  ST_DECODE_ERROR = 1,
  ST_CHECKSUM_MISMATCH = 2,
  ST_DATA_CORRUPTION = 3,
  ST_UNSUPPORTED = 4,
  ST_INTERNAL = 5,
  ST_FRONTIERS_NOT_FOUND = 6,
  ST_RETRY = 100,
  ST_MF_BAIL = 102,
};

enum : uint32_t { SEC_HEADER = 0, SEC_META, SEC_CIDS, SEC_KEYS, SEC_POS, SEC_OPS, SEC_DEL, SEC_VALUES, SEC_N };

enum : uint32_t { CK_MAP = 0, CK_LIST = 1, CK_TEXT = 2, CK_TREE = 3, CK_MOVABLE = 4, CK_COUNTER = 5 };

enum : uint32_t {
  OK_OTHER = 0, OK_TEXT_INS = 1, OK_DEL = 2, OK_STYLE_START = 3, OK_STYLE_END = 4, OK_LIST_INS = 5, OK_MAP_SET = 6, OK_MAP_DEL = 7,
  OK_LIST_MOVE = 8, OK_LIST_SET = 9
};

static constexpr uint32_t MAX_PEERS = 256;
static constexpr uint32_t MAX_COUNTER = 1u << 24;
static constexpr uint32_t MAX_CONTAINERS = 256;
static constexpr uint32_t MAX_ROOTS = 64;

struct BlockDesc {
  uint64_t base;
  uint32_t blob, doc;
  uint32_t sec_rel[SEC_N], sec_len[SEC_N];
  uint32_t counter_start, counter_len, lamport_start, lamport_len, n_changes;
  int32_t status;
  uint32_t flags;
  uint32_t pad;
};
struct BlockCounts { uint32_t n_chg, n_dep, n_op, n_key, n_cid, n_peer; };
static constexpr int BC_N = 6;

struct OpRow {
  uint32_t cidx_kind;
  int32_t prop;
  uint32_t len;
  uint32_t ctr;
  uint32_t a0, a1;
  int32_t a2;
  uint32_t chg;
};

enum : uint32_t { OPF_CONT = 1u << 24, OPF_HEAD = 1u << 25, OPF_NESTED = 1u << 26 };

struct ChangeRow {
  uint32_t peer;
  uint32_t ctr, len;
  uint32_t dep0, n_dep;
  uint32_t op0, n_op;
  uint32_t blk;
};

struct ContRow {
  uint64_t name_off;
  uint32_t name_len;
  uint32_t kind_root;
  uint32_t peer, counter;
  uint32_t touched;
  uint32_t pad;
};

struct DocMeta {
  int32_t status;
  uint32_t blk0, n_blk;
  uint32_t chg0, n_chg;
  uint32_t op0, n_op;
  uint32_t dep0, n_dep;
  uint32_t key0, n_key;
  uint32_t cid0, n_cid;
  uint32_t praw0, n_praw;
  uint32_t n_peers;
  uint32_t n_cont;
  uint32_t atoms;
  uint32_t n_valid_chg;
  uint32_t n_nodes;
  uint32_t pending_lo, pending_hi;
  uint32_t elem0_lo, elem0_hi;
  uint32_t leaf0, leaf_cap;
  uint32_t n_elems, n_mapop;
  uint32_t node0;
  uint32_t vvh0_lo, vvh0_hi;
  uint32_t out_len;
  uint32_t vv_len;
  uint32_t pad0;
  uint32_t flags;
  int32_t front_err;
};

enum : uint32_t {
  DF_SOFT_UNSUPPORTED = 1u,
  DF_REEMIT = 2u,
  DF_MOVABLE = 4u,
  DF_FRONT_ERR = 16u,
  DF_LAYOUT_SAME = 32u,
  DF_FILL_KEPT = 64u,
  DF_LWW_RETRY = 128u,
  DF_FUSED = 256u,
  DF_CUT = 512u,
  DF_REDO = 1024u,
  DF_PLAIN = 8u,
};

}
```

Before: 501,100 docs/s.

## Defer op-row remapping into elem_fill and precompute text string offsets in decode

Moves the per-op cid/peer/key remap and change-mask update out of k_remap into k_elem_fill, which already streams every op row, so the rows are read and written once instead of twice. Nested-value validation moves to a separate per-block kernel, and kept or no-element cases get their own fallback kernels. Decode now records each text insert's string offset and byte length in a1/a2, so elem_fill no longer re-reads the ULEB length from the value section. It also prefetches the next row group and chg_flag one iteration ahead. The gating across several kernels and flag bits adds complexity and correctness risk, and the fused elem_fill uses more registers.

```diff
diff --git a/loro_amd/csrc/lm_k_dag.h b/loro_amd/csrc/lm_k_dag.h
--- a/loro_amd/csrc/lm_k_dag.h
+++ b/loro_amd/csrc/lm_k_dag.h
@@ -140,37 +140,47 @@
   (void)s_n;
 }
 
-LM_KERNEL void k_remap(Dev d, uint32_t n_ops, uint32_t n_chg) {
+LM_DEV uint32_t remap_row(const Dev& d, const uint32_t* bo, OpRow& r) {
+  const uint32_t local = r.cidx_kind & 0xffff, kind = (r.cidx_kind >> 16) & 0xff;
+  const uint32_t ci = d.cid_map[bo[BC_CID] + local];
+  r.cidx_kind = ci | (r.cidx_kind & (0xff0000u | OPF_CONT | OPF_HEAD));
+  if (kind == OK_DEL || kind == OK_LIST_MOVE || kind == OK_LIST_SET) r.a0 = d.peer_map[bo[BC_PEER] + r.a0];
+  else if (kind == OK_MAP_SET || kind == OK_MAP_DEL) r.a0 = bo[BC_KEY] + (uint32_t)r.prop;
+  return ci;
+}
+LM_DEV void remap_mask(const Dev& d, uint32_t m_chg, uint32_t ci) {
+  const uint32_t m_bit = ci & 63;
+  uint32_t p_chg = lmw::shfl_up(m_chg, 1), p_bit = lmw::shfl_up(m_bit, 1);
+  bool lead = m_chg != NONE && (lmw::lane() == 0 || p_chg != m_chg || p_bit != m_bit);
+  if (lead) lmw::atomic_or(&d.chg_mask[2 * (uint64_t)m_chg + (m_bit >> 5)], 1u << (m_bit & 31));
+}
+LM_DEV void remap_nested(const Dev& d, const BlockDesc& bd, uint32_t blk, uint32_t t, uint32_t kind) {
+  const uint8_t* vend = d.data + bd.base + bd.sec_rel[SEC_VALUES] + bd.sec_len[SEC_VALUES];
+  Rd v{d.data + d.op_val[t], vend, false};
+  uint32_t n_keys = d.bcnt[(uint64_t)blk * BCN + BC_KEY];
+  if (kind == OK_STYLE_START) { (void)rd_u8(v); (void)rd_uleb(v); (void)rd_uleb(v); }
+  uint32_t vf = 0;
+  skip_loro_value_keys(v, vf, n_keys);
+  if ((vf & VF_CORRUPT) && !v.bad) LM_SETERR(d.doc[bd.doc].status, ST_DATA_CORRUPTION);
+}
+LM_DEV void remap_one(const Dev& d, uint32_t t, uint32_t& m_chg, uint32_t& ci) {
+  uint32_t blk = d.op_blk[t];
+  const BlockDesc& bd = d.blk[blk];
+  if (bd.status == ST_OK && d.doc[bd.doc].status == ST_OK) {
+    const uint32_t* bo = d.boff + (uint64_t)blk * BCN;
+    OpRow r = d.op[t];
+    if (r.cidx_kind & OPF_NESTED) remap_nested(d, bd, blk, t, (r.cidx_kind >> 16) & 0xff);
+    ci = remap_row(d, bo, r);
+    d.op[t] = r;
+    m_chg = r.chg;
+  }
+}
+LM_KERNEL void k_remap(Dev d, uint32_t n_ops, uint32_t n_chg, uint32_t defer) {
   uint32_t t = (uint32_t)(lmw::bid() * lmw::bdim() + lmw::tid());
-  uint32_t m_chg = NONE, m_bit = 0;
-  if (t < n_ops) {
-    uint32_t blk = d.op_blk[t];
-    const BlockDesc& bd = d.blk[blk];
-    if (bd.status == ST_OK && d.doc[bd.doc].status == ST_OK) {
-      const uint32_t* bo = d.boff + (uint64_t)blk * BCN;
-      OpRow r = d.op[t];
-      uint32_t local = r.cidx_kind & 0xffff, kind = (r.cidx_kind >> 16) & 0xff;
-      uint32_t ci = d.cid_map[bo[BC_CID] + local];
-      if (r.cidx_kind & OPF_NESTED) {
-        const uint8_t* vend = d.data + bd.base + bd.sec_rel[SEC_VALUES] + bd.sec_len[SEC_VALUES];
-        Rd v{d.data + d.op_val[t], vend, false};
-        uint32_t n_keys = d.bcnt[(uint64_t)blk * BCN + BC_KEY];
-        if (kind == OK_STYLE_START) { (void)rd_u8(v); (void)rd_uleb(v); (void)rd_uleb(v); }
-        uint32_t vf = 0;
-        skip_loro_value_keys(v, vf, n_keys);
-        if ((vf & VF_CORRUPT) && !v.bad) LM_SETERR(d.doc[bd.doc].status, ST_DATA_CORRUPTION);
-      }
-      r.cidx_kind = ci | (kind << 16);
-      if (kind == OK_DEL || kind == OK_LIST_MOVE || kind == OK_LIST_SET) r.a0 = d.peer_map[bo[BC_PEER] + r.a0];
-      else if (kind == OK_MAP_SET || kind == OK_MAP_DEL) r.a0 = bo[BC_KEY] + (uint32_t)r.prop;
-      d.op[t] = r;
-      m_chg = r.chg; m_bit = ci & 63;
-    }
-  }
-  {
-    uint32_t p_chg = lmw::shfl_up(m_chg, 1), p_bit = lmw::shfl_up(m_bit, 1);
-    bool lead = m_chg != NONE && (lmw::lane() == 0 || p_chg != m_chg || p_bit != m_bit);
-    if (lead) lmw::atomic_or(&d.chg_mask[2 * (uint64_t)m_chg + (m_bit >> 5)], 1u << (m_bit & 31));
+  if (!(defer && d.dec_stat[3])) {
+    uint32_t m_chg = NONE, ci = 0;
+    if (t < n_ops) remap_one(d, t, m_chg, ci);
+    remap_mask(d, m_chg, ci);
   }
   if (t < n_chg) {
     ChangeRow c = d.chg[t];
@@ -181,6 +191,35 @@
       d.chg[t] = c;
       for (uint32_t k = c.dep0; k < c.dep0 + c.n_dep; k++) d.dep_peer[k] = d.peer_map[bo[BC_PEER] + d.dep_peer[k]];
     }
+  }
+}
+LM_KERNEL void k_remap_nested(Dev d, uint32_t n_blk) {
+  uint32_t bi = (uint32_t)((lmw::bid() * lmw::bdim() + lmw::tid()) >> 6);
+  if (bi >= n_blk || !d.dec_stat[3]) return;
+  const BlockDesc& bd = d.blk[bi];
+  if (!(bd.flags & BF_NESTED) || bd.status != ST_OK || d.doc[bd.doc].status != ST_OK) return;
+  uint32_t op0 = d.boff[(uint64_t)bi * BCN + BC_OP], n_op = d.bcnt[(uint64_t)bi * BCN + BC_OP];
+  for (uint32_t i = (uint32_t)lmw::lane(); i < n_op; i += 64) {
+    uint32_t ck = d.op[op0 + i].cidx_kind;
+    if (ck & OPF_NESTED) remap_nested(d, bd, bi, op0 + i, (ck >> 16) & 0xff);
+  }
+}
+LM_KERNEL void k_remap_rows(Dev d, uint32_t n_ops, uint32_t stride) {
+  if (!d.dec_stat[3]) return;
+  for (uint64_t t0 = (uint64_t)(lmw::bid() * lmw::bdim()); t0 < n_ops; t0 += stride) {
+    const uint64_t t64 = t0 + (uint32_t)lmw::tid();
+    uint32_t t = (uint32_t)t64, m_chg = NONE, ci = 0;
+    if (t64 < n_ops) {
+      uint32_t blk = d.op_blk[t];
+      const BlockDesc& bd = d.blk[blk];
+      if (bd.status == ST_OK && d.doc[bd.doc].status == ST_OK) {
+        OpRow r = d.op[t];
+        ci = remap_row(d, d.boff + (uint64_t)blk * BCN, r);
+        d.op[t] = r;
+        m_chg = r.chg;
+      }
+    }
+    remap_mask(d, m_chg, ci);
   }
 }
 
@@ -407,7 +446,7 @@
   for (uint32_t i = (uint32_t)lane; i < m.n_blk; i += 64) {
     const BlockDesc& kb = d.blk[m.blk0 + i];
     if (kb.status != ST_OK) continue;
-    n_map += kb.flags & 0x7fffffffu; n_el += kb.pad; n_style += kb.flags >> 31;
+    n_map += kb.flags & BF_ROWS; n_el += kb.pad; n_style += kb.flags >> 31;
   }
   bool has_ml = false;
   for (uint32_t c = (uint32_t)lane; c < m.n_cont; c += 64) has_ml |= (d.cont[m.cid0 + c].kind_root & 0xff) == CK_MOVABLE;
@@ -653,7 +692,24 @@
   return lmw::any(bad) || n != len;
 }
 
-LM_KERNEL void k_elem_fill(Dev d) {
+LM_KERNEL void k_remap_kept(Dev d) {
+  uint32_t bi = (uint32_t)lmw::bid();
+  int lane = lmw::lane();
+  const BlockDesc& bd = d.blk[bi];
+  if (bd.status != ST_OK || !d.res_old_blobs || !d.dec_stat[3]) return;
+  uint32_t doc = bd.doc;
+  const DocMeta& m = d.doc[doc];
+  if (m.status != ST_OK || !(m.flags & DF_FILL_KEPT) || bd.blob - d.doc_blob[doc] >= d.res_old_blobs[doc]) return;
+  const uint32_t* bo = d.boff + (uint64_t)bi * BCN;
+  const uint32_t r0 = bo[BC_OP], nr = d.bcnt[(uint64_t)bi * BCN + BC_OP];
+  for (uint32_t g0 = 0; g0 < nr; g0 += 64) {
+    uint32_t m_chg = NONE, ci = 0;
+    if (g0 + (uint32_t)lane < nr) { OpRow r = d.op[r0 + g0 + (uint32_t)lane]; ci = remap_row(d, bo, r); d.op[r0 + g0 + (uint32_t)lane] = r; m_chg = r.chg; }
+    remap_mask(d, m_chg, ci);
+  }
+}
+
+LM_KERNEL void k_elem_fill(Dev d, uint32_t remap_rows) {
   uint32_t bi = (uint32_t)lmw::bid();
   int lane = lmw::lane();
   const BlockDesc& bd = d.blk[bi];
@@ -661,6 +717,7 @@
   uint32_t doc = bd.doc;
   const DocMeta& m = d.doc[doc];
   if (status_fatal(m.status)) return;
+  const bool remap = remap_rows && d.dec_stat[3];
   if (d.res_old_blobs && (m.flags & DF_FILL_KEPT) && bd.blob - d.doc_blob[doc] < d.res_old_blobs[doc]) return;
   const bool span = d.span != 0;
   const uint32_t* off = d.boff + (uint64_t)bi * BCN;
@@ -671,59 +728,62 @@
   uint32_t ext = d.peer_ext[m.praw0 + peer];
   uint64_t doc_data0 = d.blob_off[d.doc_blob[doc]];
   const uint8_t* vsec = d.data + bd.base + bd.sec_rel[SEC_VALUES];
-  const uint8_t* lim = vsec + bd.sec_len[SEC_VALUES];
+  const uint32_t vlen = bd.sec_len[SEC_VALUES];
+  const uint8_t* lim = vsec + vlen;
   LM_SHARED(uint32_t, s_inc, 64);
   LM_SHARED(uint32_t, s_nb, 64);
   LM_SHARED(uint32_t, s_src, 64);
   LM_SHARED(uint32_t, s_dst, 64);
+  static constexpr uint32_t DST_WANT = 0x80000000u;
   bool bad = false;
+  OpRow rn;
+  rn.cidx_kind = 0; rn.prop = 0; rn.len = 0; rn.ctr = 0; rn.a0 = rn.a1 = 0; rn.a2 = 0; rn.chg = 0;
+  auto arrived = [&](bool in, uint32_t at) {
+    uint32_t m_chg = NONE, ci = 0;
+    if (in) { ci = remap_row(d, off, rn); d.op[at] = rn; m_chg = rn.chg; }
+    remap_mask(d, m_chg, ci);
+  };
+  if ((uint32_t)lane < n_op) rn = d.op[op0 + (uint32_t)lane];
+  if (remap) arrived((uint32_t)lane < n_op, op0 + (uint32_t)lane);
+  uint32_t fn = (uint32_t)lane < n_op ? d.chg_flag[rn.chg] : 0u;
   for (uint32_t g0 = 0; g0 < n_op; g0 += 64) {
     uint32_t row = op0 + g0 + (uint32_t)lane;
     bool valid = g0 + (uint32_t)lane < n_op;
-    OpRow r;
-    r.cidx_kind = 0; r.prop = 0; r.len = 0; r.ctr = 0; r.a0 = r.a1 = 0; r.a2 = 0; r.chg = 0;
-    if (valid) r = d.op[row];
+    OpRow r = rn;
+    const uint32_t cflag = fn;
     uint32_t kind = (r.cidx_kind >> 16) & 0xff;
-    bool want = valid && (kind == OK_TEXT_INS || kind == OK_LIST_INS || kind == OK_STYLE_START || kind == OK_STYLE_END);
-    const bool cand_text = want && kind == OK_TEXT_INS;
-    if (want && !d.chg_flag[r.chg]) want = false;
-    if (want && r.ctr + r.len > ext) want = false;
-    if (cand_text && !want) {
-      const uint8_t* q = d.data + d.op_val[row];
-      Rd vq = rd_make(q, q < lim ? (uint64_t)(lim - q) : 0ull);
-      uint64_t nb = rd_uleb(vq);
-      if (vq.bad || nb > rd_left(vq)) bad = true;
+    const bool cand = valid && (kind == OK_TEXT_INS || kind == OK_LIST_INS || kind == OK_STYLE_START || kind == OK_STYLE_END);
+    const bool cand_text = cand && kind == OK_TEXT_INS;
+    const uint32_t soff = r.a1, nbytes = (uint32_t)r.a2;
+    const bool text_ok = cand_text && (uint64_t)soff + nbytes <= vlen;
+    if (cand_text && !text_ok) bad = true;
+    const uint8_t* s = vsec + (text_ok ? soff : 0u);
+    const bool flat = text_ok && span && nbytes == r.len;
+    bool want = cand && cflag != 0 && r.ctr + r.len <= ext;
+    if (text_ok && !flat && !want) {
+      uint32_t n = 0;
+      for (uint32_t i = 0; i < nbytes && !bad;) {
+        uint32_t b0 = s[i], extra = b0 < 0x80 ? 0u : (b0 & 0xE0) == 0xC0 ? 1u : (b0 & 0xF0) == 0xE0 ? 2u : (b0 & 0xF8) == 0xF0 ? 3u : 4u;
+        if (extra == 4 || (extra && i + extra >= nbytes)) { bad = true; break; }
+        for (uint32_t k = 1; k <= extra; k++) if ((s[i + k] & 0xC0) != 0x80) bad = true;
+        n++; i += extra + 1;
+      }
+      if (n != r.len) bad = true;
+    }
+    uint64_t e0 = ebase + r.ctr;
+    if (want && (kind == OK_STYLE_START || kind == OK_STYLE_END)) { if (span) d.tb[e0] = (uint8_t)TB_ANCHOR; d.cp[e0] = CP_ANCHOR | (row - m.op0); want = false; }
+    bool is_long = false;
+    if (want && kind == OK_TEXT_INS) {
+      if (!text_ok || flat) {}
+      else if (nbytes > 64) { is_long = true; }
       else {
         uint32_t n = 0;
-        for (uint64_t i = 0; i < nb && !bad;) {
-          uint32_t b0 = vq.p[i], extra = b0 < 0x80 ? 0u : (b0 & 0xE0) == 0xC0 ? 1u : (b0 & 0xF0) == 0xE0 ? 2u : (b0 & 0xF8) == 0xF0 ? 3u : 4u;
-          if (extra == 4 || i + extra >= nb + (extra ? 0 : 1)) { bad = true; break; }
-          for (uint32_t k = 1; k <= extra; k++) if ((vq.p[i + k] & 0xC0) != 0x80) bad = true;
-          n++; i += extra + 1;
-        }
-        if (n != r.len) bad = true;
-      }
-    }
-    uint64_t e0 = ebase + r.ctr;
-    if (want && (kind == OK_STYLE_START || kind == OK_STYLE_END)) { if (span) d.tb[e0] = (uint8_t)TB_ANCHOR; d.cp[e0] = CP_ANCHOR | (row - m.op0); want = false; }
-    const uint8_t* p = want ? d.data + d.op_val[row] : lim;
-    Rd v = rd_make(p, (uint64_t)(lim - p));
-    uint64_t nbytes = 0;
-    bool is_long = false, flat = false;
-    if (want && kind == OK_TEXT_INS) {
-      nbytes = rd_uleb(v);
-      if (v.bad || nbytes > rd_left(v)) { bad = true; want = false; }
-      else if (span && nbytes == r.len) flat = true;
-      else if (nbytes > 64) { is_long = true; }
-      else {
-        const uint8_t* s = v.p;
-        uint32_t n = 0;
-        for (uint32_t i = 0; i < (uint32_t)nbytes;) {
-          if (span && i + 4 <= (uint32_t)nbytes && n + 3 < r.len) {
+        for (uint32_t i = 0; i < nbytes;) {
+          if (span && i + 4 <= nbytes && n + 3 < r.len) {
             uint32_t w = ld32u(s + i);
             if (!(w & 0x80808080u)) { st32u(d.tb + e0 + n, w); n += 4; i += 4; continue; }
           }
-          if (!span && i + 4 <= (uint32_t)nbytes) {
+          if (!span && i + 4 <= nbytes) {
             uint32_t q0 = s[i], q1 = s[i + 1], q2 = s[i + 2], q3 = s[i + 3];
             if (((q0 | q1 | q2 | q3) & 0x80) == 0) {
               if (n + 3 < r.len) { d.cp[e0 + n] = q0; d.cp[e0 + n + 1] = q1; d.cp[e0 + n + 2] = q2; d.cp[e0 + n + 3] = q3; }
@@ -738,7 +798,7 @@
           else if ((b & 0xF0) == 0xE0) { cpv = b & 0x0F; extra = 2; }
           else if ((b & 0xF8) == 0xF0) { cpv = b & 0x07; extra = 3; }
           else { bad = true; break; }
-          if (i + extra >= (uint32_t)nbytes) { bad = true; break; }
+          if (i + extra >= nbytes) { bad = true; break; }
           for (uint32_t k = 1; k <= extra; k++) {
             uint32_t t = s[i + k];
             if ((t & 0xC0) != 0x80) bad = true;
@@ -754,6 +814,8 @@
         if (n != r.len) bad = true;
       }
     } else if (want) {
+      const uint8_t* p = d.data + d.op_val[row];
+      Rd v = rd_make(p, (uint64_t)(lim - p));
       (void)rd_u8(v);
       uint64_t cnt = rd_uleb(v);
       if (cnt != r.len) bad = true;
@@ -764,13 +826,28 @@
         if (v.bad) bad = true;
       }
     }
+    uint64_t lm_ = lmw::ballot(is_long);
+    while (lm_) {
+      int l = lmw::ffs64(lm_);
+      lm_ &= lm_ - 1;
+      uint64_t sp = (uint64_t)(s - d.data);
+      uint32_t sp_lo = lmw::bcast((uint32_t)sp, l), sp_hi = lmw::bcast((uint32_t)(sp >> 32), l);
+      uint32_t nb = lmw::bcast(nbytes, l);
+      uint32_t e_lo = lmw::bcast((uint32_t)e0, l), e_hi = lmw::bcast((uint32_t)(e0 >> 32), l);
+      uint32_t ln = lmw::bcast(r.len, l);
+      const uint8_t* str = d.data + (((uint64_t)sp_hi << 32) | sp_lo);
+      uint64_t e0l = ((uint64_t)e_hi << 32) | e_lo;
+      if (span ? fill_text_coop<true>(d, str, nb, e0l, ln) : fill_text_coop<false>(d, str, nb, e0l, ln)) bad = true;
+    }
+    const bool nvalid = g0 + 64 + (uint32_t)lane < n_op;
+    if (nvalid) rn = d.op[row + 64];
     if (span) {
-      uint32_t nd = flat ? ((uint32_t)nbytes + 3) / 4 : 0u;
+      uint32_t nd = flat ? (nbytes + 3) / 4 : 0u;
       uint32_t inc = lmw::scan_incl_add(nd);
       uint32_t total = lmw::bcast(inc, 63);
       if (total) {
         lmw::block_sync();
-        s_inc[lane] = inc; s_nb[lane] = (uint32_t)nbytes; s_src[lane] = (uint32_t)(v.p - vsec); s_dst[lane] = r.ctr;
+        s_inc[lane] = inc; s_nb[lane] = nbytes; s_src[lane] = soff; s_dst[lane] = r.ctr | (want ? DST_WANT : 0u);
         lmw::block_sync();
         uint32_t hi = 0;
         for (uint32_t f0 = 0; f0 < total; f0 += 64) {
@@ -781,27 +858,18 @@
             uint32_t nbr = s_nb[lo];
             uint32_t k4 = 4u * (f - (s_inc[lo] - (nbr + 3) / 4));
             const uint8_t* src = vsec + s_src[lo] + k4;
-            uint8_t* dst = d.tb + ebase + s_dst[lo] + k4;
-            if (k4 + 4 <= nbr) { uint32_t w = ld32u(src); hi |= w; st32u(dst, w); }
-            else for (uint32_t i = 0; k4 + i < nbr; i++) { uint32_t b = src[i]; hi |= b; dst[i] = (uint8_t)b; }
+            const uint32_t dw = s_dst[lo];
+            uint8_t* dst = d.tb + ebase + (dw & ~DST_WANT) + k4;
+            const bool st = (dw & DST_WANT) != 0;
+            if (k4 + 4 <= nbr) { uint32_t w = ld32u(src); hi |= w; if (st) st32u(dst, w); }
+            else for (uint32_t i = 0; k4 + i < nbr; i++) { uint32_t b = src[i]; hi |= b; if (st) dst[i] = (uint8_t)b; }
           }
         }
         if (hi & 0x80808080u) bad = true;
       }
     }
-    uint64_t lm_ = lmw::ballot(is_long);
-    while (lm_) {
-      int l = lmw::ffs64(lm_);
-      lm_ &= lm_ - 1;
-      uint64_t sp = (uint64_t)(v.p - d.data);
-      uint32_t sp_lo = lmw::bcast((uint32_t)sp, l), sp_hi = lmw::bcast((uint32_t)(sp >> 32), l);
-      uint32_t nb = lmw::bcast((uint32_t)nbytes, l);
-      uint32_t e_lo = lmw::bcast((uint32_t)e0, l), e_hi = lmw::bcast((uint32_t)(e0 >> 32), l);
-      uint32_t ln = lmw::bcast(r.len, l);
-      const uint8_t* str = d.data + (((uint64_t)sp_hi << 32) | sp_lo);
-      uint64_t e0l = ((uint64_t)e_hi << 32) | e_lo;
-      if (span ? fill_text_coop<true>(d, str, nb, e0l, ln) : fill_text_coop<false>(d, str, nb, e0l, ln)) bad = true;
-    }
+    if (remap) arrived(nvalid, row + 64);
+    if (nvalid) fn = d.chg_flag[rn.chg];
   }
   if (lmw::any(bad) && lane == 0) LM_SETERR(d.doc[doc].status, ST_DATA_CORRUPTION);
 }
diff --git a/loro_amd/csrc/lm_k_decode.h b/loro_amd/csrc/lm_k_decode.h
--- a/loro_amd/csrc/lm_k_decode.h
+++ b/loro_amd/csrc/lm_k_decode.h
@@ -444,12 +444,12 @@
 #else
 #define DEC_ST(code) do { st = st ? st : (code); } while (0)
 #endif
-LM_DEV void kc_add(uint32_t& n_map, uint32_t& n_el, uint32_t& n_style, uint32_t k, uint32_t len) {
+LM_DEV void kc_add(uint32_t& n_map, uint32_t& n_el, uint32_t& bits, uint32_t k, uint32_t len, bool nested) {
   n_map += (k == OK_MAP_SET || k == OK_MAP_DEL || k == OK_LIST_MOVE || k == OK_LIST_SET || k == OK_OTHER) ? 1u : 0u;
   n_el += (k == OK_TEXT_INS || k == OK_LIST_INS || k == OK_STYLE_START || k == OK_STYLE_END) ? len : (k == OK_LIST_MOVE ? 1u : 0u);
-  n_style += (k == OK_STYLE_START || k == OK_STYLE_END) ? 1u : 0u;
-}
-LM_DEV uint32_t kc_pack(uint32_t n_map, uint32_t n_style) { return (n_map & 0x7fffffffu) | (n_style ? 0x80000000u : 0u); }
+  bits |= ((k == OK_STYLE_START || k == OK_STYLE_END) ? 1u : 0u) | (nested ? 2u : 0u);
+}
+LM_DEV uint32_t kc_pack(uint32_t n_map, uint32_t bits) { return (n_map & BF_ROWS) | ((bits & 1u) ? BF_STYLE : 0u) | ((bits & 2u) ? BF_NESTED : 0u); }
 
 static constexpr uint32_t DEC_RECLASS = 0xDEC0DE01u;
 template <bool EXACT> LM_DEV void lane_skip_value(Rd& r, uint32_t& vf, int cdepth, uint32_t n_keys) {
@@ -634,6 +634,7 @@
       if (colbad) st = st ? st : ST_DECODE_ERROR;
     }
     Rd v = blk_sec(d, bd, SEC_VALUES);
+    const uint8_t* const vsec0 = v.p;
     uint64_t counter = bd.counter_start;
     uint32_t change_index = 0;
     uint64_t next_boundary = N > 1 ? d.chg[chg0 + 1].ctr : (uint64_t)bd.counter_start + bd.counter_len;
@@ -660,11 +661,12 @@
       uint32_t vfl = 0;
       bool nested = false;
       bool is_list_value = false;
+      uint32_t str_at = 0, str_nb = 0;
       switch (vt) {
         case 0: case 1: case 2: case 8: case 9: break;
         case 3: (void)rd_sleb(v); break;
         case 4: rd_skip(v, 8); break;
-        case 5: case 6: { uint64_t l = rd_uleb(v); rd_skip(v, l); break; }
+        case 5: case 6: { uint64_t l = rd_uleb(v); str_at = (uint32_t)(v.p - vsec0); str_nb = (uint32_t)l; rd_skip(v, l); break; }
         case 7: (void)rd_uleb(v); break;
         case 10: (void)rd_sleb(v); break;
         case 11: {
@@ -712,7 +714,7 @@
       if (EXACT && v.bad) DEC_ST(ST_DECODE_ERROR);
       bool take_del = false;
       if (ckind == CK_TEXT) {
-        if (vt == 5) kind = OK_TEXT_INS;
+        if (vt == 5) { kind = OK_TEXT_INS; r.a1 = str_at; r.a2 = (int32_t)str_nb; }
         else if (vt == 9) { kind = OK_DEL; take_del = true; }
         else if (vt == 12) { kind = OK_STYLE_START; r.a0 = mark_len; }
         else if (vt == 0) kind = OK_STYLE_END;
@@ -746,8 +748,9 @@
           if (d_peer.r.bad || d_ctr.r.bad || d_len.r.bad) DEC_ST(ST_DATA_CORRUPTION);
         }
       }
-      r.cidx_kind |= (kind << 16) | ((nested && (vt != 12 || kind == OK_STYLE_START)) ? OPF_NESTED : 0u);
-      kc_add(kc_map, kc_el, kc_style, kind, (uint32_t)len);
+      const bool row_nested = nested && (vt != 12 || kind == OK_STYLE_START);
+      r.cidx_kind |= (kind << 16) | (row_nested ? OPF_NESTED : 0u);
+      kc_add(kc_map, kc_el, kc_style, kind, (uint32_t)len, row_nested);
       d.op[op0 + row] = r;
       d.op_val[op0 + row] = val_at;
       d.op_blk[op0 + row] = bi;
@@ -770,6 +773,7 @@
   if (st == ST_OK && unsupported) st = ST_UNSUPPORTED;
   d.blk[bi].status = st;
   d.blk[bi].flags = kc_pack(kc_map, kc_style); d.blk[bi].pad = (st == ST_DECODE_ERROR || st == ST_DATA_CORRUPTION) ? DEC_RECLASS : kc_el;
+  if (st == ST_OK && kc_el && d.dec_stat) d.dec_stat[3] = 1u;
 }
 LM_KERNEL void k_block_decode(Dev d) { block_decode_lane<false>(d); }
 LM_KERNEL void k_block_head(Dev d) { block_decode_lane<false, true>(d); }
diff --git a/loro_amd/csrc/lm_k_decode_wave.h b/loro_amd/csrc/lm_k_decode_wave.h
--- a/loro_amd/csrc/lm_k_decode_wave.h
+++ b/loro_amd/csrc/lm_k_decode_wave.h
@@ -340,6 +340,7 @@
   else if (r == 6) { v_lo = -(int64_t)MAX_COUNTER; v_span = 2ull * MAX_COUNTER + 1; v_nz = true; v_repl = 1; v_prio = 7; }
   Rd v = rd_make(blk_p, 0);
   const uint64_t v_end_abs = ok ? bd.base + bdp->sec_rel[SEC_VALUES] + bdp->sec_len[SEC_VALUES] : 0ull;
+  const uint32_t vsec_lo = (uint32_t)v_end_abs - (ok ? bdp->sec_len[SEC_VALUES] : 0u);
   uint64_t counter = bd.counter_start;
   uint32_t change_index = 0, rows_in_change = 0;
   uint64_t next_boundary = 0;
@@ -423,7 +424,7 @@
             if (act) {
               uint64_t va = wpos + (inc - pay_r - base);
               uint32_t* o = sw + r * DEC_WW;
-              o[0] = (uint32_t)va; o[1] = (uint32_t)(va >> 32); o[2] = 0; o[3] = 0; o[4] = ctr7 + (cinc - len - cbase); o[5] = chg0 + ci7;
+              o[0] = (uint32_t)va; o[1] = (uint32_t)(va >> 32); o[2] = str_r ? len : 0u; o[3] = str_r ? hdr_r << 8 : 0u; o[4] = ctr7 + (cinc - len - cbase); o[5] = chg0 + ci7;
             }
             if (wn) { v.p += tot_pay; counter += tot_len; rows_in_change += wn; wn = 0; }
           }
@@ -518,9 +519,9 @@
           case 0: case 1: case 2: case 8: case 9: break;
           case 3: (void)rd_sleb(v); break;
           case 4: rd_skip(v, 8); break;
-          case 5: if (spec) { v.p += (wlen < 128u ? 1u : (wlen < 16384u ? 2u : (wlen < 2097152u ? 3u : 4u))) + wlen; break; }
+          case 5: if (spec) { const uint32_t h_ = wlen < 128u ? 1u : (wlen < 16384u ? 2u : (wlen < 2097152u ? 3u : 4u)); aux = wlen; flags = h_ << 8; v.p += h_ + wlen; break; }
             [[fallthrough]];
-          case 6: { uint64_t l = rd_uleb(v); rd_skip(v, l); break; }
+          case 6: { uint64_t l = rd_uleb(v); aux = (uint32_t)l; flags = ((uint32_t)((uint64_t)(v.p - d.data) - val_at) & 0xffu) << 8; rd_skip(v, l); break; }
           case 7: (void)rd_uleb(v); break;
           case 10: (void)rd_sleb(v); break;
           case 11: {
@@ -645,7 +646,7 @@
       orow.chg = o[5];
       uint32_t kind = OK_OTHER;
       if (ckind == CK_TEXT) {
-        if (vt == 5) kind = OK_TEXT_INS;
+        if (vt == 5) { kind = OK_TEXT_INS; orow.a1 = o[0] - vsec_lo + ((o[3] >> 8) & 0xffu); orow.a2 = (int32_t)aux; }
         else if (vt == 9) kind = OK_DEL;
         else if (vt == 12) { kind = OK_STYLE_START; orow.a0 = aux; }
         else if (vt == 0) kind = OK_STYLE_END;
@@ -672,8 +673,9 @@
         if (!has_del) dec_err(errk, row, 4, ST_DATA_CORRUPTION);
         else { orow.a0 = sx[r * 8 + 4]; orow.a1 = sx[r * 8 + 5]; orow.a2 = (int32_t)sx[r * 8 + 6]; }
       }
-      orow.cidx_kind |= (kind << 16) | (((o[3] & 4) && (vt != 12 || kind == OK_STYLE_START)) ? OPF_NESTED : 0u);
-      kc_add(kc_map, kc_el, kc_style, kind, len);
+      const bool row_nested = (o[3] & 4) && (vt != 12 || kind == OK_STYLE_START);
+      orow.cidx_kind |= (kind << 16) | (row_nested ? OPF_NESTED : 0u);
+      kc_add(kc_map, kc_el, kc_style, kind, len, row_nested);
       d.op[op0 + row] = orow;
       d.op_val[op0 + row] = (uint64_t)o[0] | ((uint64_t)o[1] << 32);
       d.op_blk[op0 + row] = bi;
@@ -704,7 +706,7 @@
     uint32_t oe = lmw::shfl_xor(errk, m), ot = lmw::shfl_xor(tail, m);
     errk = oe < errk ? oe : errk;
     tail |= ot;
-    kc_map += lmw::shfl_xor(kc_map, m); kc_el += lmw::shfl_xor(kc_el, m); kc_style += lmw::shfl_xor(kc_style, m);
+    kc_map += lmw::shfl_xor(kc_map, m); kc_el += lmw::shfl_xor(kc_el, m); kc_style |= lmw::shfl_xor(kc_style, m);
   }
   if (ok && r == 0) {
 #ifdef LM_EMU_TRACE
@@ -718,6 +720,7 @@
     if (st == ST_OK && (tail & 4)) st = ST_UNSUPPORTED;
     d.blk[bi].status = st;
     d.blk[bi].flags = kc_pack(kc_map, kc_style); d.blk[bi].pad = (st == ST_DECODE_ERROR || st == ST_DATA_CORRUPTION) ? DEC_RECLASS : kc_el;
+    if (st == ST_OK && kc_el && d.dec_stat) d.dec_stat[3] = 1u;
   }
 #ifdef LM_PROF_DEC
   DEC_PH(7);
diff --git a/loro_amd/csrc/lm_k_map_fused.h b/loro_amd/csrc/lm_k_map_fused.h
--- a/loro_amd/csrc/lm_k_map_fused.h
+++ b/loro_amd/csrc/lm_k_map_fused.h
@@ -475,7 +475,7 @@
     const BlockDesc* bdp = d.blk + bi;
     const uint64_t base = bdp->base;
     const uint32_t N = bdp->n_changes, cs = bdp->counter_start, cl = bdp->counter_len;
-    const uint32_t n_ops = bdp->flags & 0x7fffffffu;
+    const uint32_t n_ops = bdp->flags & BF_ROWS;
     const uint32_t* bo = d.boff + (uint64_t)bi * BCN;
     const uint32_t chg0 = bo[BC_CHG], cidr0 = bo[BC_CID];
     const uint32_t n_cids = d.bcnt[(uint64_t)bi * BCN + BC_CID];
diff --git a/loro_amd/csrc/lm_pipeline.h b/loro_amd/csrc/lm_pipeline.h
--- a/loro_amd/csrc/lm_pipeline.h
+++ b/loro_amd/csrc/lm_pipeline.h
@@ -172,7 +172,7 @@
     std::vector<DocMeta> h_doc;
   } sv;
 
-  struct Knobs { bool span = true, decode_wave = true, no_opt_dir = false, loc_memset = true, loc_poison = false; int plain = 2; uint32_t dec_slot = 1264, dec_slot_big = 4096, dec_big_mode = 1, dir_opt_max = 0; size_t lds_pad = 0; long long slab_cap = -1; uint32_t ht_opt = 2048, cut_min_rows = 2048, vs_row_cost = 300; bool lww_lds = true, fuse_rows = true, version_sweep = true, span_auto = true, linear = true, posdel = true, reclass = true, redo = true, map_fused = true, snapshot_state = true, snapshot_state_force = false, stage_direct = true; uint32_t mf_min_rows = 2048, mf_chg_ratio = 4, pd_state_pieces = 2; } kn;
+  struct Knobs { bool span = true, decode_wave = true, no_opt_dir = false, loc_memset = true, loc_poison = false; int plain = 2; uint32_t dec_slot = 1264, dec_slot_big = 4096, dec_big_mode = 1, dir_opt_max = 0; size_t lds_pad = 0; long long slab_cap = -1; uint32_t ht_opt = 2048, cut_min_rows = 2048, vs_row_cost = 300; bool lww_lds = true, fuse_rows = true, fill_remap = true, version_sweep = true, span_auto = true, linear = true, posdel = true, reclass = true, redo = true, map_fused = true, snapshot_state = true, snapshot_state_force = false, stage_direct = true; uint32_t mf_min_rows = 2048, mf_chg_ratio = 4, pd_state_pieces = 2; } kn;
   void read_knobs() {
     Knobs k;
     if (const char* e = getenv("LM_SPAN")) k.span = atoi(e) != 0;
@@ -195,6 +195,7 @@
     if (const char* e = getenv("LM_VERSION_SWEEP")) k.version_sweep = atoi(e) != 0;
     if (const char* e = getenv("LM_FUSE_ROWS")) k.fuse_rows = atoi(e) != 0;
     if (const char* e = getenv("LM_POSDEL")) k.posdel = atoi(e) != 0;
+    if (const char* e = getenv("LM_FILL_REMAP")) k.fill_remap = atoi(e) != 0;
     if (const char* e = getenv("LM_LINEAR")) k.linear = atoi(e) != 0;
     if (const char* e = getenv("LM_LWW_LDS")) k.lww_lds = atoi(e) != 0;
     if (const char* e = getenv("LM_REDO")) k.redo = atoi(e) != 0;
@@ -769,6 +770,7 @@
     results.assign(n_docs, DocResult{0, 0, 0, 0, 0, 0});
     if (n_docs == 0) { ran = true; return; }
     const bool reuse = resident && tables_valid;
+    bool rows_deferred = false;
     prev_copied = resident && have_prev;
     if (resident && have_prev) {
       b_prev_doc.ensure((size_t)n_docs * sizeof(DocMeta)); lmbe::d2d(b_prev_doc.p, b_doc_saved.p, (size_t)n_docs * sizeof(DocMeta));
@@ -833,7 +835,7 @@
     if (NB) LM_LAUNCH(k_block_desc, cdiv(NB, 64), 64, d);
     b_tot.ensure(64 * 4);
     d.dec_stat = b_tot.as<uint32_t>() + 48; d.dec_slot = kn.dec_slot; d.cut_min_rows = kn.cut_min_rows; d.vs_row_cost = kn.vs_row_cost;
-    lmbe::dmemset(d.dec_stat, 0, 12);
+    lmbe::dmemset(d.dec_stat, 0, 16);
     n_fused = 0;
     h_fused.assign(n_docs, 0);
     const bool mf_on = kn.map_fused && !no_map_fused && kn.redo && kn.lww_lds && kn.ht_opt && kn.ht_opt <= LWW_LDS_CAP && !resident && st_valid && NB;
@@ -920,7 +922,9 @@
     LM_LAUNCH(k_doc_ranges, cdiv(n_docs, 64), 64, d);
     LM_LAUNCH(k_doc_tables, n_docs, 64, d);
     uint32_t nmax = NO > NC ? NO : NC;
-    if (nmax) LM_LAUNCH(k_remap, cdiv(nmax, 256), 256, d, NO, NC);
+    rows_deferred = kn.fill_remap && NB && NO;
+    if (nmax) LM_LAUNCH(k_remap, cdiv(nmax, 256), 256, d, NO, NC, rows_deferred ? 1u : 0u);
+    if (rows_deferred) LM_LAUNCH(k_remap_nested, cdiv(NB, 4), 256, d, NB);
     lmbe::toc("k_doc_tables+k_remap", times, profiling);
     lmbe::tic(profiling);
     LM_LAUNCH(k_dag_a, n_docs, 64, d, g);
@@ -1144,7 +1148,9 @@
     lmbe::tic(profiling);
     bool any_elems = resident;
     for (uint32_t i = 0; i < n_docs && !any_elems; i++) any_elems = h_doc[i].status == ST_OK && h_doc[i].n_elems != 0;
-    if (NB && !reuse && any_elems) LM_LAUNCH(k_elem_fill, NB, 64, d);
+    if (NB && !reuse && any_elems && resident && rows_deferred) LM_LAUNCH(k_remap_kept, NB, 64, d);
+    if (NB && !reuse && any_elems) LM_LAUNCH(k_elem_fill, NB, 64, d, rows_deferred ? 1u : 0u);
+    else if (!reuse && rows_deferred) LM_LAUNCH(k_remap_rows, 1024, 256, d, NO, 1024u * 256u);
     lmbe::toc("k_elem_fill", times, profiling);
     lmbe::tic(profiling);
     b_tot.ensure(64 * 4);
diff --git a/loro_amd/csrc/lm_types.h b/loro_amd/csrc/lm_types.h
--- a/loro_amd/csrc/lm_types.h
+++ b/loro_amd/csrc/lm_types.h
@@ -40,6 +40,7 @@
   uint32_t flags;
   uint32_t pad;
 };
+enum : uint32_t { BF_NESTED = 1u << 30, BF_STYLE = 1u << 31, BF_ROWS = (1u << 30) - 1 };
 struct BlockCounts { uint32_t n_chg, n_dep, n_op, n_key, n_cid, n_peer; };
 static constexpr int BC_N = 6;
 
```

New measurement: 503,900 docs/s, median of 6. About the same (+0.6%).
